# Litianyu141/Gen-FVGN-steady

Hardware: AMD Instinct MI355X
Metric: training iters/sec, 50k-cell cylinder mesh (fwd + loss + bwd + Adam, batch resident in HBM) (higher is better)
Workload: dtype f32

## Files before the change

### gen-fvgn-steady_amd/csrc/cfwd.hip

```cpp
#include <cstdlib>

#include "tchain_kernel.h"

#include "gfv_limits.h"
int* gfv_internal_status_ptr();

namespace {

constexpr float CF_SH = 16.0f;
constexpr float CF_SH_INV = 1.0f / 16.0f;
constexpr float CF_SH_LIMIT = 2048.0f;

__device__ __forceinline__ void cf_barrier() {
  asm volatile("s_waitcnt lgkmcnt(0)\n\ts_barrier" ::: "memory");
}

template <int KT0, int TG, int NW>
struct CfLds {
  static constexpr int KTB = KT0 > 4 ? KT0 : 4;
  static constexpr int B0 = 0;
  static constexpr int B1 = TG * KTB * 2048;
  static constexpr int SINV = B1 + TG * 8192;
  static constexpr int LNP = SINV + TG * 64;
  static constexpr int TOTAL = LNP + TG * 16 * NW * 8;
// ... 109 lines not shown
      for (int q = 0; q < TG; ++q) {
        const gfv_f16x8* f = reinterpret_cast<const gfv_f16x8*>(xbuf + (size_t)(q * KT + T) * 2048) + lane;
        const gfv_f16x8 xh = f[0];
        if (!LOWP) {
          const gfv_f16x8 xl = f[64];
#pragma unroll
          for (int n = 0; n < NT; ++n) {
            acc[q][n] = __builtin_amdgcn_mfma_f32_16x16x32_f16(wl[n][T], xh, acc[q][n], 0, 0, 0);
            acc[q][n] = __builtin_amdgcn_mfma_f32_16x16x32_f16(wh[n][T], xl, acc[q][n], 0, 0, 0);
          }
        }
#pragma unroll
        for (int n = 0; n < NT; ++n) acc[q][n] = gfv_mma_hh<BF>(wh[n][T], xh, acc[q][n]);
      }
    }
  };
  auto load_w = [&](const void* image) {
    const gfv_f16x8* im = reinterpret_cast<const gfv_f16x8*>(image) + (size_t)(NT * w) * 128 + lane;
#pragma unroll
    for (int T = 0; T < 4; ++T)
#pragma unroll
      for (int n = 0; n < NT; ++n) {
        wh[n][T] = im[T * 1024 + n * 128];
        if (!LOWP) wl[n][T] = im[T * 1024 + n * 128 + 64];
      }
  };
  auto hidden = [&](int layer, char* xout, float* save) {
#pragma unroll
    for (int q = 0; q < TG; ++q) {
      const int row = row0 + 16 * q + j;
      const bool live = q < ngt && row < A.M;
      const float si = layer == 0 ? sinv[q * 16 + j] : CF_SH_INV;
      float a[4 * NT];
#pragma unroll
      for (int n = 0; n < NT; ++n) {
        const float4 b = bias[layer][n];
        float v[4] = {(acc[q][n][0] * si) * invw + b.x, (acc[q][n][1] * si) * invw + b.y, (acc[q][n][2] * si) * invw + b.z,
                      (acc[q][n][3] * si) * invw + b.w};
        if (PADD && layer == 0) {
          v[0] += ps[PADD ? q : 0][n].x + pr[PADD ? q : 0][n].x; v[1] += ps[PADD ? q : 0][n].y + pr[PADD ? q : 0][n].y;
          v[2] += ps[PADD ? q : 0][n].z + pr[PADD ? q : 0][n].z; v[3] += ps[PADD ? q : 0][n].w + pr[PADD ? q : 0][n].w;
        }
        if (save && live) st4(save + (size_t)row * 128 + c0 + 16 * n, v);
        const gfv_f2 g01 = gfv_gelu2(gfv_f2{v[0], v[1]}), g23 = gfv_gelu2(gfv_f2{v[2], v[3]});
        a[4 * n + 0] = g01.x; a[4 * n + 1] = g01.y; a[4 * n + 2] = g23.x; a[4 * n + 3] = g23.y;
      }
      float m = 0.f;
#pragma unroll
      for (int e = 0; e < 4 * NT; e += 2) m = max3_abs(m, a[e], a[e + 1]);
      mabs = fmaxf(mabs, live ? m : 0.f);
      if constexpr (NT == 2) {
        float e8[8];
#pragma unroll
        for (int e = 0; e < 8; ++e) e8[e] = a[e] * CF_SH;
        gfv_uint4 hi, lo;
        gfv_split8_t<BF>(e8, hi, lo);
        gfv_uint4* dst = reinterpret_cast<gfv_uint4*>(xout + (size_t)(q * 4 + w) * 2048) + lane;
        dst[0] = hi;
        if (!LOWP) dst[64] = lo;
      } else {
        unsigned h0, h1, l0, l1;
        gfv_split_pair_t<BF>(a[0] * CF_SH, a[1] * CF_SH, h0, l0);
        gfv_split_pair_t<BF>(a[2] * CF_SH, a[3] * CF_SH, h1, l1);
        char* dst = xout + (size_t)(q * 4 + (w >> 1)) * 2048 + lane * 16 + (w & 1) * 8;
        *reinterpret_cast<uint2*>(dst) = make_uint2(h0, h1);
        if (!LOWP) *reinterpret_cast<uint2*>(dst + 1024) = make_uint2(l0, l1);
      }
    }
  };

  mma(b0, std::integral_constant<int, KT0>{});
  load_w(A.layer[1].Wh);
  hidden(0, b1, A.layer[0].save);
  cf_barrier();
  mma(b1, std::integral_constant<int, 4>{});
  load_w(A.layer[2].Wh);
  hidden(1, b0, A.layer[1].save);
  float4 gam[NT], bet[NT];
  if constexpr (FINLN) {
#pragma unroll
    for (int n = 0; n < NT; ++n) { gam[n] = ld4(A.fin_gamma + c0 + 16 * n); bet[n] = ld4(A.fin_beta + c0 + 16 * n); }
  }
  float4 rres[TG][NT];
  if (A.res[0]) {
#pragma unroll
    for (int q = 0; q < TG; ++q) {
      const float* rp = A.res[0] + (size_t)min(row0 + 16 * q + j, A.M - 1) * A.res_ld[0] + c0;
#pragma unroll
      for (int n = 0; n < NT; ++n) rres[q][n] = ld4(rp + 16 * n);
    }
  }
  cf_barrier();
  if constexpr (!FINLN) {
    if (w == 0) {
      mma(b0, std::integral_constant<int, 4>{});
      const int ncol = A.layer[2].N;
      const float* bp = A.layer[2].bias;
#pragma unroll
      for (int q = 0; q < TG; ++q) {
        const int row = row0 + 16 * q + j;
        if (q < ngt && row < A.M) {
#pragma unroll
          for (int r = 0; r < 4; ++r) {
            const int col = 4 * g + r;
            if (col < ncol) A.out[0][(size_t)row * A.out_ld[0] + col] = (acc[q][0][r] * CF_SH_INV) * invw + (bp ? bp[col] : 0.f);
          }
        }
      }
    }
    if (mabs > CF_SH_LIMIT) atomicOr(status, 2);
    return;
  }
  mma(b0, std::integral_constant<int, 4>{});
  const int hcols = (A.hidden > 0 && A.hidden < 128) ? A.hidden : 128;
  float y[TG][4 * NT];
#pragma unroll
  for (int q = 0; q < TG; ++q) {
    const int row = row0 + 16 * q + j;
    const bool live = q < ngt && row < A.M;
    float s = 0.f;
#pragma unroll
    for (int n = 0; n < NT; ++n) {
      const float4 b = bias[2][n];
      float v[4] = {(acc[q][n][0] * CF_SH_INV) * invw + b.x, (acc[q][n][1] * CF_SH_INV) * invw + b.y,
                    (acc[q][n][2] * CF_SH_INV) * invw + b.z, (acc[q][n][3] * CF_SH_INV) * invw + b.w};
      if (A.fin_presave && live) st4(A.fin_presave + (size_t)row * 128 + c0 + 16 * n, v);
#pragma unroll
      for (int r = 0; r < 4; ++r) {
        y[q][4 * n + r] = v[r];
        s += v[r];
      }
    }
    const float mw = row_sum(s) * (1.0f / (16.0f * NT));
    float m2 = 0.f;
#pragma unroll
    for (int e = 0; e < 4 * NT; ++e) {
      const float d = y[q][e] - mw;
      m2 += d * d;
    }
    m2 = row_sum(m2);
    if (g == 0) *reinterpret_cast<float2*>(lnp + ((q * 16 + j) * NW + w) * 2) = make_float2(mw, m2);
  }
  cf_barrier();
  {
    const float inv_h = 1.0f / (float)hcols, npad = (float)(128 - hcols);
#pragma unroll
    for (int q = 0; q < TG; ++q) {
      const int row = row0 + 16 * q + j;
      const bool live = q < ngt && row < A.M;
      const float4* pp = reinterpret_cast<const float4*>(lnp + (q * 16 + j) * 2 * NW);
      float m128, m2a;
      if constexpr (NW == 4) {
        const float4 p0 = pp[0], p1 = pp[1];
        m128 = ((p0.x + p0.z) + (p1.x + p1.z)) * 0.25f;
        const float e0 = p0.x - m128, e1 = p0.z - m128, e2 = p1.x - m128, e3 = p1.z - m128;
        m2a = ((p0.y + p0.w) + (p1.y + p1.w)) + 32.0f * ((e0 * e0 + e1 * e1) + (e2 * e2 + e3 * e3));
      } else {
        const float4 p0 = pp[0], p1 = pp[1], p2 = pp[2], p3 = pp[3];
        m128 = (((p0.x + p0.z) + (p1.x + p1.z)) + ((p2.x + p2.z) + (p3.x + p3.z))) * 0.125f;
        const float e0 = p0.x - m128, e1 = p0.z - m128, e2 = p1.x - m128, e3 = p1.z - m128, e4 = p2.x - m128, e5 = p2.z - m128,
                    e6 = p3.x - m128, e7 = p3.z - m128;
        m2a = (((p0.y + p0.w) + (p1.y + p1.w)) + ((p2.y + p2.w) + (p3.y + p3.w))) +
              16.0f * (((e0 * e0 + e1 * e1) + (e2 * e2 + e3 * e3)) + ((e4 * e4 + e5 * e5) + (e6 * e6 + e7 * e7)));
      }
      const float mean = hcols == 128 ? m128 : (m128 * 128.0f) * inv_h;
      const float dm = m128 - mean;
      const float m2 = hcols == 128 ? m2a : (m2a + 128.0f * dm * dm) - npad * (mean * mean);
      const float rstd = rsqrtf(m2 * inv_h + 1e-5f);
      if (A.fin_stats && live && w == 0 && g == 0) *reinterpret_cast<float2*>(A.fin_stats + 2 * (size_t)row) = make_float2(mean, rstd);
#pragma unroll
      for (int n = 0; n < NT; ++n) {
        const float4 ga = gam[n], be = bet[n];
        float o[4] = {(y[q][4 * n + 0] - mean) * rstd * ga.x + be.x, (y[q][4 * n + 1] - mean) * rstd * ga.y + be.y,
                      (y[q][4 * n + 2] - mean) * rstd * ga.z + be.z, (y[q][4 * n + 3] - mean) * rstd * ga.w + be.w};
        if (live) {
          if (A.out_nores) st4(A.out_nores + (size_t)row * 128 + c0 + 16 * n, o);
          if (A.res[0]) { o[0] += rres[q][n].x; o[1] += rres[q][n].y; o[2] += rres[q][n].z; o[3] += rres[q][n].w; }
          st4(A.out[0] + (size_t)row * A.out_ld[0] + c0 + 16 * n, o);
        }
      }
    }
  }
  if (mabs > CF_SH_LIMIT) atomicOr(status, 2);
}

inline bool cf_al16(const void* p) { return (reinterpret_cast<size_t>(p) & 15) == 0; }

template <int KT0, int N0, bool PADD, bool RAGIN, bool FINLN = true>
void cf_launch(const gfv_rowtile_args_t& a, int lowp, hipStream_t stream) {
  int* st = gfv_internal_status_ptr();
  constexpr int tg = 2;
  const int tiles = (a.M + 16 * tg - 1) / (16 * tg);
  const dim3 grid(PADD ? gfv_xcd_grid(tiles) : tiles), blk(512);
  if (lowp == 2) GFV_LAUNCH((cfwd_kernel<KT0, N0, 2, PADD, 2, RAGIN, 8, FINLN>), grid, blk, 0, stream, a, st);
  else if (lowp) GFV_LAUNCH((cfwd_kernel<KT0, N0, 2, PADD, 1, RAGIN, 8, FINLN>), grid, blk, 0, stream, a, st);
  else GFV_LAUNCH((cfwd_kernel<KT0, N0, 2, PADD, 0, RAGIN, 8, FINLN>), grid, blk, 0, stream, a, st);
}

}

int gfv_internal_cfwd_try(const gfv_rowtile_args_t* a, int lowp, hipStream_t stream, int dry) {
  if (!gfv_internal_status_ptr()) return 0;
  const int on = gfv_internal_limit(GFV_LIM_CFWD_ON);
  const int max_m = gfv_internal_limit(GFV_LIM_CFWD_MAX_M);
  if (!on || a->nlayers != 3 || a->M > max_m || a->M < 1 || (a->flags & (GFV_CHAIN_ROW_OWNER | GFV_CHAIN_COLUMN_OWNER))) return 0;
  const bool dec = a->fin_op == GFV_FIN_PLAIN && a->layer[2].N >= 1 && a->layer[2].N <= 16 && !a->res[0] && !a->out_nores && !a->fin_presave &&
                   !a->fin_stats && !a->padd && a->nseg == 1 && a->layer[0].K == 128;
  if (a->in_op != GFV_IN_NONE || !a->wmax) return 0;
  if (!dec && (a->fin_op != GFV_FIN_LN || !a->fin_gamma || !a->fin_beta)) return 0;
  if (a->in_add || a->gadd || a->in_save || a->in_aux || a->ln_partial || a->gscale || a->dw_partial || a->in_stats || a->fin_aux) return 0;
  for (int l = 0; l < 3; ++l) {
    const gfv_layer_t& L = a->layer[l];
    if (!L.Wh || (L.N != 128 && !(dec && l == 2)) || L.aux || L.bias2 || (L.bias && !cf_al16(L.bias) && !(dec && l == 2))) return 0;
    if (L.op != (l < 2 ? GFV_OP_BIAS_GELU : GFV_OP_NONE)) return 0;
    if (l > 0 && L.K != 128) return 0;
    if (L.save && !cf_al16(L.save)) return 0;
  }
  if (a->layer[2].save) return 0;
  if (!a->out[0] || a->out[1] || a->out[2] || (!dec && ((a->out_ld[0] & 3) || !cf_al16(a->out[0]))) || a->res[1] || a->res[2]) return 0;
  if (a->res[0] && ((a->res_ld[0] & 3) || !cf_al16(a->res[0]))) return 0;
  if ((a->out_nores && !cf_al16(a->out_nores)) || (a->fin_presave && !cf_al16(a->fin_presave)) ||
      (!dec && (!cf_al16(a->fin_gamma) || !cf_al16(a->fin_beta))))
    return 0;
  if (a->fin_stats && (reinterpret_cast<size_t>(a->fin_stats) & 7)) return 0;
  for (int i = 0; i < a->nseg; ++i)
    if (a->seg[i].idx || a->seg[i].csr_rowptr || a->seg[i].csr_scale || a->seg[i].save) return 0;
  const int K0 = a->layer[0].K;
  int shape = -1;
  auto plain = [&](int i, int width) {
    const gfv_seg_t& s = a->seg[i];
    return s.width == width && (s.ld & 3) == 0 && cf_al16(s.ptr);
  };
  if (a->padd) {
    if (a->nseg == 1 && K0 == 128 && plain(0, 128) && a->padd_s && a->padd_r && a->padd_ld >= 256 && (a->padd_ld & 3) == 0 && cf_al16(a->padd))
      shape = 1;
  } else if (a->nseg == 2 && K0 == 192 && plain(0, 64) && plain(1, 128)) {
    shape = 0;
  } else if (dec) {
    if (plain(0, 128)) shape = 4;
  } else if (a->nseg == 1 && K0 == 128 && plain(0, 128)) {
    shape = 2;
  } else if (a->nseg == 1 && K0 <= 32 && a->seg[0].width == K0) {
    shape = 3;
  }
  if (shape < 0) return 0;
  if (dry) return 1;
  if (shape == 0) cf_launch<6, 4, false, false>(*a, lowp, stream);
  else if (shape == 1) cf_launch<4, 8, true, false>(*a, lowp, stream);
  else if (shape == 2) cf_launch<4, 8, false, false>(*a, lowp, stream);
  else if (shape == 4) cf_launch<4, 8, false, false, false>(*a, lowp, stream);
  else cf_launch<1, 2, false, true>(*a, lowp, stream);
  return 1;
}
```

### gen-fvgn-steady_amd/csrc/colchain.hip

```cpp
#include "colchain_kernel.h"

int* gfv_internal_status_ptr();

static int cc_env(const char* name, int dflt) {
  const char* e = getenv(name);
  return e ? atoi(e) : dflt;
}
static bool al16(const void* p) { return (reinterpret_cast<size_t>(p) & 15) == 0; }

static int cc_cus() {
  static int n = 0;
  if (!n) {
    int dev = 0;
    hipDeviceProp_t pr;
    if (hipGetDevice(&dev) == hipSuccess && hipGetDeviceProperties(&pr, dev) == hipSuccess) n = pr.multiProcessorCount;
    if (n <= 0) n = 256;
    const int want = cc_env("GFV_COLCHAIN_WGS", 0);
    if (want > 0 && want <= n) n = want;
  }
  return n;
}

static bool cc_bwd_ok(const gfv_rowtile_args_t* a) {
  static const int on = cc_env("GFV_COLCHAIN_BWD", 1);
  static const int min_m = cc_env("GFV_COLCHAIN_BWD_MIN_M", 2048);
  if (a->flags & GFV_CHAIN_ROW_OWNER) return false;
  if (!(a->flags & GFV_CHAIN_COLUMN_OWNER) && (!on || a->M < min_m)) return false;
  if (!a->dw_partial || a->dw_partial_stride < GFV_DW_FUSED_FLOATS || !a->in_stats || !a->wmax) return false;
  if (a->dw_in) return false;
  const bool noout = a->nlayers == 2;
  const bool rc = a->rc_Wh[0] != nullptr;
  if (rc && (!a->rc_Wh[1] || a->dw_in || !al16(a->rc_Wh[0]) || !al16(a->rc_Wh[1]) || (a->rc_bias[0] && !al16(a->rc_bias[0])) ||
             (a->rc_bias[1] && !al16(a->rc_bias[1]))))
    return false;
  if (!rc && a->rc_Wh[1]) return false;
  if ((a->nlayers != 3 && !noout) || a->in_op != GFV_IN_LNBWD || a->fin_op != GFV_FIN_PLAIN || a->nseg != 1) return false;
  if (noout && (a->layer[1].op != GFV_OP_MUL_DGELU || a->layer[1].save || a->res[0] || a->gadd || a->dw_in || !a->out[0])) return false;
  if (a->seg[0].width != 128 || a->seg[0].idx || a->seg[0].csr_rowptr || a->seg[0].save || a->seg[0].ld != 128 || !al16(a->seg[0].ptr)) return false;
  if (a->M > (1 << 22) || a->out_ld[0] != 128 || (a->res[0] && a->res_ld[0] != 128) || (a->dw_in && a->dw_in_ld != 128)) return false;
  if (a->layer[0].op != GFV_OP_MUL_DGELU || a->layer[1].op != GFV_OP_MUL_DGELU || (!noout && a->layer[2].op != GFV_OP_NONE)) return false;
  for (int l = 0; l < a->nlayers; ++l) {
    const gfv_layer_t& L = a->layer[l];
    if (!L.Wh || (L.N != 128 && !(l == 2 && L.N == 192)) || L.K != 128 || L.bias || L.bias2) return false;
    if (l < 2 && !(rc && l == 0) && (!L.aux || !al16(L.aux))) return false;
    if (L.save && !al16(L.save)) return false;
  }
  if ((!rc && (!a->in_aux || !al16(a->in_aux))) || !a->in_gamma || !al16(a->in_gamma) || a->ln_partial || a->padd) return false;
  const bool out2 = !noout && a->layer[2].N == 192;
  if (!a->out[0] || (out2 ? (!a->out[1] || a->out_ld[1] != 64 || !al16(a->out[1]) || a->dw_in) : a->out[1] != nullptr) || a->out[2] ||
      a->res[1] || a->res[2] || a->out_nores)
    return false;
  if ((a->out_ld[0] & 3) || !al16(a->out[0]) || (a->res[0] && ((a->res_ld[0] & 3) || !al16(a->res[0])))) return false;
  if (a->in_add && !al16(a->in_add)) return false;
  if (a->gadd && (!al16(a->gadd) || !a->gadd_s || !a->gadd_r)) return false;
  if (a->in_save && !al16(a->in_save)) return false;
  if ((reinterpret_cast<size_t>(a->in_stats) & 7) || !al16(a->dw_partial) || (a->dw_partial_stride & 3)) return false;
  return true;
}
extern "C" int gfv_hidden_size(void);
extern "C" int gfv_f16split_enabled(void);
extern "C" int gfv_rowtile_dw_partials(void) { return cc_cus(); }
extern "C" int gfv_rowtile_dw_partials_m(int32_t M) {
  const int tiles = (M + 63) / 64;
  return tiles < cc_cus() ? (tiles > 0 ? tiles : 1) : cc_cus();
}
extern "C" int gfv_rowtile_fuses_dw(const gfv_rowtile_args_t* a) {
  if (!a || gfv_hidden_size() != 128 || gfv_f16split_enabled() == 0) return 0;
  gfv_rowtile_args_t t = *a;
  t.hidden = 128;
  return cc_bwd_ok(&t) ? 1 : 0;
}

int gfv_internal_colchain_try(const gfv_rowtile_args_t* a, hipStream_t stream) {
  if (a->hidden == 128 && cc_bwd_ok(a)) {
    int* st = gfv_internal_status_ptr();
    if (!st) return 0;
    const dim3 grid(gfv_rowtile_dw_partials_m(a->M)), blk(64 * CC_W);
#define CB_K(...) GFV_LAUNCH((colchain_bwd_kernel<__VA_ARGS__>), grid, blk, 0, stream, *a, st)
#define CB_LAUNCH(LOWP, RC)                                                                                                      \
  do {                                                                                                                           \
    if (a->nlayers == 2) CB_K(LOWP, false, false, true, RC);                                                                     \
    else if (a->layer[2].N == 192 && a->gadd) CB_K(LOWP, true, true, false, RC);                                                 \
    else if (a->layer[2].N == 192) CB_K(LOWP, false, true, false, RC);                                                           \
    else if (a->gadd) CB_K(LOWP, true, false, false, RC);                                                                        \
    else CB_K(LOWP, false, false, false, RC);                                                                                    \
  } while (0)
    const bool rc = a->rc_Wh[0] != nullptr;
    if (a->product_form == 2) { if (rc) CB_LAUNCH(2, true); else CB_LAUNCH(2, false); }
    else if (a->product_form != 0) { if (rc) CB_LAUNCH(1, true); else CB_LAUNCH(1, false); }
    else { if (rc) CB_LAUNCH(0, true); else CB_LAUNCH(0, false); }
#undef CB_K
#undef CB_LAUNCH
    return 2;
  }
  return 0;
}
```

### gen-fvgn-steady_amd/csrc/colchain_kernel.h

```cpp
#pragma once
#include "tchain_kernel.h"

namespace {

constexpr int CC_W = 8;
constexpr float CC_SH = 16.0f;
constexpr float CC_SH_INV = 1.0f / 16.0f;
constexpr float CC_SH_LIMIT = 2048.0f;
#ifdef GFV_CC_TIMING
#define CT_DECL long long ct_[16] = {0, 0, 0, 0, 0, 0, 0, 0, 0, 0, 0, 0, 0, 0, 0, 0}; long long ct_prev_ = clock64();
#define CT(k) do { __builtin_amdgcn_s_waitcnt(0xc07f); const long long now_ = clock64(); ct_[k] += now_ - ct_prev_; ct_prev_ = now_; } while (0)
#else
#define CT_DECL
#define CT(k)
#endif
__device__ __forceinline__ void cc_barrier() {
  asm volatile("s_waitcnt lgkmcnt(0)\n\ts_barrier" ::: "memory");
}

struct CcCtx {
  int w, lane, j, g, col0;
  int M;
  int row0;
  int ngt;
// ... 16 lines not shown
      a0 = __builtin_amdgcn_mfma_f32_16x16x32_f16(wl[T], xh0, a0, 0, 0, 0);
      a1 = __builtin_amdgcn_mfma_f32_16x16x32_f16(wl[T], xh1, a1, 0, 0, 0);
      a0 = __builtin_amdgcn_mfma_f32_16x16x32_f16(wh[T], xl0, a0, 0, 0, 0);
      a1 = __builtin_amdgcn_mfma_f32_16x16x32_f16(wh[T], xl1, a1, 0, 0, 0);
    }
    a0 = gfv_mma_hh<LOWP == 2>(wh[T], xh0, a0);
    a1 = gfv_mma_hh<LOWP == 2>(wh[T], xh1, a1);
    if (FENCE) __builtin_amdgcn_sched_barrier(0);
  }
}

template <bool BF>
__device__ __forceinline__ void cc_put_frag(char* xbuf, int q, const CcCtx& c, const float (&a)[4], float scale) {
  unsigned h0, h1, l0, l1;
  const gfv_f2 s01 = gfv_f2{a[0], a[1]} * gfv_splat2(scale), s23 = gfv_f2{a[2], a[3]} * gfv_splat2(scale);
  gfv_split_pair_t<BF>(s01.x, s01.y, h0, l0);
  gfv_split_pair_t<BF>(s23.x, s23.y, h1, l1);
  char* dst = xbuf + (size_t)((q * 4 + (c.w >> 1)) * 2) * 1024 + c.lane * 16 + (c.w & 1) * 8;
  *reinterpret_cast<uint2*>(dst) = make_uint2(h0, h1);
  *reinterpret_cast<uint2*>(dst + 1024) = make_uint2(l0, l1);
}

constexpr int CB_TG = 4;
struct CbLds {
  static constexpr int BUF = CB_TG * 8192;
  static constexpr int B0 = 0, B1 = BUF, B2 = 2 * BUF;
  static constexpr int PART = 3 * BUF;
  static constexpr int SMAX = PART + CB_TG * 16 * 8 * 8;
  static constexpr int TOTAL = SMAX + 64;
};

__device__ __forceinline__ void cb_tr_operand(const char* xbuf, int q0, int ct, int lane, gfv_f16x8& hi, gfv_f16x8& lo) {
  typedef short s4 __attribute__((ext_vector_type(4)));
  typedef __attribute__((address_space(3))) s4* lds_s4;
  const int s = lane & 15, gp = lane >> 4;
  const int off = ((q0 * 4 + (ct >> 1)) * 2) * 1024 + (16 * (s & 3) + 4 * gp + (s >> 2)) * 16 + (ct & 1) * 8;
  const char* p = xbuf + off;
  const s4 h0 = __builtin_amdgcn_ds_read_tr16_b64_v4i16((lds_s4)(p));
  const s4 l0 = __builtin_amdgcn_ds_read_tr16_b64_v4i16((lds_s4)(p + 1024));
  const s4 h1 = __builtin_amdgcn_ds_read_tr16_b64_v4i16((lds_s4)(p + 8192));
  const s4 l1 = __builtin_amdgcn_ds_read_tr16_b64_v4i16((lds_s4)(p + 8192 + 1024));
  typedef short s8 __attribute__((ext_vector_type(8)));
  const s8 h = {h0[0], h0[1], h0[2], h0[3], h1[0], h1[1], h1[2], h1[3]};
  const s8 l = {l0[0], l0[1], l0[2], l0[3], l1[0], l1[1], l1[2], l1[3]};
  hi = __builtin_bit_cast(gfv_f16x8, h);
  lo = __builtin_bit_cast(gfv_f16x8, l);
}

__device__ __forceinline__ int cb_dw_ntile(int w, int i) { return 2 * (w >> 1) + (i >> 2); }
__device__ __forceinline__ int cb_dw_ktile(int w, int i) { return 4 * (w & 1) + (i & 3); }
__device__ __forceinline__ int cb_dw_btile(int w) { return 2 * (w >> 1) + (w & 1); }
template <int LOWP>
__device__ __forceinline__ void cb_dw_tile(const char* gbuf, const char* abuf, int npairs, int w, int lane, floatx4 (&acc)[8],
                                           floatx4& accb) {
  const gfv_f16x8 ones = gfv_frag_ones<LOWP == 2>();
  const int nt0 = 2 * (w >> 1), kt0 = 4 * (w & 1);
  for (int pr = 0; pr < npairs; ++pr) {
    gfv_f16x8 gh[2], gl[2];
    cb_tr_operand(gbuf, 2 * pr, nt0, lane, gh[0], gl[0]);
    cb_tr_operand(gbuf, 2 * pr, nt0 + 1, lane, gh[1], gl[1]);
    {
      const bool odd = (w & 1) != 0;
      const gfv_f16x8 bh = odd ? gh[1] : gh[0], bl = odd ? gl[1] : gl[0];
      if (!LOWP) accb = __builtin_amdgcn_mfma_f32_16x16x32_f16(bl, ones, accb, 0, 0, 0);
      accb = gfv_mma_hh<LOWP == 2>(bh, ones, accb);
    }
#pragma unroll
    for (int kk = 0; kk < 4; ++kk) {
      gfv_f16x8 ah, al;
      cb_tr_operand(abuf, 2 * pr, kt0 + kk, lane, ah, al);
#pragma unroll
      for (int nn = 0; nn < 2; ++nn) {
        if (!LOWP) {
          acc[4 * nn + kk] = __builtin_amdgcn_mfma_f32_16x16x32_f16(gl[nn], ah, acc[4 * nn + kk], 0, 0, 0);
          acc[4 * nn + kk] = __builtin_amdgcn_mfma_f32_16x16x32_f16(gh[nn], al, acc[4 * nn + kk], 0, 0, 0);
        }
        acc[4 * nn + kk] = gfv_mma_hh<LOWP == 2>(gh[nn], ah, acc[4 * nn + kk]);
      }
    }
    __builtin_amdgcn_sched_barrier(0);
  }
}

template <bool BF>
__device__ __forceinline__ void cb_hidden_bwd(CcCtx& c, int q, const floatx4& acc, float inv_in, const float4& z, float sg,
                                              char* gout, char* aout, float (&v)[4]) {
  const gfv_f2 z01 = {z.x, z.y}, z23 = {z.z, z.w};
  gfv_f2 a01, a23, d01, d23;
  gfv_gelu_dgelu2(z01, a01, d01);
  gfv_gelu_dgelu2(z23, a23, d23);
  const gfv_f2 ki = gfv_splat2(inv_in), kw = gfv_splat2(c.invw);
  const gfv_f2 v01 = ((gfv_f2{acc[0], acc[1]} * ki) * kw) * d01, v23 = ((gfv_f2{acc[2], acc[3]} * ki) * kw) * d23;
  v[0] = v01.x; v[1] = v01.y; v[2] = v23.x; v[3] = v23.y;
  const float a[4] = {a01.x, a01.y, a23.x, a23.y};
  const float mq = max3_abs(max3_abs(0.f, v[0], v[1]), v[2], v[3]) * sg;
  const float ma = max3_abs(max3_abs(0.f, a[0], a[1]), a[2], a[3]) * (60000.0f / CC_SH_LIMIT);
  c.mabs = fmaxf(c.mabs, q < c.ngt ? fmaxf(mq, ma) : 0.f);
  cc_put_frag<BF>(gout, q, c, v, sg);
  cc_put_frag<BF>(aout, q, c, a, CC_SH);
}

__device__ __forceinline__ char* cb_own_slot(char* xbuf, int q, const CcCtx& c) {
  return xbuf + (size_t)((q * 4 + (c.w >> 1)) * 2) * 1024 + c.lane * 16 + (c.w & 1) * 8;
}
__device__ __forceinline__ void cb_park4(char* xbuf, int q, const CcCtx& c, const float (&v)[4]) {
  char* d = cb_own_slot(xbuf, q, c);
  *reinterpret_cast<float2*>(d) = make_float2(v[0], v[1]);
  *reinterpret_cast<float2*>(d + 1024) = make_float2(v[2], v[3]);
}
__device__ __forceinline__ void cb_unpark4(char* xbuf, int q, const CcCtx& c, float (&v)[4]) {
  const char* d = cb_own_slot(xbuf, q, c);
  const float2 a = *reinterpret_cast<const float2*>(d), b = *reinterpret_cast<const float2*>(d + 1024);
  v[0] = a.x; v[1] = a.y; v[2] = b.x; v[3] = b.y;
}

template <bool BF>
__device__ __forceinline__ void cb_hidden_bwd_dg(CcCtx& c, int q, const floatx4& acc, float inv_in, const float (&dg)[4], float sg,
                                                 char* gout, float (&v)[4]) {
#pragma unroll
  for (int r = 0; r < 4; ++r) v[r] = ((acc[r] * inv_in) * c.invw) * dg[r];
  const float mq = max3_abs(max3_abs(0.f, v[0], v[1]), v[2], v[3]) * sg;
  c.mabs = fmaxf(c.mabs, q < c.ngt ? mq : 0.f);
  cc_put_frag<BF>(gout, q, c, v, sg);
}

typedef int cb_i32x4 __attribute__((ext_vector_type(4)));
typedef int cb_i32x2 __attribute__((ext_vector_type(2)));
typedef __amdgpu_buffer_rsrc_t cb_rsrc;
constexpr int CB_OFF_DEAD = 0x7ffffff0;
__device__ __forceinline__ cb_rsrc cb_buf(const void* p, size_t bytes) {
  const size_t n = p ? (bytes < 0x7fffffe0ull ? bytes : 0x7fffffe0ull) : 0;
  return __builtin_amdgcn_make_buffer_rsrc(const_cast<void*>(p), 0, (int)n, 0x00020000);
}
typedef float cb_f32x2 __attribute__((ext_vector_type(2)));
__device__ __forceinline__ float4 cb_ld4(cb_rsrc r, int off) {
  const floatx4 f = __builtin_bit_cast(floatx4, __builtin_amdgcn_raw_buffer_load_b128(r, off, 0, 0));
  return make_float4(f[0], f[1], f[2], f[3]);
}
__device__ __forceinline__ float2 cb_ld2(cb_rsrc r, int off) {
  const cb_f32x2 f = __builtin_bit_cast(cb_f32x2, __builtin_amdgcn_raw_buffer_load_b64(r, off, 0, 0));
  return make_float2(f[0], f[1]);
}
__device__ __forceinline__ void cb_st4v(cb_rsrc r, int off, const floatx4& f) {
  __builtin_amdgcn_raw_buffer_store_b128(__builtin_bit_cast(cb_i32x4, f), r, off, 0, 0);
}
__device__ __forceinline__ void cb_st4(cb_rsrc r, int off, const float (&v)[4]) {
  const floatx4 f = {v[0], v[1], v[2], v[3]};
  __builtin_amdgcn_raw_buffer_store_b128(__builtin_bit_cast(cb_i32x4, f), r, off, 0, 0);
}

struct CbIn {
  float4 dy[CB_TG], yv[CB_TG], ga[CB_TG];
  float2 st[CB_TG];
};
struct CbBufs {
  cb_rsrc dy, y3, stats, z2, z1, gadd, gidx, save1, res, out;
};
__device__ __forceinline__ int cb_off(const CcCtx& c, int row0, int q) { return min(row0 + 16 * q + c.j, c.M - 1) * 512 + c.col0 * 4; }

template <bool GADD>
__device__ __forceinline__ void cb_load_gidx(const CbBufs& B, const CcCtx& c, int row0, int (&gidx)[CB_TG]) {
  if (GADD) {
#pragma unroll
    for (int q = 0; q < CB_TG; ++q) gidx[q] = __builtin_amdgcn_raw_buffer_load_b32(B.gidx, min(row0 + 16 * q + c.j, c.M - 1) * 4, 0, 0);
  }
}
__device__ __forceinline__ void cb_load_inputs(const CbBufs& B, const CcCtx& c, int row0, CbIn& in) {
#pragma unroll
  for (int q = 0; q < CB_TG; ++q) {
    const int off = cb_off(c, row0, q);
    in.dy[q] = cb_ld4(B.dy, off);
    in.yv[q] = cb_ld4(B.y3, off);
    in.st[q] = cb_ld2(B.stats, min(row0 + 16 * q + c.j, c.M - 1) * 8);
  }
}
__device__ __forceinline__ void cb_load_dy_stats(const CbBufs& B, const CcCtx& c, int row0, CbIn& in) {
#pragma unroll
  for (int q = 0; q < CB_TG; ++q) {
    in.dy[q] = cb_ld4(B.dy, cb_off(c, row0, q));
    in.st[q] = cb_ld2(B.stats, min(row0 + 16 * q + c.j, c.M - 1) * 8);
  }
}
__device__ __forceinline__ void cb_load_rows(cb_rsrc r, const CcCtx& c, int row0, float4 (&v)[CB_TG]) {
#pragma unroll
  for (int q = 0; q < CB_TG; ++q) v[q] = cb_ld4(r, cb_off(c, row0, q));
}
template <bool GADD>
__device__ __forceinline__ void cb_load_gathers(const CbBufs& B, const CcCtx& c, const int (&gidx)[CB_TG], CbIn& in) {
  if (GADD) {
#pragma unroll
    for (int q = 0; q < CB_TG; ++q) in.ga[q] = cb_ld4(B.gadd, gidx[q] * 256 + (c.col0 & 63) * 4);
  }
}

template <int LOWP, bool GADD, bool OUT2 = false, bool NOOUT = false, bool RC = false>
__global__ __launch_bounds__(64 * CC_W, 2) void colchain_bwd_kernel(const gfv_rowtile_args_t A, int* status) {
  constexpr int TG = CB_TG;
  __shared__ __attribute__((aligned(16))) char lds[CbLds::TOTAL + (RC ? CbLds::BUF : 0)];
  char* b0 = lds + CbLds::B0;
  char* b1 = lds + CbLds::B1;
  char* b2 = lds + CbLds::B2;
  char* b3 = lds + CbLds::TOTAL;
  float* part = reinterpret_cast<float*>(lds + CbLds::PART);
  float* smax = reinterpret_cast<float*>(lds + CbLds::SMAX);

  CcCtx c;
  c.w = __builtin_amdgcn_readfirstlane(threadIdx.x >> 6);
  c.lane = threadIdx.x & 63;
  c.j = c.lane & 15;
  c.g = c.lane >> 4;
  c.col0 = 16 * c.w + 4 * c.g;
  c.M = A.M;
  c.mabs = 0.f;
  c.invw = 1.0f / gfv_pow2_scale(*A.wmax);

  const int nwg = gridDim.x;
  const int wg = (nwg & 7) == 0 ? (int)(blockIdx.x & 7) * (nwg >> 3) + (int)(blockIdx.x >> 3) : (int)blockIdx.x;
  const int NG = (A.M + 15) >> 4;
  const int g_beg = (int)((long)NG * wg / nwg), g_end = (int)((long)NG * (wg + 1) / nwg);

  const size_t rows128 = (size_t)A.M * 512;
  CbBufs B;
  B.dy = cb_buf(A.seg[0].ptr, rows128);
  B.y3 = cb_buf(RC ? nullptr : A.in_aux, rows128);
  B.stats = cb_buf(A.in_stats, (size_t)A.M * 8);
  B.z2 = cb_buf(RC ? nullptr : A.layer[0].aux, rows128);
  B.z1 = cb_buf(A.layer[1].aux, rows128);
  B.gadd = cb_buf(A.gadd, 0x7fffffe0ull);
  B.gidx = cb_buf(c.w < 4 ? A.gadd_s : A.gadd_r, (size_t)A.M * 4);
  B.save1 = cb_buf(NOOUT ? A.out[0] : A.layer[1].save, rows128);
  B.res = cb_buf(NOOUT ? nullptr : A.res[0], rows128);
  B.out = cb_buf(NOOUT ? nullptr : A.out[0], rows128);
  const cb_rsrc out2 = cb_buf(OUT2 ? A.out[1] : nullptr, (size_t)A.M * 256);

  const cb_rsrc w0 = cb_buf(A.layer[0].Wh, 65536), w1 = cb_buf(A.layer[1].Wh, 65536),
                w2 = cb_buf(NOOUT ? nullptr : A.layer[2].Wh, OUT2 ? 131072 : 65536);
  const cb_rsrc rw2 = cb_buf(RC ? A.rc_Wh[0] : nullptr, 65536), rw3 = cb_buf(RC ? A.rc_Wh[1] : nullptr, 65536);
  const int woff = (c.w * 128 + c.lane) * 16;
  floatx4 dw3[8], dw2[8], db3 = floatx4{0.f, 0.f, 0.f, 0.f}, db2 = db3;
#pragma unroll
  for (int kt = 0; kt < 8; ++kt) dw3[kt] = dw2[kt] = floatx4{0.f, 0.f, 0.f, 0.f};
  float dgam[4] = {0.f, 0.f, 0.f, 0.f}, dbet[4] = {0.f, 0.f, 0.f, 0.f};
  float sacc = 0.f;
  float scap = 3.0e38f;

  float step1, step2;
  {
    float l1[2];
#pragma unroll
    for (int l = 0; l < 2; ++l) {
      const cb_rsrc wb = l == 0 ? w0 : w1;
      float acc = 0.f;
#pragma unroll
      for (int T = 0; T < 4; ++T) {
        const gfv_f16x8 h = __builtin_bit_cast(gfv_f16x8, __builtin_amdgcn_raw_buffer_load_b128(wb, woff + T * 16384, 0, 0));
        const gfv_f16x8 lo = __builtin_bit_cast(gfv_f16x8, __builtin_amdgcn_raw_buffer_load_b128(wb, woff + T * 16384 + 1024, 0, 0));
        if (LOWP == 2) {
          const gfv_bf16x8 hb = __builtin_bit_cast(gfv_bf16x8, h);
#pragma unroll
          for (int e = 0; e < 8; ++e) acc += fabsf((float)hb[e]);
        } else {
#pragma unroll
          for (int e = 0; e < 8; ++e) acc += fabsf((float)h[e] + (float)lo[e]);
        }
      }
      l1[l] = gfv_wave_max(row_sum(acc));
    }
    if (c.lane == 0) { smax[c.w] = l1[0]; part[c.w] = l1[1]; }
    cc_barrier();
    float m0 = 0.f, m1 = 0.f;
#pragma unroll
    for (int k = 0; k < 8; ++k) { m0 = fmaxf(m0, smax[k]); m1 = fmaxf(m1, part[k]); }
    cc_barrier();
    const float g0 = 1.13f * m0 * c.invw, g1 = 1.13f * m1 * c.invw;
    step1 = 1.0f / gfv_pow2_ceil(g0);
    step2 = 1.0f / gfv_pow2_ceil(g1);
  }

  constexpr bool PRE = true;
  int gidx[TG] = {0, 0, 0, 0};
  CbIn in;
  float4 zn[RC ? TG : 1];
  if (g_beg < g_end) {
    cb_load_gidx<GADD>(B, c, 16 * g_beg, gidx);
    if constexpr (RC) {
      cb_load_rows(B.z1, c, 16 * g_beg, zn);
      cb_load_dy_stats(B, c, 16 * g_beg, in);
      cb_load_gathers<GADD>(B, c, gidx, in);
    } else if (PRE) {
      cb_load_inputs(B, c, 16 * g_beg, in);
      cb_load_gathers<GADD>(B, c, gidx, in);
    }
  }
  const bool CB_LATE = c.w >= 4;
  CT_DECL
  for (int t0 = g_beg; t0 < g_end; t0 += TG) {
    c.row0 = 16 * t0;
    c.ngt = min(TG, g_end - t0);
    const int np = (c.ngt + 1) >> 1;
    const int next_row0 = t0 + TG < g_end ? 16 * (t0 + TG) : c.M;
    int offL[TG], offS[TG];
#pragma unroll
    for (int q = 0; q < TG; ++q) {
      const int row = c.row0 + 16 * q + c.j;
      offL[q] = cb_off(c, c.row0, q);
      offS[q] = (q < c.ngt && row < c.M) ? row * 512 + c.col0 * 4 : CB_OFF_DEAD;
    }
    if constexpr (RC) {
      gfv_f16x8 rh[4], rl[4];
#pragma unroll
      for (int T = 0; T < 4; ++T) {
        rh[T] = __builtin_bit_cast(gfv_f16x8, __builtin_amdgcn_raw_buffer_load_b128(rw2, woff + T * 16384, 0, 0));
        rl[T] = __builtin_bit_cast(gfv_f16x8, __builtin_amdgcn_raw_buffer_load_b128(rw2, woff + T * 16384 + 1024, 0, 0));
      }
      const float4 zero4 = make_float4(0.f, 0.f, 0.f, 0.f);
#pragma unroll
      for (int q = 0; q < TG; ++q) {
        const float z4[4] = {zn[q].x, zn[q].y, zn[q].z, zn[q].w};
        float a[4];
#pragma unroll
        for (int r = 0; r < 4; ++r) a[r] = gfv_gelu(z4[r]);
        const float ma = max3_abs(max3_abs(0.f, a[0], a[1]), a[2], a[3]) * (60000.0f / CC_SH_LIMIT);
        c.mabs = fmaxf(c.mabs, q < c.ngt ? ma : 0.f);
        cc_put_frag<LOWP == 2>(b3, q, c, a, CC_SH);
      }
// ... 135 lines not shown
      s3 = fminf(gfv_pow2_scale(mx * 13.5f) * 2.0f, scap);
      scap = fminf(scap, s3 * 1048576.0f);
#pragma unroll
      for (int q = 0; q < TG; ++q) {
        const float4* pp = reinterpret_cast<const float4*>(part + (q * 16 + c.j) * 16);
        const float4 p0 = pp[0], p1 = pp[1], p2 = pp[2], p3 = pp[3];
        const float m1 = (((p0.x + p0.z) + (p1.x + p1.z)) + ((p2.x + p2.z) + (p3.x + p3.z))) * 0.0078125f;
        const float m2 = (((p0.y + p0.w) + (p1.y + p1.w)) + ((p2.y + p2.w) + (p3.y + p3.w))) * 0.0078125f;
        float g3[4];
#pragma unroll
        for (int h = 0; h < 2; ++h) {
          const int r = 2 * h;
          const gfv_f2 t = gfv_splat2(rs[q]) * ((gfv_f2{gg[q][r], gg[q][r + 1]} - gfv_splat2(m1)) - gfv_f2{xh[q][r], xh[q][r + 1]} * gfv_splat2(m2));
          g3[r] = t.x; g3[r + 1] = t.y;
        }
        if (A.in_save) cb_st4(cb_buf(A.in_save, rows128), offS[q], g3);
        cc_put_frag<LOWP == 2>(b0, q, c, g3, s3);
      }
    }
    if (sacc != 0.f && sacc != s3) {
      const float ratio = s3 / sacc;
#pragma unroll
      for (int kt = 0; kt < 8; ++kt) { dw3[kt] *= ratio; dw2[kt] *= ratio; }
      db3 *= ratio;
      db2 *= ratio;
    }
    sacc = s3;
    const float s2s = s3 * step1, s1s = s2s * step2;
    if (A.gscale && c.w == 0 && c.lane < c.ngt) {
      const size_t grp = (size_t)(c.row0 >> 4) + c.lane;
      A.gscale[grp] = s3 * 0.25f;
      A.gscale[(size_t)A.gscale_ld + grp] = s2s * 0.25f;
      A.gscale[2 * (size_t)A.gscale_ld + grp] = s1s * 0.25f;
    }
    CT(2);
    cc_barrier();
    CT(3);
    cb_load_gidx<GADD>(B, c, next_row0, gidx);
    {
      const float inv_in = 1.0f / s3;
      floatx4 a0, a1;
      cc_mma_pair<4, LOWP, true>(b0, 0, wh, wl, c.lane, a0, a1);
#pragma unroll
      for (int p = 0; p < TG / 2; ++p) {
        if (p >= np) break;
        floatx4 n0 = a0, n1 = a1;
        float v0[4], v1[4];
        if (!CB_LATE && p + 1 < TG / 2) cc_mma_pair<4, LOWP, true>(b0, p + 1, wh, wl, c.lane, n0, n1);
        if constexpr (RC) {
          float d0[4], d1[4];
          cb_unpark4(b1, 2 * p, c, d0);
          cb_unpark4(b1, 2 * p + 1, c, d1);
          cb_hidden_bwd_dg<LOWP == 2>(c, 2 * p, a0, inv_in, d0, s2s, b1, v0);
          cb_hidden_bwd_dg<LOWP == 2>(c, 2 * p + 1, a1, inv_in, d1, s2s, b1, v1);
        } else {
          cb_hidden_bwd<LOWP == 2>(c, 2 * p, a0, inv_in, zq[2 * p], s2s, b1, b2, v0);
          cb_hidden_bwd<LOWP == 2>(c, 2 * p + 1, a1, inv_in, zq[2 * p + 1], s2s, b1, b2, v1);
        }
        if (A.layer[0].save) {
          const cb_rsrc s0 = cb_buf(A.layer[0].save, rows128);
          cb_st4(s0, offS[2 * p], v0);
          cb_st4(s0, offS[2 * p + 1], v1);
        }
        if (CB_LATE && p + 1 < TG / 2) cc_mma_pair<4, LOWP, true>(b0, p + 1, wh, wl, c.lane, n0, n1);
        a0 = n0; a1 = n1;
      }
    }
#pragma unroll
    for (int T = 0; T < 4; ++T) {
      wh[T] = __builtin_bit_cast(gfv_f16x8, __builtin_amdgcn_raw_buffer_load_b128(w1, woff + T * 16384, 0, 0));
      wl[T] = __builtin_bit_cast(gfv_f16x8, __builtin_amdgcn_raw_buffer_load_b128(w1, woff + T * 16384 + 1024, 0, 0));
    }
#pragma unroll
    for (int q = 0; q < TG; ++q) zq[q] = cb_ld4(B.z1, offL[q]);
    CT(4);
    cc_barrier();
    CT(5);
    if constexpr (RC) cb_load_rows(B.z1, c, next_row0, zn);
    cb_dw_tile<LOWP>(b0, b2, np, c.w, c.lane, dw3, db3);
    if constexpr (RC) cb_dw_tile<LOWP>(b1, b3, np, c.w, c.lane, dw2, db2);
    CT(6);
    cc_barrier();
    CT(7);
    {
      const float inv_in = 1.0f / s2s;
      floatx4 a0, a1;
      cc_mma_pair<4, LOWP, true>(b1, 0, wh, wl, c.lane, a0, a1);
#pragma unroll
      for (int p = 0; p < TG / 2; ++p) {
        if (p >= np) break;
        floatx4 n0 = a0, n1 = a1;
        float v0[4], v1[4];
        if (!CB_LATE && p + 1 < TG / 2) cc_mma_pair<4, LOWP, true>(b1, p + 1, wh, wl, c.lane, n0, n1);
        if constexpr (RC) {
          const float d0[4] = {gfv_dgelu(zq[2 * p].x), gfv_dgelu(zq[2 * p].y), gfv_dgelu(zq[2 * p].z), gfv_dgelu(zq[2 * p].w)};
          const float d1[4] = {gfv_dgelu(zq[2 * p + 1].x), gfv_dgelu(zq[2 * p + 1].y), gfv_dgelu(zq[2 * p + 1].z),
                               gfv_dgelu(zq[2 * p + 1].w)};
          cb_hidden_bwd_dg<LOWP == 2>(c, 2 * p, a0, inv_in, d0, s1s, b0, v0);
          cb_hidden_bwd_dg<LOWP == 2>(c, 2 * p + 1, a1, inv_in, d1, s1s, b0, v1);
        } else {
          cb_hidden_bwd<LOWP == 2>(c, 2 * p, a0, inv_in, zq[2 * p], s1s, b0, b2, v0);
          cb_hidden_bwd<LOWP == 2>(c, 2 * p + 1, a1, inv_in, zq[2 * p + 1], s1s, b0, b2, v1);
        }
        cb_st4(B.save1, offS[2 * p], v0);
        cb_st4(B.save1, offS[2 * p + 1], v1);
        if (CB_LATE && p + 1 < TG / 2) cc_mma_pair<4, LOWP, true>(b1, p + 1, wh, wl, c.lane, n0, n1);
        a0 = n0; a1 = n1;
      }
    }
    if constexpr (!NOOUT) {
#pragma unroll
      for (int T = 0; T < 4; ++T) {
        wh[T] = __builtin_bit_cast(gfv_f16x8, __builtin_amdgcn_raw_buffer_load_b128(w2, woff + T * 16384, 0, 0));
        wl[T] = __builtin_bit_cast(gfv_f16x8, __builtin_amdgcn_raw_buffer_load_b128(w2, woff + T * 16384 + 1024, 0, 0));
      }
    }
    float4 rr[NOOUT ? 1 : TG];
    if constexpr (!NOOUT) {
#pragma unroll
      for (int q = 0; q < TG; ++q) rr[q] = cb_ld4(B.res, offL[q]);
    }
    CT(8);
    cc_barrier();
    CT(9);
    if constexpr (!NOOUT) {
      const float inv_in = 1.0f / s1s;
      floatx4 a0, a1;
      cc_mma_pair<4, LOWP, true>(b0, 0, wh, wl, c.lane, a0, a1);
#pragma unroll
      for (int p = 0; p < TG / 2; ++p) {
        if (p >= np) break;
        floatx4 n0 = a0, n1 = a1;
        if (!CB_LATE && p + 1 < TG / 2) cc_mma_pair<4, LOWP, true>(b0, p + 1, wh, wl, c.lane, n0, n1);
        const floatx4 o0 = (a0 * inv_in) * c.invw + floatx4{rr[2 * p].x, rr[2 * p].y, rr[2 * p].z, rr[2 * p].w};
        const floatx4 o1 = (a1 * inv_in) * c.invw + floatx4{rr[2 * p + 1].x, rr[2 * p + 1].y, rr[2 * p + 1].z, rr[2 * p + 1].w};
        cb_st4v(B.out, offS[2 * p], o0);
        cb_st4v(B.out, offS[2 * p + 1], o1);
        if (CB_LATE && p + 1 < TG / 2) cc_mma_pair<4, LOWP, true>(b0, p + 1, wh, wl, c.lane, n0, n1);
        a0 = n0; a1 = n1;
      }
      if constexpr (OUT2) {
        if (c.w < 4) {
          gfv_f16x8 xh2[4], xl2[4];
#pragma unroll
          for (int T = 0; T < 4; ++T) {
            xh2[T] = __builtin_bit_cast(gfv_f16x8, __builtin_amdgcn_raw_buffer_load_b128(w2, 65536 + woff + T * 16384, 0, 0));
            xl2[T] = __builtin_bit_cast(gfv_f16x8, __builtin_amdgcn_raw_buffer_load_b128(w2, 65536 + woff + T * 16384 + 1024, 0, 0));
          }
#pragma unroll
          for (int p = 0; p < TG / 2; ++p) {
            if (p >= np) break;
            floatx4 e0, e1;
            cc_mma_pair<4, LOWP, true>(b0, p, xh2, xl2, c.lane, e0, e1);
            const floatx4 o0 = (e0 * inv_in) * c.invw, o1 = (e1 * inv_in) * c.invw;
            const int ra = c.row0 + 32 * p + c.j, rb = ra + 16;
            cb_st4v(out2, (2 * p < c.ngt && ra < c.M) ? ra * 256 + c.col0 * 4 : CB_OFF_DEAD, o0);
            cb_st4v(out2, (2 * p + 1 < c.ngt && rb < c.M) ? rb * 256 + c.col0 * 4 : CB_OFF_DEAD, o1);
          }
        }
      }
    }
    CT(10);
    if constexpr (RC) {
      cb_load_dy_stats(B, c, next_row0, in);
      cb_load_gathers<GADD>(B, c, gidx, in);
    } else {
      if (PRE) {
        cb_load_inputs(B, c, next_row0, in);
        cb_load_gathers<GADD>(B, c, gidx, in);
      }
      cb_dw_tile<LOWP>(b1, b2, np, c.w, c.lane, dw2, db2);
    }
    CT(11);
  }

#ifdef GFV_CC_TIMING
  if (c.lane == 0 && A.fin_aux) {
    long long* dbg = reinterpret_cast<long long*>(const_cast<float*>(A.fin_aux)) + ((size_t)blockIdx.x * CC_W + c.w) * 16;
    for (int kk = 0; kk < 16; ++kk) dbg[kk] = ct_[kk];
  }
#endif
  if (A.dw_partial) {
    float* blk = A.dw_partial + (size_t)blockIdx.x * A.dw_partial_stride;
    const float is = sacc != 0.f ? 1.0f / sacc : 0.f;
    const float r2 = 1.0f / step1, r1 = r2 / step2;
    const float u3 = is * CC_SH_INV, u2 = (is * r2) * CC_SH_INV;
#pragma unroll
    for (int kt = 0; kt < 8; ++kt)
#pragma unroll
      for (int r = 0; r < 4; ++r) {
        const int n = 16 * cb_dw_ntile(c.w, kt) + 4 * c.g + r, k = 16 * cb_dw_ktile(c.w, kt) + c.j;
        blk[n * 128 + k] = dw3[kt][r] * u3;
        blk[16384 + 128 + n * 128 + k] = dw2[kt][r] * u2;
      }
    if (c.j == 0) {
#pragma unroll
      for (int r = 0; r < 4; ++r) {
        const int nb = 16 * cb_dw_btile(c.w) + 4 * c.g + r;
        blk[16384 + nb] = db3[r] * is;
        blk[2 * 16384 + 128 + nb] = db2[r] * (is * r2);
      }
    }
#pragma unroll
    for (int r = 0; r < 4; ++r) {
      const float dg = gfv_row16_sum(dgam[r]), db = gfv_row16_sum(dbet[r]);
      if (c.j == 0) {
        blk[2 * 16384 + 256 + c.col0 + r] = dg;
        blk[2 * 16384 + 384 + c.col0 + r] = db;
      }
    }
  }
  if (c.mabs > 60000.0f) atomicOr(status, 2);
}


}
```

### gen-fvgn-steady_amd/csrc/rowtile.hip

```cpp
#include <atomic>
#include <stdio.h>
#include <stdlib.h>
#include <mutex>
#include "gfv_common.h"
#include "gfv_limits.h"
#include "gfv_prof.h"
#include "../../include/gfv.h"

namespace {
constexpr int BM = 64;
}

int gfv_internal_tchain_launch(const gfv_rowtile_args_t* args, int ragged, int f16, hipStream_t stream);

static std::atomic<int> g_f16_default{-1};
static thread_local int g_f16split = -1;
static int f16_default() {
  int d = g_f16_default.load(std::memory_order_relaxed);
  if (d < 0) {
    const char* e = getenv("GFV_F16SPLIT");
    d = e ? ((atoi(e) == 2 || atoi(e) == 3) ? atoi(e) : (atoi(e) != 0)) : 1;
    int expect = -1;
    if (!g_f16_default.compare_exchange_strong(expect, d)) d = expect;
  }
// ... 22 lines not shown

static thread_local int g_last_path = -1;
extern "C" int gfv_rowtile_last_path(void) { return g_last_path; }
namespace {
struct LimitDef { const char* env; int dflt; };
const LimitDef k_limits[GFV_LIM_COUNT] = {
    {"GFV_CBWD", 1},        {"GFV_CBWD_MAX_M", 25000},      {"GFV_CFWD", 1},          {"GFV_CFWD_MAX_M", 250000},
    {"GFV_CTRANS", 1},         {"GFV_CTRANS_MAX_M", 16384},
    {"GFV_LIN1S", 1},       {"GFV_LIN1S_MAX_M", 16384}};
int g_limit[GFV_LIM_COUNT];
bool g_limit_set[GFV_LIM_COUNT];
std::once_flag g_limit_once;
void limits_init() {
  for (int i = 0; i < GFV_LIM_COUNT; ++i) {
    const char* e = getenv(k_limits[i].env);
    g_limit[i] = e ? atoi(e) : k_limits[i].dflt;
    g_limit_set[i] = false;
  }
}
}
int gfv_internal_limit(int which) {
  std::call_once(g_limit_once, limits_init);
  return (which >= 0 && which < GFV_LIM_COUNT) ? g_limit[which] : 0;
}
extern "C" int gfv_get_limit(int32_t which) { return (which >= 0 && which < GFV_LIM_COUNT) ? gfv_internal_limit(which) : -1; }
extern "C" int gfv_set_limit(int32_t which, int32_t value) {
  if (which < 0 || which >= GFV_LIM_COUNT) return GFV_ERR_ARG;
  std::call_once(g_limit_once, limits_init);
  if (value < 0) {
    const char* e = getenv(k_limits[which].env);
    g_limit[which] = e ? atoi(e) : k_limits[which].dflt;
  } else {
    g_limit[which] = value;
  }
  return GFV_OK;
}
extern "C" const char* gfv_limit_name(int32_t which) { return (which >= 0 && which < GFV_LIM_COUNT) ? k_limits[which].env : nullptr; }

static thread_local int g_last_ln_rows = 0;
extern "C" int gfv_rowtile_last_ln_rows(void) { return g_last_ln_rows; }

extern "C" int gfv_rowtile_tiles(int32_t M) { return (M + BM - 1) / BM; }

static int rowtile_chain_impl(const gfv_rowtile_args_t* args, void* stream);
extern "C" int gfv_rowtile_chain(const gfv_rowtile_args_t* args, void* stream) {
  if (!args) return GFV_ERR_ARG;
  if (args->product_form < 0 || args->product_form > 4 || (args->hidden != 0 && (args->hidden < 16 || args->hidden > 128 || (args->hidden & 15))))
    return GFV_ERR_ARG;
  if (args->product_form == 0 && args->hidden == 0) return rowtile_chain_impl(args, stream);
  const int f0 = g_f16split, h0 = g_hidden;
  if (args->product_form) g_f16split = args->product_form - 1;
  if (args->hidden) g_hidden = args->hidden;
  const int rc = rowtile_chain_impl(args, stream);
  g_f16split = f0;
  g_hidden = h0;
  return rc;
}
int gfv_internal_lin1_try(const gfv_rowtile_args_t* a, int lowp, hipStream_t stream, int dry);
int gfv_internal_cfwd_try(const gfv_rowtile_args_t* a, int lowp, hipStream_t stream, int dry);
bool gfv_internal_wimg_form_ok(const float* wmax);
int gfv_internal_cbwd_try(const gfv_rowtile_args_t* a, int lowp, hipStream_t stream, int dry);
static int cfwd_try(const gfv_rowtile_args_t* args, int lowp, hipStream_t stream, int dry) {
  if (args->nlayers != 3 || (args->fin_op != GFV_FIN_LN && args->fin_op != GFV_FIN_PLAIN)) return 0;
  gfv_rowtile_args_t local = *args;
  local.hidden = g_hidden;
  return gfv_internal_cfwd_try(&local, lowp, stream, dry);
}
static int cbwd_try(const gfv_rowtile_args_t* args, int lowp, hipStream_t stream, int dry) {
  if (args->in_op != GFV_IN_LNBWD || args->dw_partial || !args->in_stats) return 0;
  gfv_rowtile_args_t local = *args;
  local.hidden = g_hidden;
  return gfv_internal_cbwd_try(&local, lowp, stream, dry);
}
static int rowtile_chain_impl(const gfv_rowtile_args_t* args, void* stream) {
  if (!args || args->M < 0 || args->nlayers < 1 || args->nlayers > 3 || args->nseg < 1 || args->nseg > 3) return GFV_ERR_ARG;
  if (args->M == 0) {
    g_last_ln_rows = 0;
    return GFV_OK;
  }
  for (int i = 0; i < args->nseg; ++i)
    if (args->seg[i].width < 1 || args->seg[i].width > 128) return GFV_ERR_ARG;
  for (int l = 0; l + 1 < args->nlayers; ++l)
    if (args->layer[l].N != 128 || args->layer[l + 1].K != 128) return GFV_ERR_ARG;
  int k0 = 0;
  for (int i = 0; i < args->nseg; ++i) k0 += args->seg[i].width;
  if (k0 != args->layer[0].K) return GFV_ERR_ARG;
  const gfv_layer_t& last = args->layer[args->nlayers - 1];
  if (last.N > 384 || last.N < 1) return GFV_ERR_ARG;
  if ((args->rc_Wh[0] || args->rc_Wh[1]) && !args->dw_partial) return GFV_ERR_ARG;
  if (args->padd && (args->nlayers < 2 || args->padd_ld < 256 || (args->padd_ld & 3) || !args->padd_s || !args->padd_r)) return GFV_ERR_ARG;
  for (int l = 0; l < args->nlayers; ++l)
    if (args->layer[l].ldw != 0 && args->layer[l].ldw < args->layer[l].K) return GFV_ERR_ARG;
  if (last.N > 128 && (last.N & 15)) return GFV_ERR_ARG;
  if ((args->fin_op != GFV_FIN_PLAIN || args->in_op == GFV_IN_LN || args->in_op == GFV_IN_LNBWD) &&
      (args->fin_op != GFV_FIN_PLAIN ? last.N != 128 : false))
    return GFV_ERR_ARG;
  if ((args->in_op == GFV_IN_LN || args->in_op == GFV_IN_LNBWD) && (args->nseg != 1 || args->seg[0].width != 128))
    return GFV_ERR_ARG;
  bool fast_t = true;
  for (int i = 0; i < args->nseg; ++i) fast_t = fast_t && (args->seg[i].width % 32 == 0) && (args->seg[i].ld % 4 == 0);
  for (int l = 0; l < args->nlayers; ++l) {
    const bool lastl = (l == args->nlayers - 1);
    fast_t = fast_t && (args->layer[l].K % 4 == 0) && (args->layer[l].ldw % 4 == 0) && (args->layer[l].N % (lastl ? 64 : 128) == 0);
  }
  if (args->fin_op != GFV_FIN_PLAIN) fast_t = fast_t && last.N == 128;
  for (int c = 0; c < 3; ++c) {
    if (args->out[c]) fast_t = fast_t && (args->out_ld[c] % 4 == 0);
    if (args->res[c]) fast_t = fast_t && (args->res_ld[c] % 4 == 0);
  }
  bool rag_t = !fast_t && args->in_op != GFV_IN_LNBWD && args->fin_op != GFV_FIN_LNBWD;
  for (int l = 0; l + 1 < args->nlayers; ++l) rag_t = rag_t && args->layer[l].N == 128;
  if (last.N > 128) rag_t = rag_t && (last.N % 64 == 0);
  if (last.N % 16) rag_t = rag_t && last.op != GFV_OP_MUL_DGELU && args->fin_op == GFV_FIN_PLAIN && !args->out_nores;
  if (args->in_op == GFV_IN_LN) rag_t = rag_t && args->seg[0].width == 128 && (args->seg[0].ld % 4 == 0);
  if (args->gadd) rag_t = rag_t && args->seg[0].width == 128 && (args->seg[0].ld % 4 == 0);
  for (int l = 1; l < args->nlayers; ++l) rag_t = rag_t && (args->layer[l].K == 128);
  {
    bool csr = false;
    for (int i = 0; i < args->nseg; ++i) {
      const gfv_seg_t& sg = args->seg[i];
      csr = csr || sg.csr_rowptr != nullptr || sg.save != nullptr;
      if (sg.csr_rowptr && (!sg.idx || (i == 0 && args->in_add))) return GFV_ERR_ARG;
    }
    if (csr && (!fast_t || args->in_op == GFV_IN_LNBWD || args->fin_op == GFV_FIN_LNBWD))
      return GFV_ERR_ARG;
  }
  bool f16 = (fast_t || rag_t) && f16_mode() != 0 && args->wmax != nullptr;
  for (int l = 0; l < args->nlayers; ++l) f16 = f16 && args->layer[l].Wh != nullptr;
  for (int i = 0; i + 1 < args->nseg; ++i) f16 = f16 && (args->seg[i].width % 32 == 0);
  if (f16 && !gfv_internal_wimg_form_ok(args->wmax)) return GFV_ERR_ARG;
  for (int l = 0; l < args->nlayers; ++l)
    if ((!args->layer[l].W || args->layer[l].bias2) && !f16) return GFV_ERR_ARG;
  if (!fast_t && !rag_t) {
    static const bool dbg = getenv("GFV_ROWTILE_DEBUG") != nullptr;
    if (dbg)
      fprintf(stderr, "[gfv] gfv_rowtile_chain: unsupported shape M=%d nseg=%d widths=%d,%d,%d ld0=%d nlayers=%d K0=%d Nlast=%d out_ld=%d in_op=%d fin_op=%d\n",
              args->M, args->nseg, args->seg[0].width, args->nseg > 1 ? args->seg[1].width : 0,
              args->nseg > 2 ? args->seg[2].width : 0, args->seg[0].ld, args->nlayers, args->layer[0].K, last.N,
              args->out_ld[0], args->in_op, args->fin_op);
    return GFV_ERR_ARG;
  }
  void* tok = nullptr;
  if (gfv_prof_enabled()) {
    double fl = 0, by = 0;
    for (int l = 0; l < args->nlayers; ++l) {
      fl += 2.0 * args->M * (double)args->layer[l].K * args->layer[l].N;
      by += 4.0 * ((double)args->layer[l].K * args->layer[l].N + args->layer[l].N);
      if (args->layer[l].save) by += 4.0 * args->M * args->layer[l].N;
      if (args->layer[l].aux) by += 4.0 * args->M * args->layer[l].N;
    }
    by += 4.0 * args->M * (double)args->layer[0].K + 4.0 * args->M * (double)last.N;
    for (int i = 0; i < args->nseg; ++i) if (args->seg[i].idx) by += 4.0 * args->M;
    if (args->in_aux || args->fin_aux) by += 4.0 * args->M * 128.0;
    if (args->in_save) by += 4.0 * args->M * 128.0;
    if (args->fin_presave) by += 4.0 * args->M * 128.0;
    if (args->out_nores) by += 4.0 * args->M * 128.0;
    if (args->padd) by += 4.0 * args->M * 258.0;
    for (int c = 0; c < 3; ++c) if (args->res[c]) by += 4.0 * args->M * 128.0;
    const int lnm = args->in_op == GFV_IN_LNBWD ? 1 : (args->fin_op == GFV_FIN_LNBWD ? 2 : 0);
    int kind = fast_t ? GFV_K_TCHAIN0 + lnm : GFV_K_TCHAIN_RAG;
    for (int i = 0; i < args->nseg; ++i)
      if (args->seg[i].csr_rowptr || args->seg[i].save) kind = GFV_K_TCHAIN_CSR;
    if (fast_t && f16 && args->nlayers == 1 && gfv_internal_lin1_try(args, f16_mode() >= 2 ? f16_mode() - 1 : 0, (hipStream_t)stream, 1))
      kind = GFV_K_LIN1;
    if (f16 && cfwd_try(args, f16_mode() >= 2 ? f16_mode() - 1 : 0, (hipStream_t)stream, 1))
      kind = GFV_K_COLCHAIN_FWD;
    if (args->dw_partial) {
      kind = GFV_K_COLCHAIN_BWD;
      const int nfused = 2 + (args->rc_Wh[0] ? 2 : 0);
      fl += nfused * 2.0 * args->M * 128.0 * 128.0;
      by += 8.0 * args->M + 4.0 * (double)gfv_rowtile_dw_partials_m(args->M) * (double)args->dw_partial_stride;
    }
    tok = gfv_prof_begin(kind, fl, by, (hipStream_t)stream);
  }
  g_last_path = (fast_t ? 1 : 2) + (f16 ? 4 : 0);
  g_last_ln_rows = (args->M + BM - 1) / BM;
  if (args->dw_partial && !(fast_t && f16)) return GFV_ERR_ARG;
  if (fast_t && f16 && args->nlayers == 1 && gfv_internal_lin1_try(args, f16_mode() >= 2 ? f16_mode() - 1 : 0, (hipStream_t)stream, 0)) {
    g_last_path += 32;
  } else if (f16 && !args->dw_partial && cfwd_try(args, f16_mode() >= 2 ? f16_mode() - 1 : 0, (hipStream_t)stream, 0)) {
    g_last_path += 64;
  } else if (fast_t && f16 && cbwd_try(args, f16_mode() >= 2 ? f16_mode() - 1 : 0, (hipStream_t)stream, 0)) {
    g_last_path += 128;
    g_last_ln_rows = (args->M + 31) / 32;
  } else if (fast_t) {
    const int took = gfv_internal_tchain_launch(args, 0, f16 ? 1 : 0, (hipStream_t)stream);
    if (args->dw_partial && took != 2) return GFV_ERR_ARG;
    g_last_path += 8 * took;
  }
  else
    gfv_internal_tchain_launch(args, 1, f16 ? 1 : 0, (hipStream_t)stream);
  gfv_prof_end(tok, (hipStream_t)stream);
  GFV_CHECK_LAUNCH();
  return GFV_OK;
}
```

### gen-fvgn-steady_amd/csrc/tchain_kernel.h

```cpp
#pragma once
#include <stdlib.h>
#include "gfv_common.h"
#include "gfv_prof.h"
#include "gfv_split.h"
#include "../../include/gfv.h"

#ifdef GFV_TIMING
#define TS_DECL long long ts_[10] = {0, 0, 0, 0, 0, 0, 0, 0, 0, 0}; long long t_prev_ = clock64(); const long long t_start_ = t_prev_;
#define TS(k) do { const long long now_ = clock64(); ts_[k] += now_ - t_prev_; t_prev_ = now_; } while (0)
#define TS_WAIT() __builtin_amdgcn_s_waitcnt(0)
#else
#define TS_DECL
#define TS(k)
#define TS_WAIT()
#endif

namespace {

constexpr int WK = 32;
constexpr int WS_FLOATS = 128 * WK;
constexpr int PAR_GAMMA = 640, PAR_BETA = 768, PAR_FLOATS = 896;

struct WBlk {
  const float* w;
// ... 622 lines not shown
            } else {
              {
                const float4 b = ld4(par + 128 * layer + 16 * nt + 4 * g);
                v[0] += b.x; v[1] += b.y; v[2] += b.z; v[3] += b.w;
              }
              if (layer == 0 && A.padd) {
                const float4 pa = ld4(pad_s[tt] + 16 * nt), pb = ld4(pad_r[tt] + 16 * nt);
                v[0] += pa.x + pb.x; v[1] += pa.y + pb.y; v[2] += pa.z + pb.z; v[3] += pa.w + pb.w;
              }
              if (lop == GFV_OP_BIAS_GELU) {
                if (L.save && live) st4_save(L.save + mrow + 16 * nt, v);
#pragma unroll
                for (int r = 0; r < 4; ++r) v[r] = gfv_gelu(v[r]);
              }
            }
#pragma unroll
            for (int r = 0; r < 4; ++r) act[tt][nt][r] = v[r];
          }
        }
        if (H) {
          sx = row_scale(act[0]);
          if (A.gscale && lop == GFV_OP_MUL_DGELU) group_scale_out(A.gscale + (size_t)(layer + 1) * A.gscale_ld + rowgroup, sx, lane);
          to_halves<BF>(act[0], sx, xh, xl);
        }
        TS_WAIT();
        TS(6);
      } else {
        float* out = pass == 0 ? A.out[0] : (pass == 1 ? A.out[1] : A.out[2]);
        const float* res = pass == 0 ? A.res[0] : (pass == 1 ? A.res[1] : A.res[2]);
        const int old = pass == 0 ? A.out_ld[0] : (pass == 1 ? A.out_ld[1] : A.out_ld[2]);
        const int rld = pass == 0 ? A.res_ld[0] : (pass == 1 ? A.res_ld[1] : A.res_ld[2]);
        const int ncols = min(128, L.N - 128 * pass);
        const int ntv = (ncols + 15) >> 4;
        const bool rag_out = RAG && ((ncols & 15) || (old & 3));
        float dgam[8][4], dbet[8][4];
        if (lnb_fin) {
#pragma unroll
          for (int t = 0; t < 8; ++t)
#pragma unroll
            for (int r = 0; r < 4; ++r) dgam[t][r] = dbet[t][r] = 0.f;
        }
#pragma unroll
        for (int tt = 0; tt < T; ++tt) {
          const int m = rowbase + 16 * tt;
          const bool live = m < A.M;
          const size_t mc = (size_t)(live ? m : A.M - 1);
          float v[8][4];
#pragma unroll
          for (int nt = 0; nt < 8; ++nt) {
#pragma unroll
            for (int r = 0; r < 4; ++r) v[nt][r] = H ? (acc[tt][nt][r] * invx) * invw : acc[tt][nt][r];
            if (nt < ntv) {
              const float4 b = ld4(par + 128 * layer + 128 * pass + 16 * nt + 4 * g);
              v[nt][0] += b.x; v[nt][1] += b.y; v[nt][2] += b.z; v[nt][3] += b.w;
            }
            if (L.op == GFV_OP_MUL_DGELU && nt < ntv) {
              const float4 z = ld4(L.aux + mc * (size_t)L.N + 128 * pass + 16 * nt + 4 * g);
              v[nt][0] *= gfv_dgelu(z.x); v[nt][1] *= gfv_dgelu(z.y); v[nt][2] *= gfv_dgelu(z.z); v[nt][3] *= gfv_dgelu(z.w);
            }
          }
          if (A.fin_op == GFV_FIN_LN) {
            if (A.fin_presave && live) {
#pragma unroll
              for (int nt = 0; nt < 8; ++nt) st4_save(A.fin_presave + mc * 128 + 16 * nt + 4 * g, v[nt]);
            }
            ln_apply(v, par + PAR_GAMMA, par + PAR_BETA, g, lnw, (A.fin_stats && live) ? A.fin_stats + 2 * mc : nullptr);
          } else if (lnb_fin) {
            float y[8][4];
#pragma unroll
            for (int nt = 0; nt < 8; ++nt) {
              const float4 yy = ld4(A.fin_aux + mc * 128 + 16 * nt + 4 * g);
              y[nt][0] = yy.x; y[nt][1] = yy.y; y[nt][2] = yy.z; y[nt][3] = yy.w;
              const float livef = live ? 1.0f : 0.0f;
              v[nt][0] *= livef; v[nt][1] *= livef; v[nt][2] *= livef; v[nt][3] *= livef;
            }
            if (tt == 0) ln_bwd<true>(v, y, par + PAR_GAMMA, g, dgam, dbet, lnw);
            else ln_bwd<false>(v, y, par + PAR_GAMMA, g, dgam, dbet, lnw);
          }
          if (H && A.gscale && npass == 1 && A.nlayers <= 2 && L.op == GFV_OP_MUL_DGELU && !res) {
            float rs = row_scale(v);
            if (!live) rs = 8.5070592e37f;
            group_scale_out(A.gscale + (size_t)A.nlayers * A.gscale_ld + rowgroup, rs, lane);
          }
          if (live) {
            if (pass == 0 && A.out_nores) {
#pragma unroll
              for (int nt = 0; nt < 8; ++nt) st4(A.out_nores + mc * 128 + 16 * nt + 4 * g, v[nt]);
            }
#pragma unroll
            for (int nt = 0; nt < 8; ++nt) {
              if (nt < ntv) {
                if (rag_out) {
#pragma unroll
                  for (int r = 0; r < 4; ++r) {
                    const int col = 16 * nt + 4 * g + r;
                    if (col < ncols) out[mc * (size_t)old + col] = v[nt][r] + (res ? res[mc * (size_t)rld + col] : 0.f);
                  }
                } else {
                  if (res) {
                    const float4 rv = ld4(res + mc * (size_t)rld + 16 * nt + 4 * g);
                    v[nt][0] += rv.x; v[nt][1] += rv.y; v[nt][2] += rv.z; v[nt][3] += rv.w;
                  }
                  st4(out + mc * (size_t)old + 16 * nt + 4 * g, v[nt]);
                }
              }
            }
          }
        }
        if (lnb_fin) ln_park(dgam, dbet, red, wave, li, g);
        TS_WAIT();
        TS(7);
      }
    }
  }

#ifdef GFV_TIMING
  if (A.ln_partial && LNM == 0) {
    ts_[8] = clock64() - t_start_;
    ts_[9] = t_start_;
    if (lane == 0)
      for (int k = 0; k < 10; ++k) reinterpret_cast<long long*>(A.ln_partial)[((size_t)blockIdx.x * 4 + wave) * 10 + k] = ts_[k];
    return;
  }
#endif
  if (A.ln_partial) {
    __syncthreads();
    const int q = tid >> 8, t = tid & 255;
    const float* rq = red + q * 1024;
    const float s = rq[t] + rq[256 + t] + rq[512 + t] + rq[768 + t];
    const size_t tile64 = (size_t)tile * (NW / 4) * T + q * T;
    if (tile64 < (size_t)((A.M + 63) / 64)) A.ln_partial[tile64 * 256 + t] = s;
#pragma unroll
    for (int x = 1; x < T; ++x)
      if (tile64 + x < (size_t)((A.M + 63) / 64)) A.ln_partial[(tile64 + x) * 256 + t] = 0.f;
  }
}

}
```

### gen-fvgn-steady_amd/gfv/engine.py

```python
from __future__ import annotations

import contextlib
import os
import struct

import torch

from . import cmdlist
from . import lib as L
from . import ops
from .ops import LayerSpec, Seg

_MODE = {"explicit": 0, "implicit": 1, "imex": 2}


def _empty(dev, *shape):
    return torch.empty(shape, dtype=torch.float32, device=dev)


def pick_concurrent_stream(priority=0, candidates=8):
    if torch.cuda.is_current_stream_capturing():
        return torch.cuda.Stream(priority=priority)
    main = torch.cuda.current_stream()
    cycles = 400_000
# ... 12 lines not shown
        e1.record(main)
        torch.cuda.synchronize()
        return e0.elapsed_time(e1)

    timed(None)
    alone = min(timed(None) for _ in range(2))
    first = None
    for _ in range(candidates):
        cand = torch.cuda.Stream(priority=priority)
        first = first or cand
        timed(cand)
        if min(timed(cand) for _ in range(2)) < 1.5 * alone:
            return cand
    return first


class GradStore:

    def __init__(self, names, shapes, device, flat=None, skip=()):
        self.off, self.shape = {}, {}
        off = 0
        for n, sh in zip(names, shapes):
            k = 1
            for d in sh:
                k *= int(d)
            self.off[n], self.shape[n] = off, tuple(sh)
            off += (k + 3) // 4 * 4
        self.total = off
        self.flat = torch.zeros(off, dtype=torch.float32, device=device) if flat is None else flat
        self.skip = set(skip)

    def numel(self, n):
        k = 1
        for d in self.shape[n]:
            k *= d
        return k

    def view(self, n):
        if n in self.skip:
            return None
        return self.flat[self.off[n]:self.off[n] + self.numel(n)].view(self.shape[n])

    def block(self, first, last):
        end = self.off[last] + (self.numel(last) + 3) // 4 * 4
        return self.off[first], end - self.off[first]


class Engine:
    def __init__(self, message_passing_num=3, integrator="imex", ncn_smooth=True, net="TransFVGN_v2", conserved_form=True,
                 order="2nd", hidden=128):
        self.hidden = int(hidden)
        self._dw_ws, self._dw_ws_main = None, None
        self._pending = []
        self._defer_mode = os.environ.get("GFV_DEFER", "1") == "1"
        self._wt, self._wt_key, self._wt_live = {}, None, False
        self._wt_desc, self._wt_n, self._wt_max = None, 0, (0, 0)
        self._last_gn = False
        self.mp = message_passing_num
        self.mode = _MODE[integrator]
        self.smooth = 1 if ncn_smooth else 0
        self.nc = 0 if conserved_form else 1
        if order not in ("1st", "2nd", "3rd", "4th"):
            raise ValueError("order must be specified in [\"1st\", \"2nd\", \"3rd\", \"4th\"]")
        self.order_terms = {"1st": 2, "2nd": 5, "3rd": 9, "4th": 14}[order]
        self.n_proc = 2 if net in ("TransFVGN_v2", "TransFVGN") else 1
        self.net = net
        self.overlap = os.environ.get("GFV_OVERLAP", "1") != "0"
        self.factor = os.environ.get("GFV_EDGE_FACTOR", "1") != "0"
        self.f16split = os.environ.get("GFV_F16SPLIT", "1") != "0"
        self.csr_fuse = ops.csr_prologue_enabled()
        self._fuse_mask = int(os.environ.get("GFV_CSR_FUSE_MASK", "4"))
        self._csr1_max = int(os.environ.get("GFV_CSR1_MAX_M", "16384"))
        self.fuse_dw = os.environ.get("GFV_FUSE_DW", "1") != "0"
        self.recompute = os.environ.get("GFV_RECOMPUTE", "0") != "0"
        self._slice_fuse = os.environ.get("GFV_SLICE_FUSE", "1") != "0"
        self._trans_fuse = os.environ.get("GFV_TRANS_FUSE", "1") != "0"
        self._trans_fuse_min = int(os.environ.get("GFV_TRANS_FUSE_MIN_M", "16385"))
        self._trans_fuse_fwd_small = bool(L.get_limit("GFV_CTRANS")) if torch.cuda.is_available() else True
        self._trans_reduce_merge = os.environ.get("GFV_TRANS_REDUCE_MERGE", "1") != "0"
        self._tail_env = ("GFV_TAIL_MAIN" in os.environ) or ("GFV_TAIL_SPLIT" in os.environ)
        self._tail_main = int(os.environ.get("GFV_TAIL_MAIN", "2"))
        self._tail_split = int(os.environ.get("GFV_TAIL_SPLIT", "1"))
        self._fuse_noout = os.environ.get("GFV_FUSE_NOOUT", "1") != "0"
        self._fuse_dw_min = int(os.environ.get("GFV_COLCHAIN_BWD_MIN_M", "2048"))
        self._cbwd_max_fixed = None
        self._wi, self._wi_key, self._wmax, self._wi_abs = None, None, None, None
        self._pkey_cache = None
        self._zero_e = None
        self._etmp = None
        self._prep_ws = None
        self._fvm_cnt = None
        self._fvm_fuse = os.environ.get("GFV_FVM_FUSE", "1") != "0"
        self._agg_ln = os.environ.get("GFV_AGG_LN", "1") != "0"
        self._side, self._sides = None, []
        self._keep = []
        self.dist_world, self.dist_group, self.dist_force = 1, None, False
        self._retired = []
        self.bucket_hook = None

    class _Fork:
        def __init__(self, eng, keep):
            self.eng, self.keep = eng, keep

        def __enter__(self):
            e = self.eng
            if not e.overlap:
                return self
            if e._side is None:
                e._side = pick_concurrent_stream()
                e._sides = [e._side]
            L.stream_wait(e._side, torch.cuda.current_stream())
            e._keep.extend(t for t in self.keep if t is not None)
            self._ctx = torch.cuda.stream(e._side)
            self._ctx.__enter__()
            return self

        def __exit__(self, *exc):
            if self.eng.overlap:
                self._ctx.__exit__(*exc)
            return False

    def fork(self, *keep):
        return Engine._Fork(self, keep)

    @contextlib.contextmanager
    def model_width(self):
        lib = L.load()
        if self.hidden == 128 and lib.gfv_hidden_size() == 128:
            yield
            return
        L.check(lib.gfv_set_hidden_size(self.hidden), "gfv_set_hidden_size")
        try:
            yield
        finally:
            L.check(lib.gfv_set_hidden_size(128), "gfv_set_hidden_size")

    @property
    def _cbwd_max(self):
        if self._cbwd_max_fixed is not None:
            return self._cbwd_max_fixed
        return L.get_limit("GFV_CBWD_MAX_M") if L.get_limit("GFV_CBWD") else 0

    def _tail_cfg(self, pl):
        if self._tail_env:
            return self._tail_main, self._tail_split
        if pl.E < 32000:
            return 2, 0
        return (2, 2) if pl.E < 150000 else (2, 1)

    def defer(self, fn, *keep):
        if not self.overlap:
            fn()
        elif self._defer_mode:
            self._pending.append((fn, keep))
        else:
            with self.fork(*keep):
                fn()

    def flush(self, on_main=False, split=0):
        if not self._pending:
            return
        pend, self._pending = self._pending, []
        if split and len(pend) > 1:
            k = 1 if split == 1 else len(pend) - 1
            main_part, side_part = (pend[:k], pend[k:]) if split == 1 else (pend[k:], pend[:k])
            self._pending = side_part
            self.flush()
            self._pending = main_part
            self.flush(on_main=True)
            return
        if on_main:
            ws, self._dw_ws = self._dw_ws, self._dw_ws_main
            try:
                for fn, _ in pend:
                    fn()
            finally:
# ... 52 lines not shown
        if self._wi is None or self._wi_key != self._pkey(P, fresh=True):
            raise RuntimeError("static weight images belong to another parameter set: call build_static_images(P) first")
        wi = self._wi["fwd"]
        if len(wi.valid) != len(wi.images) and cmdlist.active() is None:
            L.check(L.load().gfv_weight_absmax(self._wi_abs[0].data_ptr(), self._wi_abs[1], self._wmax.data_ptr(),
                                               L.stream_ptr()), "gfv_weight_absmax")
            wi.build()
        return ops.set_weight_images(wi)

    def capture_signature(self):
        wi = self._wi or {}
        return (self._wi_key, self._wt_key, L.load().gfv_f16split_enabled(),
                tuple((ph, len(w.images), None if w._desc is None else w._desc.data_ptr()) for ph, w in sorted(wi.items())))

    def _wi_exit(self, phase, prev):
        if not self.f16split:
            return
        self._wi[phase].invalidate()
        ops.set_weight_images(prev)

    def _T(self, W, perm=False):
        hit = self._wt.get((W.data_ptr(), perm)) if self._wt_live else None
        if hit is not None:
            return hit
        if not perm:
            return ops.transpose(W)
        if perm == "c":
            return ops.transpose(W, col0=256, ncols=128)
        if perm == "ab":
            return torch.cat((ops.transpose(W, col0=0, ncols=128), ops.transpose(W, col0=128, ncols=128)), 1).contiguous()
        out = _empty(W.device, 192, 128)
        ops.transpose(W, out=out[0:128], col0=64, ncols=128)
        ops.transpose(W, out=out[128:192], col0=0, ncols=64)
        return out

    def prepare_transposes(self, P):
        lib = L.load()
        key = self._pkey(P)
        if self._wt_key != key:
            rows = []
            self._retired.append((self._wt, self._wt_desc))
            self._wt = {}
            dev = next(iter(P.values())).device
            for n, W in P.items():
                if not n.endswith(".weight") or W.dim() != 2:
                    continue
                if any(t in n for t in (".to_q.", ".to_k.", ".to_v.", ".in_project_slice.")):
                    continue
                if ".encoder." in n and n.endswith(".0.0.weight"):
                    continue
                r, c = W.shape
                if ".nb_module.net.0.0.weight" in n:
                    out = _empty(dev, 192, 128)
                    rows.append((W.data_ptr() + 4 * 64, out.data_ptr(), r, 128, c, 0))
                    rows.append((W.data_ptr(), out.data_ptr() + 4 * 128 * 128, r, 64, c, 0))
                    self._wt[(W.data_ptr(), True)] = out
                elif self.factor and ".eb_module.net.0.0.weight" in n:
                    oc, oab = _empty(dev, 128, 128), _empty(dev, 128, 256)
                    rows.append((W.data_ptr() + 4 * 256, oc.data_ptr(), r, 128, c, 0))
                    rows.append((W.data_ptr(), oab.data_ptr(), r, 128, c, 256))
                    rows.append((W.data_ptr() + 4 * 128, oab.data_ptr() + 4 * 128, r, 128, c, 256))
                    self._wt[(W.data_ptr(), "c")] = oc
                    self._wt[(W.data_ptr(), "ab")] = oab
                else:
                    out = _empty(dev, c, r)
                    rows.append((W.data_ptr(), out.data_ptr(), r, c, c, 0))
                    self._wt[(W.data_ptr(), False)] = out
            blob = b"".join(struct.pack("<QQiiii", a, b, r, c, ld, ldo) for a, b, r, c, ld, ldo in rows)
            self._wt_desc = torch.frombuffer(bytearray(blob), dtype=torch.uint8).to(dev)
            self._wt_n = len(rows)
            self._wt_max = (max(r[2] for r in rows), max(r[3] for r in rows))
            self._wt_key = key
        L.check(lib.gfv_transpose_batch(self._wt_desc.data_ptr(), self._wt_n, self._wt_max[0], self._wt_max[1],
                                        L.stream_ptr()), "gfv_transpose_batch")
        self._wt_live = True

    @staticmethod
    def _mlp_names(prefix, ln):
        lin = prefix + ".0" if ln else prefix
        return [f"{lin}.0.weight", f"{lin}.0.bias", f"{lin}.2.weight", f"{lin}.2.bias", f"{lin}.4.weight",
                f"{lin}.4.bias"] + ([f"{prefix}.1.weight", f"{prefix}.1.bias"] if ln else [])

    def mlp3_fwd(self, P, prefix, M, segs, *, ln=True, res=None, in_add=None, want_nores=False, keep=True, w1=None,
                 padd=None, saved_segs=None, nores_from_saved=False):
        names = self._mlp_names(prefix, ln)
        W1, b1, W2, b2, W3, b3 = (P[n] for n in names[:6])
        if w1 is not None:
            W1 = w1
        dev = W1.device
        nout = W3.shape[0]
        would_fuse = (ln and self.fuse_dw and self.f16split and self.hidden == 128 and nout == 128
                      and M >= self._fuse_dw_min and M > self._cbwd_max
                      and (self._fuse_noout or all(sg.width % 32 == 0 for sg in segs)))
        fused_bwd = keep and would_fuse
        would_stats = would_fuse or (ln and self.f16split and nout == 128 and M <= self._cbwd_max)
        lean = fused_bwd and self.recompute
        if keep:
            stats = _empty(dev, M, 2) if would_stats else None
            z1 = _empty(dev, M, 128)
            z2 = _empty(dev, M, 128) if not lean else None
            y3 = _empty(dev, M, 128) if (ln and not lean) else None
        else:
            from_saved = (want_nores and nores_from_saved and would_stats and ln and nout == 128
                          and not (would_fuse and self.recompute))
            z1 = z2 = None
            y3 = _empty(dev, M, 128) if from_saved else None
            stats = _empty(dev, M, 2) if from_saved else None
        out = _empty(dev, M, nout)
        if want_nores and nores_from_saved and y3 is not None and stats is not None and nout == 128:
            want_nores = False
        nores = _empty(dev, M, 128) if want_nores else None
        ops.rowtile_chain(
            M, segs,
            [LayerSpec(W1, b1, L.OP_BIAS_GELU, save=z1), LayerSpec(W2, b2, L.OP_BIAS_GELU, save=z2), LayerSpec(W3, b3)],
            [out], in_add=in_add, fin_op=L.FIN_LN if ln else L.FIN_PLAIN,
            fin_gamma=P[names[6]] if ln else None, fin_beta=P[names[7]] if ln else None, fin_presave=y3,
            res=[res] if res is not None else None, out_nores=nores, fin_stats=stats,
            **(dict(padd=padd[0], padd_s=padd[1], padd_r=padd[2]) if padd is not None else {}))
        if not keep:
            return out, nores, dict(y3=y3, stats=stats)
        saved = dict(z1=z1, z2=z2, y3=y3, segs=segs if saved_segs is None else saved_segs, in_add=in_add, M=M, ln=ln,
                     prefix=prefix, stats=stats, lean=lean, fused=fused_bwd)
        return out, nores, saved

    def _rematerialize(self, P, sv):
        if not sv.get("lean") or sv["z2"] is not None:
            return
        names = self._mlp_names(sv["prefix"], sv["ln"])
        M, dev = sv["M"], sv["z1"].device
        sv["z2"], sv["y3"] = _empty(dev, M, 128), _empty(dev, M, 128)
        ops.rowtile_chain(M, [Seg(sv["z1"])], [LayerSpec(P[names[2]], P[names[3]], L.OP_BIAS_GELU, save=sv["z2"]),
                                              LayerSpec(P[names[4]], P[names[5]])], [sv["y3"]], in_op=L.IN_GELU)

    def mlp3_bwd(self, P, sv, G, grads, *, outs=None, res=None, gadd=None, W1t=None, g_ld=None, g_add=None):
        prefix, M, ln = sv["prefix"], sv["M"], sv["ln"]
        names = self._mlp_names(prefix, ln)
        W1, W2, W3 = P[names[0]], P[names[2]], P[names[4]]
        dev = W1.device
        nout = W3.shape[0]
        W3t, W2t = self._T(W3), self._T(W2)
        if (self.fuse_dw and ln and sv.get("fused", sv.get("stats") is not None) and G.stride(0) == 128 and g_ld is None and gadd is None
                and (outs is not None or (res is None and self._fuse_noout))
                and self._mlp3_bwd_fused(P, sv, G, grads, names, W3t, W2t,
                                         None if outs is None else (W1t if W1t is not None else self._T(W1)), outs, res, g_add)):
            return
        self._rematerialize(P, sv)
        gz2, gz1 = _empty(dev, M, 128), _empty(dev, M, 128)
        part = _empty(dev, ops.ln_rows(M), 2, 128) if ln else None
        g3 = _empty(dev, M, 128) if ln else G
        gseg = Seg(G, width=nout, ld=G.stride(0) if g_ld is None else g_ld)
        kw = dict(in_op=L.IN_LNBWD, in_gamma=P[names[6]], in_aux=sv["y3"], in_save=g3, ln_partial=part,
                  in_stats=sv.get("stats")) if ln else {}
        if gadd is not None:
            kw.update(gadd=gadd[0], gadd_s=gadd[1], gadd_r=gadd[2])
        if g_add is not None:
            assert ln, "the addend is folded into the LayerNorm-backward prologue"
            kw.update(in_add=g_add)
        gs = _empty(dev, 3, ops.gscale_ld(M))
        if outs is not None:
            if W1t is None:
                W1t = self._T(W1)
            have = ops.rowtile_chain(M, [gseg],
                                     [LayerSpec(W3t, None, L.OP_MUL_DGELU, save=gz2, aux=sv["z2"]),
                                      LayerSpec(W2t, None, L.OP_MUL_DGELU, save=gz1, aux=sv["z1"]), LayerSpec(W1t)],
                                     outs, res=res, gscale=gs, **kw)
        else:
            have = ops.rowtile_chain(M, [gseg],
                                     [LayerSpec(W3t, None, L.OP_MUL_DGELU, save=gz2, aux=sv["z2"]),
                                      LayerSpec(W2t, None, L.OP_MUL_DGELU, aux=sv["z1"])], [gz1], gscale=gs, **kw)
        tiles_n = ops.last_ln_rows()
        s0, s1, s2 = (gs[0], gs[1], gs[2]) if have else (None, None, None)
        if not ln and (gadd is not None or g_add is not None):
            s0 = None
        tiles = self._first_layer_tiles(sv, gz1, s2)
        tiles.append(self._tile(gz2, 128, Seg(sv["z1"]), a_op=1, gscale=s1))
        tiles.append(self._tile(g3, nout, Seg(sv["z2"]), a_op=1, ldg=(G.stride(0) if g_ld is None else g_ld) if not ln else None,
                                gscale=s0))
        def side():
            lay = [(names[0], names[1], len(sv["segs"])), (names[2], names[3], 1), (names[4], names[5], 1)]
            pieces = [self._slab_piece(grads, lay, self._dw_block(grads, lay, tiles, M, reduce=False))]
            if ln:
                pieces.append(self._ln_piece(part, tiles_n, grads, names[6], names[7]))
            ops.reduce_multi(pieces)
        self.defer(side, gz1, gz2, g3, G, part, gs, sv["z1"], sv["z2"], sv["in_add"], *[sg.t for sg in sv["segs"]],
                   *[sg.idx for sg in sv["segs"]])

    def _mlp3_bwd_fused(self, P, sv, G, grads, names, W3t, W2t, W1t, outs, res, g_add):
        M = sv["M"]
        dev = G.device
        lib = L.load()
        nwg = lib.gfv_rowtile_dw_partials_m(M)
        dwp = _empty(dev, nwg, L.DW_FUSED_FLOATS)
        gz1 = _empty(dev, M, 128)
        gs = _empty(dev, 3, ops.gscale_ld(M))
        if outs is None:
            layers = [LayerSpec(W3t, None, L.OP_MUL_DGELU, aux=sv["z2"]), LayerSpec(W2t, None, L.OP_MUL_DGELU, aux=sv["z1"])]
            outs = [gz1]
        else:
            layers = [LayerSpec(W3t, None, L.OP_MUL_DGELU, aux=sv["z2"]),
                      LayerSpec(W2t, None, L.OP_MUL_DGELU, save=gz1, aux=sv["z1"]), LayerSpec(W1t)]
        kw = dict(res=res, in_op=L.IN_LNBWD, in_gamma=P[names[6]], in_aux=sv["y3"], in_stats=sv["stats"], dw_partial=dwp, gscale=gs,
                  in_add=g_add, rc=(P[names[2]], P[names[3]], P[names[4]], P[names[5]]) if sv["z2"] is None else None)
        if not ops.rowtile_chain(M, [Seg(G)], layers, outs, query_fused=True, **kw):
            return False
        ops.rowtile_chain(M, [Seg(G)], layers, outs, **kw)
        segs = sv["segs"]
        fused_pieces = self._fused_pieces(dwp, nwg, grads, names)

        def side():
            lay = [(names[0], names[1], len(segs))]
            first = self._dw_block(grads, lay, self._first_layer_tiles(sv, gz1, gs[2]), M, reduce=False)
            ops.reduce_multi([self._slab_piece(grads, lay, first)] + fused_pieces)
        self.defer(side, dwp, gz1, gs, sv["in_add"], *[sg.t for sg in segs], *[sg.idx for sg in segs])
        return True

    @staticmethod
    def _gview2(grads, n0, n1):
        off, length = grads.block(n0, n1)
        return grads.flat[off:off + length]

    @staticmethod
    def _piece(partial, out, n_chunks, chunk_stride, cols, rows=1, ld_out=None):
        p = dict(partial=partial, out=out, n_chunks=n_chunks, chunk_stride=chunk_stride, rows=rows, cols=cols)
        if ld_out is not None:
            p["ld_out"] = ld_out
        return p

    def _ln_piece(self, part, n_rows, grads, gamma, beta):
        return self._piece(part, self._gview2(grads, gamma, beta), n_rows, 256, 256)

    def _fused_pieces(self, dwp, nwg, grads, names):
        base, FL, WB = dwp.data_ptr(), L.DW_FUSED_FLOATS, L.DW_FUSED_WB
        return [self._piece(base + 4 * L.DW_FUSED_OFF_W2, self._gview2(grads, names[2], names[3]), nwg, FL, WB),
                self._piece(base + 4 * L.DW_FUSED_OFF_W3, self._gview2(grads, names[4], names[5]), nwg, FL, WB),
                self._piece(base + 4 * L.DW_FUSED_OFF_LN, self._gview2(grads, names[6], names[7]), nwg, FL, 256)]

    @staticmethod
    def _layers_block(grads, layers):
        last = layers[-1]
        return grads.block(layers[0][0], last[1] if last[1] is not None else last[0])

    def _slab_piece(self, grads, layers, slabs):
        wptr, n, blen, _ = slabs
        return self._piece(wptr, grads.flat.data_ptr() + 4 * self._layers_block(grads, layers)[0], n, blen, blen)

    def _first_layer_tiles(self, sv, gz1, scale):
        return [self._tile(gz1, 128, sg, in_add=sv["in_add"] if i == 0 else None, gscale=scale,
                           a_op=L.DW_COLSCALE if sg.width <= 16 else 0) for i, sg in enumerate(sv["segs"])]

    @staticmethod
    def _tile(G, n_out, seg, *, a_op=0, a_gamma=None, a_beta=None, in_add=None, ldg=None, g_offset=0, gscale=None):
        return dict(G=G, n_out=n_out, seg=seg, a_op=a_op, a_gamma=a_gamma, a_beta=a_beta, in_add=in_add,
                    ldg=G.stride(0) if ldg is None else ldg, g_offset=g_offset, gscale=gscale)

    def _workspace(self, n_floats, dev):
        if self._dw_ws is None or self._dw_ws.numel() < n_floats or self._dw_ws.device != dev:
            self._dw_ws = torch.zeros(int(n_floats * 1.25) + 1024, dtype=torch.float32, device=dev)
        return self._dw_ws

    def _dw_block(self, grads, layers, tiles, M, row0s=None, reduce=True, ws_offset=0):
        lib = L.load()
        off0, blen = self._layers_block(grads, layers)
        ct = (L.DwTile * 6)()
        ti = 0
        for li, (wname, bname, nt) in enumerate(layers):
            K = grads.shape[wname][1]
            koff = 0
            for j in range(nt):
                t, c = tiles[ti], ct[ti]
                sg = t["seg"]
                row0 = 0 if row0s is None else row0s[ti]
                c.G = t["G"].data_ptr() + 4 * t["g_offset"]
                c.A = sg.t.data_ptr() + 4 * sg.offset
                c.idx = None if sg.idx is None else sg.idx.data_ptr()
                c.in_add = None if t["in_add"] is None else t["in_add"].data_ptr()
                c.a_gamma = None if t["a_gamma"] is None else t["a_gamma"].data_ptr()
                c.a_beta = None if t["a_beta"] is None else t["a_beta"].data_ptr()
                c.gscale = None if t.get("gscale") is None else t["gscale"].data_ptr()
                c.ldg, c.n_out, c.width, c.ld = t["ldg"], t["n_out"], sg.width, sg.ld
                c.a_op, c.ld_out = t["a_op"], K
                if row0s is None:
                    c.out_off = grads.off[wname] - off0 + koff
                    c.db_off = (grads.off[bname] - off0) if (bname is not None and j == 0) else -1
                    koff += sg.width
                else:
                    c.out_off = grads.off[wname] - off0 + row0 * K
                    c.db_off = (grads.off[bname] - off0 + row0) if bname is not None else -1
                ti += 1
        need = lib.gfv_dw_multi_workspace_floats(M, ti, blen)
        dev = grads.flat.device
        ws = self._workspace(ws_offset + need, dev)
        wptr = ws.data_ptr() + 4 * ws_offset
        L.check(lib.gfv_dw_multi(ct, ti, M, blen, wptr, (grads.flat.data_ptr() + 4 * off0) if reduce else None, 0,
                                 L.stream_ptr()), "gfv_dw_multi")
        if not reduce:
            return wptr, lib.gfv_dw_slabs(M, ti, None), blen, (need + 3) // 4 * 4

    def _dw_jobs(self, grads, jobs, pieces=()):
        lib = L.load()
        dev = grads.flat.device
        needs = [(lib.gfv_dw_multi_workspace_floats(j["M"], len(j["tiles"]), self._layers_block(grads, j["layers"])[1]) + 3) // 4 * 4
                 for j in jobs]
        self._workspace(sum(needs) + 8, dev)
        out, off = [], 0
        for j, need in zip(jobs, needs):
            slabs = self._dw_block(grads, j["layers"], j["tiles"], j["M"], row0s=j.get("row0s"), reduce=False, ws_offset=off)
            assert slabs[3] <= need
            out.append(self._slab_piece(grads, j["layers"], slabs))
            off += need
        out += list(pieces)
        for k in range(0, len(out), 12):
            ops.reduce_multi(out[k:k + 12])

    @staticmethod
    def _put(grads, name, value):
        cmdlist.call(grads.view(name).copy_, value.reshape(grads.shape[name]))

    def gn_fwd(self, P, prefix, x, e, pl, keep=True):
        N, E = pl.N, pl.E
        fuse = self.csr_fuse
        if self.factor:
            W1 = P[f"{prefix}.eb_module.net.0.0.weight"]
            pab = _empty(x.device, N, 256)
            if fuse and ((self._fuse_mask & 1) or N <= self._csr1_max) and ops.stack_ready(W1[:, 0:128], W1[:, 128:256], rows=True):
                nb = _empty(x.device, N, 128) if keep else None
                ops.rowtile_chain(N, [Seg(x, csr=(pl.n_rowptr, pl.n_col_node), save=nb)],
                                  [LayerSpec(W1[:, 0:128], stack=W1[:, 128:256])], [(pab, 256), (pab.data_ptr() + 512, 256)])
            else:
                nb = ops.seg_gather_sum(x, pl.n_rowptr, pl.n_col_node, N)
                ops.rowtile_chain(N, [Seg(nb)], [LayerSpec(W1[:, 0:128], stack=W1[:, 128:256])],
                                  [(pab, 256), (pab.data_ptr() + 512, 256)])
            e_out, e_new, sv_e = self.mlp3_fwd(P, f"{prefix}.eb_module.net", E, [Seg(e)], res=e, want_nores=True,
                                               w1=W1[:, 256:384], padd=(pab, pl.es, pl.er), nores_from_saved=self._agg_ln, keep=keep)
            sv_e["nb"] = nb
        else:
            nb = ops.seg_gather_sum(x, pl.n_rowptr, pl.n_col_node, N)
            e_out, e_new, sv_e = self.mlp3_fwd(P, f"{prefix}.eb_module.net", E, [Seg(nb, pl.es), Seg(nb, pl.er), Seg(e)],
                                               res=e, want_nores=True, nores_from_saved=self._agg_ln, keep=keep)
        if e_new is None:
            ln_names = self._mlp_names(f"{prefix}.eb_module.net", True)
            agg = ops.seg_gather_sum_ln(sv_e["y3"], sv_e["stats"], P[ln_names[6]], P[ln_names[7]], pl.n_rowptr, pl.n_col_edge2, N)
        else:
            agg = ops.seg_gather_sum(e_new.view(2 * E, 64), pl.n_rowptr, pl.n_col_edge2, N)
        if fuse and (self._fuse_mask & 2):
            nbm = _empty(x.device, N, 128) if keep else None
            x_out, _, sv_n = self.mlp3_fwd(P, f"{prefix}.nb_module.net", N,
                                           [Seg(agg, csr=(pl.n_rowptr, pl.n_col_node), scale=pl.inv_deg, save=nbm), Seg(x)],
                                           res=x, saved_segs=[Seg(nbm, width=64, ld=128), Seg(x)] if keep else None, keep=keep)
        else:
            nbm = ops.seg_gather_sum(agg, pl.n_rowptr, pl.n_col_node, N, scale=pl.inv_deg)
            x_out, _, sv_n = self.mlp3_fwd(P, f"{prefix}.nb_module.net", N, [Seg(nbm), Seg(x)], res=x, keep=keep)
        if not keep:
            return x_out, e_out, None
        return x_out, e_out, dict(sv_e=sv_e, sv_n=sv_n, prefix=prefix)

    def _edge_tmp(self, dev):
        if self._etmp is None or self._etmp[0].flat.device != dev:
            e = GradStore(["W1c", "b1", "W2", "b2", "W3", "b3"], [(128, 128), (128,), (128, 128), (128,), (128, 128), (128,)], dev)
            n = GradStore(["W1ab"], [(128, 256)], dev)
            self._etmp = (e, n)
        return self._etmp

    def _edge_gather_adjoint(self, gz1, pl, Wabt):
        N, dev = pl.N, gz1.device
        g_nb = _empty(dev, N, 128)
        if self.csr_fuse and (self._fuse_mask & 4):
            G_s, G_r = _empty(dev, N, 128), _empty(dev, N, 128)
            ops.rowtile_chain(N, [Seg(gz1, csr=(pl.s_rowptr, pl.s_col), save=G_s), Seg(gz1, csr=(pl.r_rowptr, pl.r_col), save=G_r)],
                              [LayerSpec(Wabt)], [g_nb])
        else:
            G_s = ops.seg_gather_sum(gz1, pl.s_rowptr, pl.s_col, N)
            G_r = ops.seg_gather_sum(gz1, pl.r_rowptr, pl.r_col, N)
            ops.rowtile_chain(N, [Seg(G_s), Seg(G_r)], [LayerSpec(Wabt)], [g_nb])
        return g_nb, G_s, G_r

    def _edge_dw(self, grads, names, M, N, tilesE, G_s, G_r, nb, before=(), after=()):
        lib = L.load()
        dev = grads.flat.device
        tmpE, tmpN = self._edge_tmp(dev)
        layE, layN = [("W1c", "b1", 1), ("W2", "b2", 1), ("W3", "b3", 1)][:len(tilesE)], [("W1ab", None, 2)]
        self._workspace(lib.gfv_dw_multi_workspace_floats(M, len(tilesE), self._layers_block(tmpE, layE)[1])
                        + lib.gfv_dw_multi_workspace_floats(N, 2, self._layers_block(tmpN, layN)[1]) + 8, dev)
        w1, slabs1, blen1, used = self._dw_block(tmpE, layE, tilesE, M, reduce=False)
        w2, slabs2, blen2, _ = self._dw_block(tmpN, layN, [self._tile(G_s, 128, Seg(nb)), self._tile(G_r, 128, Seg(nb))], N,
                                              reduce=False, ws_offset=used)
        assert w2 == w1 + 4 * used
        gW1 = grads.view(names[0])
        ob, lb = tmpE.block("b1", layE[-1][1])
        assert lb == grads.block(names[1], names[2 * len(tilesE) - 1])[1]
        ops.reduce_multi([*before,
                          self._piece(w1, gW1.data_ptr() + 4 * 256, slabs1, blen1, 128, rows=128, ld_out=384),
                          self._piece(w1 + 4 * ob, grads.flat.data_ptr() + 4 * grads.off[names[1]], slabs1, blen1, lb),
                          self._piece(w2, gW1.data_ptr(), slabs2, blen2, 256, rows=128, ld_out=384), *after])

    def edge_bwd_factored(self, P, sv, G, grads, pl, gadd):
        prefix, M, N = sv["prefix"], sv["M"], pl.N
        names = self._mlp_names(prefix, True)
        W1, W2, W3 = P[names[0]], P[names[2]], P[names[4]]
        dev = W1.device
        W3t, W2t, W1ct, Wabt = self._T(W3), self._T(W2), self._T(W1, perm="c"), self._T(W1, perm="ab")
        e = sv["segs"][0].t
        if self.fuse_dw and sv.get("fused", sv.get("stats") is not None) and e.stride(0) == 128 and G.stride(0) == 128:
            fused = self._edge_bwd_fused(P, sv, G, grads, pl, gadd, names, (W3t, W2t, W1ct, Wabt))
            if fused is not None:
                return fused
        self._rematerialize(P, sv)
        gz2, gz1, g3, g_e_in = (_empty(dev, M, 128) for _ in range(4))
        part = _empty(dev, ops.ln_rows(M), 2, 128)
        gs = _empty(dev, 3, ops.gscale_ld(M))
        have = ops.rowtile_chain(M, [Seg(G)],
                                 [LayerSpec(W3t, None, L.OP_MUL_DGELU, save=gz2, aux=sv["z2"]),
                                  LayerSpec(W2t, None, L.OP_MUL_DGELU, save=gz1, aux=sv["z1"]), LayerSpec(W1ct)],
                                 [g_e_in], res=[G], in_op=L.IN_LNBWD, in_gamma=P[names[6]], in_aux=sv["y3"], in_save=g3,
                                 ln_partial=part, gadd=gadd[0], gadd_s=gadd[1], gadd_r=gadd[2], gscale=gs, in_stats=sv.get("stats"))
        tiles_n = ops.last_ln_rows()
        s0, s1, s2 = (gs[0], gs[1], gs[2]) if have else (None, None, None)
        g_nb, G_s, G_r = self._edge_gather_adjoint(gz1, pl, Wabt)
        nb = sv["nb"]
        def side():
            self._edge_dw(grads, names, M, N, [self._tile(gz1, 128, Seg(e), gscale=s2),
                                               self._tile(gz2, 128, Seg(sv["z1"]), a_op=1, gscale=s1),
                                               self._tile(g3, 128, Seg(sv["z2"]), a_op=1, gscale=s0)], G_s, G_r, nb,
                          after=[self._ln_piece(part, tiles_n, grads, names[6], names[7])])
        self.defer(side, gz1, gz2, g3, G_s, G_r, nb, e, part, gs, sv["z1"], sv["z2"])
        return g_nb, g_e_in

    def _edge_bwd_fused(self, P, sv, G, grads, pl, gadd, names, Wt):
        M, N = sv["M"], pl.N
        W3t, W2t, W1ct, Wabt = Wt
        dev = G.device
        e = sv["segs"][0].t
        lib = L.load()
        nwg = lib.gfv_rowtile_dw_partials_m(M)
        lean = sv["z2"] is None
        dwp = _empty(dev, nwg, L.DW_FUSED_FLOATS)
        gz1, g_e_in = _empty(dev, M, 128), _empty(dev, M, 128)
        layers = [LayerSpec(W3t, None, L.OP_MUL_DGELU, aux=sv["z2"]), LayerSpec(W2t, None, L.OP_MUL_DGELU, save=gz1, aux=sv["z1"]),
                  LayerSpec(W1ct)]
        gs = _empty(dev, 3, ops.gscale_ld(M))
        kw = dict(res=[G], in_op=L.IN_LNBWD, in_gamma=P[names[6]], in_aux=sv["y3"], in_stats=sv["stats"], gadd=gadd[0], gadd_s=gadd[1],
                  gadd_r=gadd[2], dw_partial=dwp, gscale=gs,
                  rc=(P[names[2]], P[names[3]], P[names[4]], P[names[5]]) if lean else None)
        if not ops.rowtile_chain(M, [Seg(G)], layers, [g_e_in], query_fused=True, **kw):
            return None
        ops.rowtile_chain(M, [Seg(G)], layers, [g_e_in], **kw)
        g_nb, G_s, G_r = self._edge_gather_adjoint(gz1, pl, Wabt)
        nb = sv["nb"]

        def side():
            self._edge_dw(grads, names, M, N, [self._tile(gz1, 128, Seg(e), gscale=gs[2])], G_s, G_r, nb,
                          before=self._fused_pieces(dwp, nwg, grads, names))
        self.defer(side, dwp, gz1, e, G_s, G_r, nb, gs)
        return g_nb, g_e_in

    def gn_bwd(self, P, sv, g_x_out, g_e_out, grads, pl):
        N, E = pl.N, pl.E
        dev = g_x_out.device
        prefix = sv["prefix"]
        W1n = P[f"{prefix}.nb_module.net.0.0.weight"]
        W1t = self._T(W1n, perm=True)
        g_x_in, g_nbm = _empty(dev, N, 128), _empty(dev, N, 64)
        self.mlp3_bwd(P, sv["sv_n"], g_x_out, grads, outs=[g_x_in, (g_nbm, 64)], res=[g_x_out, None], W1t=W1t)
        g_agg = ops.seg_gather_sum(g_nbm, pl.n_rowptr, pl.n_col_node, N, src_scale=pl.inv_deg)
        if "nb" in sv["sv_e"]:
            g_nb, g_e_in = self.edge_bwd_factored(P, sv["sv_e"], g_e_out, grads, pl, (g_agg, pl.es, pl.er))
        else:
            gnb2, g_e_in = _empty(dev, E, 256), _empty(dev, E, 128)
            self.mlp3_bwd(P, sv["sv_e"], g_e_out, grads, outs=[(gnb2, 256), (gnb2.data_ptr() + 512, 256), g_e_in],
                          res=[None, None, g_e_out], gadd=(g_agg, pl.es, pl.er))
            g_nb = ops.seg_gather_sum(gnb2.view(2 * E, 128), pl.n_rowptr, pl.n_col_edge2, N)
        ops.seg_gather_sum(g_nb, pl.n_rowptr, pl.n_col_node, N, out=g_x_in, accumulate=True)
        last = self._defer_mode and self._last_gn
        tail_main, tail_split = self._tail_cfg(pl)
        self.flush(on_main=last and tail_main >= 3, split=tail_split if last else 0)
        return g_x_in, g_e_in

    def trans_fwd(self, P, prefix, xg, emb, pl, keep=True):
        lib = L.load()
        st = L.stream_ptr()
        N, B = pl.N, pl.B
        dev = xg.device
        a = f"{prefix}.Attn"
        fx_in, fx_mid, x_mid = _empty(dev, N, 128), _empty(dev, N, 128), _empty(dev, N, 128)
        ops.rowtile_chain(N, [Seg(xg)],
                          [LayerSpec(P[f"{a}.in_project_fx.weight"], P[f"{a}.in_project_fx.bias"],
                                     stack=P[f"{a}.in_project_x.weight"], bias2=P[f"{a}.in_project_x.bias"])],
                          [fx_mid, x_mid], in_add=emb, in_save=fx_in)
        w = _empty(dev, N, 256)
        temp = P[f"{a}.graph_temperature"]
        partial = _empty(dev, pl.n_chunks, 256, 17)
        if self._slice_fuse:
            L.check(lib.gfv_slice_softmax_token(x_mid.data_ptr(), P[f"{a}.in_project_slice.weight"].data_ptr(),
                                                P[f"{a}.in_project_slice.bias"].data_ptr(), temp.data_ptr(), fx_mid.data_ptr(),
                                                pl.chunk_beg.data_ptr(), pl.chunk_end.data_ptr(), pl.n_chunks, w.data_ptr(),
                                                partial.data_ptr(), st), "slice_softmax_token")
        else:
            L.check(lib.gfv_slice_softmax_fwd(x_mid.data_ptr(), P[f"{a}.in_project_slice.weight"].data_ptr(),
                                              P[f"{a}.in_project_slice.bias"].data_ptr(), temp.data_ptr(), w.data_ptr(), N,
                                              st), "slice_softmax_fwd")
            L.check(lib.gfv_slice_token_partial(w.data_ptr(), fx_mid.data_ptr(), pl.chunk_beg.data_ptr(),
                                                pl.chunk_end.data_ptr(), pl.n_chunks, partial.data_ptr(), st), "token_partial")
        partial, gptr = self._graph_partials(partial, pl)
        token, norm = (_empty(dev, B, 8, 32, 16), _empty(dev, B, 8, 32)) if keep else (None, None)
        attn, out_token = _empty(dev, B, 8, 32, 32) if keep else None, _empty(dev, B, 8, 32, 16)
        L.check(lib.gfv_slice_attention_fwd(partial.data_ptr(), gptr.data_ptr(), B, P[f"{a}.to_q.weight"].data_ptr(),
                                            P[f"{a}.to_k.weight"].data_ptr(), P[f"{a}.to_v.weight"].data_ptr(),
                                            L.ptr(token), L.ptr(norm), L.ptr(attn), out_token.data_ptr(), st),
                "slice_attention_fwd")
        if not keep:
            del partial, fx_mid, x_mid
        out_x = _empty(dev, N, 128)
        L.check(lib.gfv_deslice(w.data_ptr(), out_token.data_ptr(), pl.batch.data_ptr(), out_x.data_ptr(), N,
                                4 if B == 1 else 0, st), "deslice")
        if not keep:
            del w
        fx1, z = (_empty(dev, N, 128), _empty(dev, N, 256)) if keep else (None, None)
        out = _empty(dev, N, 128)
        if not (self._trans_fuse and (N >= self._trans_fuse_min or self._trans_fuse_fwd_small) and ops.trans_mlp_fwd(
                out_x, fx_in, P[f"{a}.to_out.0.weight"], P[f"{a}.to_out.0.bias"], P[f"{prefix}.ln_2.weight"], P[f"{prefix}.ln_2.bias"],
                P[f"{prefix}.mlp.linear_pre.0.weight"], P[f"{prefix}.mlp.linear_pre.0.bias"], P[f"{prefix}.mlp.linear_post.weight"],
                P[f"{prefix}.mlp.linear_post.bias"], fx1, z, out)):
            if not keep:
                fx1, z = _empty(dev, N, 128), _empty(dev, N, 256)
            ops.rowtile_chain(N, [Seg(out_x)], [LayerSpec(P[f"{a}.to_out.0.weight"], P[f"{a}.to_out.0.bias"])], [fx1],
                              res=[fx_in])
            ops.rowtile_chain(N, [Seg(fx1)],
                              [LayerSpec(P[f"{prefix}.mlp.linear_pre.0.weight"], P[f"{prefix}.mlp.linear_pre.0.bias"])],
                              [(z, 256), (z.data_ptr() + 512, 256)], in_op=L.IN_LN, in_gamma=P[f"{prefix}.ln_2.weight"],
                              in_beta=P[f"{prefix}.ln_2.bias"])
            ops.rowtile_chain(N, [Seg(z, width=128, ld=256), Seg(z, width=128, ld=256, offset=128)],
                              [LayerSpec(P[f"{prefix}.mlp.linear_post.weight"], P[f"{prefix}.mlp.linear_post.bias"])], [out],
                              in_op=L.IN_GELU, res=[fx1])
        if not keep:
            return out, None
        sv = dict(prefix=prefix, fx_in=fx_in, fx_mid=fx_mid, x_mid=x_mid, w=w, token=token, norm=norm, attn=attn,
                  out_token=out_token, out_x=out_x, fx1=fx1, z=z)
        return out, sv

    def _graph_partials(self, partial, pl):
        out = _empty(partial.device, pl.B, 256, 17)
        L.check(L.load().gfv_reduce_partials_seg(partial.data_ptr(), pl.gchunk_ptr.data_ptr(), pl.B, 256 * 17,
                                                 out.data_ptr(), L.stream_ptr()), "reduce_partials_seg")
        return out, pl.gunit_ptr

    def _trans_group_alone(self, grads, job, pieces):
        if job is None:
# ... 244 lines not shown
        if sync:
            from . import parallel
            before = parallel.snapshot_normalizer(buffers)

        def update(acc):
            L.check(lib.gfv_normalizer_update(src.data_ptr(), 12, N, 1 if acc else 0, buffers["acc_count"].data_ptr(),
                                              buffers["num_accumulations"].data_ptr(), buffers["acc_sum"].data_ptr(),
                                              buffers["acc_sum_squared"].data_ptr(), pws.data_ptr(),
                                              mean_std.data_ptr(), L.stream_ptr()), "normalizer_update")
        update(accumulate)
        if sync:
            parallel.allreduce_normalizer(buffers, before, self.dist_world, self.dist_group, force=self.dist_force)
            update(False)

    def prep_fwd(self, x, buffers, pl, norm_global, accumulate, want_edge_attr15=True, x_raw=None):
        lib = L.load()
        st = L.stream_ptr()
        N, E, B = pl.N, pl.E, pl.B
        dev = x.device
        assert x.is_contiguous() and x.shape[1] == 12
        if os.environ.get("GFV_PREP_FUSE", "1") == "0" or B > 1024:
            return self._prep_fwd_unfused(x, buffers, pl, norm_global, accumulate, want_edge_attr15, x_raw)
        stats = _empty(dev, B, 6)
        ws = self._prep_ws
        need = lib.gfv_prep_workspace_bytes(B) // 4
        if ws is None or ws.numel() < need or ws.device != dev:
            ws = self._prep_ws = torch.zeros(need, dtype=torch.float32, device=dev)
        mean_std = _empty(dev, 18)
        fused_norm = False
        if norm_global:
            if accumulate:
                self._normalizer_update(x if x_raw is None else x_raw, buffers, N, True, mean_std)
            else:
                fused_norm = True
        own_raw = x_raw is None
        if own_raw:
            x_raw = _empty(dev, N, 12)
        L.check(lib.gfv_prep_stats((x if own_raw else x_raw).data_ptr(), 12, pl.gnode_ptr.data_ptr(), B, stats.data_ptr(), ws.data_ptr(),
                                   x_raw.data_ptr() if own_raw else None,
                                   buffers["acc_count"].data_ptr() if fused_norm else None,
                                   buffers["acc_sum"].data_ptr() if fused_norm else None,
                                   buffers["acc_sum_squared"].data_ptr() if fused_norm else None,
                                   mean_std.data_ptr() if fused_norm else None, st), "prep_stats")
        uv_old = _empty(dev, N, 2)
        ea16 = _empty(dev, E, 16)
        ea15 = _empty(dev, E, 15) if want_edge_attr15 else None
        L.check(lib.gfv_prep_apply(x_raw.data_ptr(), x.data_ptr(), pl.batch.data_ptr(), stats.data_ptr(), pl.uvp_dim.data_ptr(),
                                   mean_std.data_ptr(), 1 if norm_global else 0, uv_old.data_ptr(), N, pl.pos.data_ptr(),
                                   pl.es.data_ptr(), pl.er.data_ptr(), ea16.data_ptr(),
                                   None if ea15 is None else ea15.data_ptr(), E, st), "prep_apply")
        return uv_old, ea16, ea15

    def _prep_fwd_unfused(self, x, buffers, pl, norm_global, accumulate, want_edge_attr15=True, x_raw=None):
        lib = L.load()
        st = L.stream_ptr()
        N, E, B = pl.N, pl.E, pl.B
        dev = x.device
        if x_raw is not None:
            cmdlist.call(x.copy_, x_raw)
        stats = _empty(dev, B, 6)
        nws = _empty(dev, B, 64 * 12)
        L.check(lib.gfv_graph_norm_stats_ws(x.data_ptr(), 12, pl.gnode_ptr.data_ptr(), B, stats.data_ptr(), nws.data_ptr(), st),
                "norm_stats")
        mean_std = _empty(dev, 18)
        if norm_global:
            self._normalizer_update(x, buffers, N, accumulate, mean_std)
        uv_old = _empty(dev, N, 2)
        L.check(lib.gfv_node_prep(x.data_ptr(), 12, pl.batch.data_ptr(), stats.data_ptr(), pl.uvp_dim.data_ptr(),
                                  mean_std.data_ptr(), 1 if norm_global else 0, uv_old.data_ptr(), N, st), "node_prep")
        ea16 = _empty(dev, E, 16)
        ea15 = _empty(dev, E, 15) if want_edge_attr15 else None
        L.check(lib.gfv_edge_attr(x.data_ptr(), 12, pl.pos.data_ptr(), pl.es.data_ptr(), pl.er.data_ptr(), ea16.data_ptr(),
                                  None if ea15 is None else ea15.data_ptr(), E, st), "edge_attr")
        return uv_old, ea16, ea15

    def simulator_fwd(self, P, x, ea16, pl, prefix="simulator", keep=True):
        N, E = pl.N, pl.E
        xn, _, sv_nenc = self.mlp3_fwd(P, f"{prefix}.encoder.nb_encoder", N, [Seg(x, width=12, ld=12)], keep=keep)
        en, _, sv_eenc = self.mlp3_fwd(P, f"{prefix}.encoder.eb_encoder", E, [Seg(ea16, width=15, ld=16)], keep=keep)
        procs = []
        if self.net == "EPD":
            blocks = []
            for ig in range(self.mp):
                xn, en, sv = self.gn_fwd(P, f"{prefix}.GN_block_list.{ig}", xn, en, pl, keep=keep)
                blocks.append(sv)
            procs.append(dict(blocks=blocks, trans=None))
        else:
            pps = [prefix] if self.net == "TransFVGN_v1" else [f"{prefix}.processpr_list.{ip}" for ip in range(self.n_proc)]
            for pp in pps:
                emb = xn
                blocks = []
                for ig in range(self.mp):
                    xn, en, sv = self.gn_fwd(P, f"{pp}.GN_block_list.{ig}", xn, en, pl, keep=keep)
                    blocks.append(sv)
                xn, svt = self.trans_fwd(P, f"{pp}.TransBlock", xn, emb, pl, keep=keep)
                procs.append(dict(blocks=blocks, trans=svt))
        dec, _, sv_dec = self.mlp3_fwd(P, f"{prefix}.decoder.node_decode_module", N, [Seg(xn)], ln=False, keep=keep)
        if not keep:
            return dec, None
        return dec, dict(sv_nenc=sv_nenc, sv_eenc=sv_eenc, procs=procs, sv_dec=sv_dec)

    def simulator_bwd(self, P, sv, g_dec, grads, pl):
        N, E = pl.N, pl.E
        dev = g_dec.device
        g_x = _empty(dev, N, 128)
        self.mlp3_bwd(P, sv["sv_dec"], g_dec, grads, outs=[g_x])
        self.flush()
        g_e = None
        pending = None
        for proc in reversed(sv["procs"]):
            g_emb = None
            if proc["trans"] is not None:
                g_x = self.trans_bwd(P, proc["trans"], g_x, grads, pl, g_add=pending)
                pending = None
                g_emb = g_x
            elif pending is not None:
                g_x, pending = g_x + pending, None
            for blk in reversed(proc["blocks"]):
                if g_e is None:
                    if self._zero_e is None or self._zero_e.shape[0] != E or self._zero_e.device != dev:
                        self._zero_e = torch.zeros((E, 128), dtype=torch.float32, device=dev)
                    g_e = self._zero_e
                self._last_gn = proc is sv["procs"][0] and blk is proc["blocks"][0]
                g_x, g_e = self.gn_bwd(P, blk, g_x, g_e, grads, pl)
            if g_emb is not None:
                pending = g_emb
            if self.bucket_hook is not None and proc is sv["procs"][-1] and len(sv["procs"]) > 1:
                self.flush()
                self.bucket_hook()
        tail = self._tail_cfg(pl)[0] if self._defer_mode else 0
        self.mlp3_bwd(P, sv["sv_eenc"], g_e, grads)
        self.flush(on_main=tail >= 2)
        self.mlp3_bwd(P, sv["sv_nenc"], g_x, grads, g_add=pending)
        self.flush(on_main=tail >= 1)

    def forward(self, P, buffers, x, pl, *, norm_global=True, accumulate=True, want_outputs=True, want_edge_attr15=True,
                before_prep=None, x_raw=None, train_loss=None, keep=True, static_weights=False):
        if static_weights:
            prev = self._wi_static_enter(P)
        else:
            with self.fork():
                prev = self._wi_enter("fwd", P)
        try:
            if before_prep is not None:
                before_prep()
            uv_old, ea16, ea15 = self.prep_fwd(x, buffers, pl, norm_global, accumulate, want_edge_attr15, x_raw=x_raw)
            if not static_weights:
                self.join()
            dec, sv_sim = self.simulator_fwd(P, x, ea16, pl, keep=keep)
        finally:
            if not static_weights:
                self._wi_exit("fwd", prev)
            elif self.f16split:
                ops.set_weight_images(prev)
        if not keep:
            del ea16
        losses, uvp_node, uvp_cell, sv_fvm = self.fvm_fwd(dec, uv_old, pl, want_outputs, train_loss=train_loss, keep=keep)
        return losses, uvp_node, uvp_cell, ea15, (dict(sim=sv_sim, fvm=sv_fvm) if keep else None)

    def backward(self, P, ctx, gloss, grads, pl):
        with self.fork():
            self.prepare_transposes(P)
            prev = self._wi_enter("bwd", P)
        try:
            g_dec = self.fvm_bwd(ctx["fvm"], gloss, pl)
            self.join()
            self.simulator_bwd(P, ctx["sim"], g_dec, grads, pl)
            self.join()
        finally:
            self._wt_live = False
            self._wi_exit("bwd", prev)
        return grads
```

### gen-fvgn-steady_amd/gfv/lib.py

```python
from __future__ import annotations

import ctypes as C
import os

import torch

HERE = os.path.dirname(os.path.abspath(__file__))
LIB_PATH = os.environ.get("GFV_LIB", os.path.join(HERE, "libgfv.so"))

c_float_p = C.c_void_p
c_int_p = C.c_void_p

OP_NONE, OP_BIAS_GELU, OP_MUL_DGELU = 0, 1, 2
IN_NONE, IN_GELU, IN_LN, IN_LNBWD = 0, 1, 2, 3
FIN_PLAIN, FIN_LN, FIN_LNBWD = 0, 1, 2
CHAIN_ROW_OWNER, CHAIN_COLUMN_OWNER = 1, 2
DW_COLSCALE = 8


class Seg(C.Structure):
    _fields_ = [("ptr", C.c_void_p), ("idx", C.c_void_p), ("width", C.c_int32), ("ld", C.c_int32),
                ("csr_rowptr", C.c_void_p), ("csr_scale", C.c_void_p), ("save", C.c_void_p)]


class Layer(C.Structure):
    _fields_ = [("W", C.c_void_p), ("bias", C.c_void_p), ("K", C.c_int32), ("N", C.c_int32), ("op", C.c_int32),
                ("ldw", C.c_int32), ("save", C.c_void_p), ("aux", C.c_void_p), ("Wh", C.c_void_p),
                ("bias2", C.c_void_p)]


class RowtileArgs(C.Structure):
    _fields_ = [
        ("M", C.c_int32), ("nseg", C.c_int32), ("seg", Seg * 3), ("in_add", C.c_void_p), ("in_op", C.c_int32),
        ("nlayers", C.c_int32), ("in_gamma", C.c_void_p), ("in_beta", C.c_void_p), ("in_aux", C.c_void_p),
        ("gadd", C.c_void_p), ("gadd_s", C.c_void_p), ("gadd_r", C.c_void_p), ("in_save", C.c_void_p),
        ("ln_partial", C.c_void_p), ("layer", Layer * 3), ("fin_op", C.c_int32), ("hidden", C.c_int32),
        ("fin_gamma", C.c_void_p), ("fin_beta", C.c_void_p), ("fin_aux", C.c_void_p), ("fin_presave", C.c_void_p),
        ("res", C.c_void_p * 3), ("res_ld", C.c_int32 * 3), ("out_ld", C.c_int32 * 3), ("out", C.c_void_p * 3),
        ("out_nores", C.c_void_p), ("padd", C.c_void_p), ("padd_s", C.c_void_p), ("padd_r", C.c_void_p),
        ("padd_ld", C.c_int32), ("flags", C.c_int32), ("wmax", C.c_void_p),
        ("gscale", C.c_void_p), ("gscale_ld", C.c_int32), ("product_form", C.c_int32),
        ("fin_stats", C.c_void_p), ("in_stats", C.c_void_p), ("dw_partial", C.c_void_p), ("dw_partial_stride", C.c_int64),
        ("dw_in", C.c_void_p), ("dw_in_ld", C.c_int32), ("reserved2_", C.c_int32),
        ("rc_Wh", C.c_void_p * 2), ("rc_bias", C.c_void_p * 2),
    ]


ABI_VERSION = 3

DW_FUSED_FLOATS = 2 * 128 * 128 + 4 * 128
DW_FUSED_WB = 128 * 128 + 128
DW_FUSED_OFF_W3 = 0
DW_FUSED_OFF_W2 = DW_FUSED_WB
DW_FUSED_OFF_LN = 2 * DW_FUSED_WB
assert DW_FUSED_OFF_LN + 256 == DW_FUSED_FLOATS


class WimgDesc(C.Structure):
    _fields_ = [("W", C.c_void_p), ("img", C.c_void_p), ("ldw", C.c_int32), ("N", C.c_int32), ("K", C.c_int32),
                ("reserved", C.c_int32)]


class DwTile(C.Structure):
    _fields_ = [("G", C.c_void_p), ("A", C.c_void_p), ("idx", C.c_void_p), ("in_add", C.c_void_p),
                ("a_gamma", C.c_void_p), ("a_beta", C.c_void_p), ("ldg", C.c_int32), ("n_out", C.c_int32),
                ("width", C.c_int32), ("ld", C.c_int32), ("a_op", C.c_int32), ("ld_out", C.c_int32),
                ("out_off", C.c_int64), ("db_off", C.c_int64), ("gscale", C.c_void_p)]


class ReducePiece(C.Structure):
    _fields_ = [("partial", C.c_void_p), ("out", C.c_void_p), ("chunk_stride", C.c_int64), ("n_chunks", C.c_int32),
                ("rows", C.c_int32), ("cols", C.c_int32), ("ld_in", C.c_int32), ("ld_out", C.c_int32), ("reserved", C.c_int32)]


class TransMlp(C.Structure):
    _fields_ = [("x", C.c_void_p), ("res", C.c_void_p), ("img_out", C.c_void_p), ("img_pre", C.c_void_p), ("img_post", C.c_void_p),
                ("b_out", C.c_void_p), ("b_pre", C.c_void_p), ("b_post", C.c_void_p), ("gamma", C.c_void_p), ("beta", C.c_void_p),
                ("wmax", C.c_void_p), ("fx1", C.c_void_p), ("z", C.c_void_p), ("out", C.c_void_p), ("M", C.c_int32),
                ("reserved", C.c_int32)]


class TransMlpBwd(C.Structure):
    _fields_ = [("g", C.c_void_p), ("g_add", C.c_void_p), ("g_sum", C.c_void_p), ("z", C.c_void_p), ("fx1", C.c_void_p),
                ("img_post_t", C.c_void_p), ("img_pre_t", C.c_void_p), ("img_out_t", C.c_void_p), ("gamma", C.c_void_p),
                ("wmax", C.c_void_p), ("g_z", C.c_void_p), ("g_fx1", C.c_void_p), ("g_out_x", C.c_void_p),
                ("ln_partial", C.c_void_p), ("gscale", C.c_void_p), ("M", C.c_int32), ("reserved", C.c_int32)]


class FvmMesh(C.Structure):
    _fields_ = ([("N", C.c_int32), ("E", C.c_int32), ("C", C.c_int32), ("B", C.c_int32), ("terms", C.c_int32), ("mode", C.c_int32),
                 ("smooth", C.c_int32), ("reserved", C.c_int32)]
                + [(n, C.c_void_p) for n in (
                    "node_type", "batch", "ftype", "cbatch", "gcell_ptr", "pos", "fpos", "y", "centroid", "area", "theta", "sigma",
                    "uvp_dim", "dt", "crow", "kcell", "kS", "frow", "fk", "nfrow", "nfcol2", "nrow", "ncell", "An", "rn",
                    "xo_rowptr", "xo_in", "xo_B", "sumB")])


POOL_MAX_GRAPHS, POOL_MAX_ATTRS, POOL_ROW_HEAD = 64, 56, 8
POOL_COPY, POOL_ADD, POOL_ROWPTR, POOL_FILL = 0, 1, 2, 3


class PoolArgs(C.Structure):
    _fields_ = [("table_host", C.c_void_p), ("table_dev", C.c_void_p), ("n_entries", C.c_int32), ("n_attrs", C.c_int32),
                ("max_graphs", C.c_int32), ("slice_chunk", C.c_int32), ("max_chunks", C.c_int64),
                ("attr_info", C.c_int32 * POOL_MAX_ATTRS), ("dst", C.c_void_p * POOL_MAX_ATTRS),
                ("dst_cap_words", C.c_int64 * POOL_MAX_ATTRS), ("small", C.c_void_p * 6), ("B", C.c_int32),
                ("reserved", C.c_int32), ("idx", C.c_int32 * POOL_MAX_GRAPHS)]


_lib = None

_SIGNATURES = {
    "gfv_pool_args_bytes": (C.c_size_t, []),
    "gfv_pool_table_bytes": (C.c_size_t, [C.c_int32, C.c_int32]),
    "gfv_pool_table_check": (C.c_int, [C.c_void_p, C.c_int32, C.c_int32, C.c_void_p]),
    "gfv_pool_assemble": (C.c_int, [C.POINTER(PoolArgs), C.c_void_p]),
    "gfv_pool_payback": (C.c_int, [C.c_void_p, C.c_void_p, C.c_int32, C.c_int32, C.c_int32, C.c_void_p, C.c_int32, C.c_void_p,
                                   C.c_int64, C.c_void_p, C.c_void_p]),
    "gfv_abi_version": (C.c_int, []),
    "gfv_struct_size": (C.c_int, [C.c_int32]),
    "gfv_seg_gather_sum": (C.c_int, [C.c_void_p, C.c_void_p, C.c_void_p, C.c_void_p, C.c_void_p, C.c_void_p, C.c_int32,
                                     C.c_int32, C.c_int32, C.c_void_p]),
    "gfv_seg_gather_sum_nnz": (C.c_int, [C.c_void_p, C.c_void_p, C.c_void_p, C.c_void_p, C.c_void_p, C.c_void_p, C.c_int32,
                                         C.c_int32, C.c_int32, C.c_int64, C.c_void_p]),
    "gfv_seg_gather_sum_ex": (C.c_int, [C.c_void_p, C.c_void_p, C.c_void_p, C.c_void_p, C.c_void_p, C.c_void_p, C.c_int32,
                                        C.c_int32, C.c_int32, C.c_int64, C.c_int64, C.c_void_p]),
    "gfv_seg_gather_sum_ln": (C.c_int, [C.c_void_p, C.c_void_p, C.c_void_p, C.c_void_p, C.c_void_p, C.c_void_p, C.c_void_p, C.c_int32,
                                        C.c_int64, C.c_int64, C.c_void_p]),
    "gfv_transpose_batch": (C.c_int, [C.c_void_p, C.c_int32, C.c_int32, C.c_int32, C.c_void_p]),
    "gfv_status_flags": (C.c_int, [C.POINTER(C.c_int32)]),
    "gfv_status_mirror": (C.c_int, [C.POINTER(C.POINTER(C.c_int32))]),
    "gfv_status_publish": (C.c_int, [C.c_void_p]),
    "gfv_profile_enable": (C.c_int, [C.c_int]),
    "gfv_profile_collect": (C.c_int, [C.c_int, C.POINTER(C.c_double)]),
    "gfv_profile_reset": (C.c_int, []),
    "gfv_profile_set_sizes": (C.c_int, [C.c_double, C.c_double]),
    "gfv_gather_pair": (C.c_int, [C.c_void_p, C.c_void_p, C.c_void_p, C.c_void_p, C.c_void_p, C.c_int32, C.c_int32,
                                  C.c_void_p]),
# ... 275 lines not shown
```

### gen-fvgn-steady_amd/gfv/ops.py

```python
from __future__ import annotations

import ctypes as C

import torch

from . import lib as L


def _p(t):
    return None if t is None else t.data_ptr()


def seg_gather_sum(src, rowptr, col, n_rows, scale=None, src_scale=None, out=None, accumulate=False):
    lib = L.load()
    F = src.shape[-1]
    L.f32c(src)
    if out is None:
        assert not accumulate
        out = torch.empty((n_rows, F), dtype=torch.float32, device=src.device)
    rc = lib.gfv_seg_gather_sum_ex(_p(src), _p(L.i32c(rowptr)), _p(L.i32c(col)), _p(scale), _p(src_scale), _p(out),
                                   n_rows, F, 1 if accumulate else 0, col.shape[0], src.shape[0], L.stream_ptr())
    L.check(rc, "gfv_seg_gather_sum")
    return out

# ... 11 lines not shown

def gather_pair(a, s, r, base=None, out=None):
    lib = L.load()
    F = a.shape[-1]
    E = s.shape[0]
    if out is None:
        out = torch.empty((E, 2 * F), dtype=torch.float32, device=a.device)
    rc = lib.gfv_gather_pair(_p(L.f32c(a)), _p(L.i32c(s)), _p(L.i32c(r)), _p(base), _p(out), E, F, L.stream_ptr())
    L.check(rc, "gfv_gather_pair")
    return out


def transpose(w, out=None, col0=0, ncols=None):
    lib = L.load()
    rows, cols = w.shape
    ncols = cols - col0 if ncols is None else ncols
    if out is None:
        out = torch.empty((ncols, rows), dtype=torch.float32, device=w.device)
    rc = lib.gfv_transpose(L.f32c(w).data_ptr() + 4 * col0, cols, _p(out), rows, ncols, L.stream_ptr())
    L.check(rc, "gfv_transpose")
    return out


def reduce_partials(partial, n_chunks, n, out=None, accumulate=False):
    lib = L.load()
    if out is None:
        out = torch.empty((n,), dtype=torch.float32, device=partial.device)
    rc = lib.gfv_reduce_partials(_p(partial), n_chunks, n, _p(out), 1 if accumulate else 0, L.stream_ptr())
    L.check(rc, "gfv_reduce_partials")
    return out


def reduce_multi(pieces):
    lib = L.load()
    arr = (L.ReducePiece * len(pieces))()
    for a, p in zip(arr, pieces):
        a.partial = p["partial"].data_ptr() if torch.is_tensor(p["partial"]) else p["partial"]
        a.out = p["out"].data_ptr() if torch.is_tensor(p["out"]) else p["out"]
        a.n_chunks, a.chunk_stride, a.rows, a.cols = p["n_chunks"], p["chunk_stride"], p["rows"], p["cols"]
        a.ld_in = p.get("ld_in", p["cols"])
        a.ld_out = p.get("ld_out", p["cols"])
    L.check(lib.gfv_reduce_multi(arr, len(pieces), L.stream_ptr()), "gfv_reduce_multi")


def csr_prologue_enabled():
    import os
    return os.environ.get("GFV_CSR_FUSE", "1") != "0"


def rowtile_tiles(M):
    return (M + 63) // 64


def ln_rows(M):
    return (M + 31) // 32


def last_ln_rows():
    return L.load().gfv_rowtile_last_ln_rows()


def gscale_ld(M):
    return (M + 127) // 128 * 8


class Seg:

    def __init__(self, t, idx=None, width=None, ld=None, offset=0, csr=None, scale=None, save=None):
        self.t, self.idx = t, idx
        self.width = t.shape[-1] if width is None else width
        self.ld = t.stride(0) if ld is None else ld
        self.offset = offset
        self.csr, self.scale, self.save = csr, scale, save
        assert csr is None or idx is None

    def fill(self, cs):
        cs.ptr = self.t.data_ptr() + 4 * self.offset
        cs.idx = _p(self.idx) if self.csr is None else self.csr[1].data_ptr()
        cs.width = self.width
        cs.ld = self.ld
        cs.csr_rowptr = None if self.csr is None else self.csr[0].data_ptr()
        cs.csr_scale = _p(self.scale)
        cs.save = _p(self.save)


class LayerSpec:
    def __init__(self, W, bias=None, op=L.OP_NONE, save=None, aux=None, stack=None, bias2=None, stack_cols=None):
        self.W, self.bias, self.op, self.save, self.aux = W, bias, op, save, aux
        self.stack, self.bias2, self.stack_cols = stack, bias2, stack_cols


class WeightImages:

    def __init__(self, device, wmax):
        self.device, self.wmax = device, wmax
        self.images = {}
        self.valid = set()
        self.static = []
        self._desc, self._desc_keys, self._max_frags = None, (), 0
        self._retired = []
        self._bf = None

    def add_static(self, tensors):
        for t in tensors:
            st = t.untyped_storage()
            self.static.append((st.data_ptr(), st.data_ptr() + st.nbytes()))
        self.static.sort()

    def _is_static(self, ptr):
        import bisect
        i = bisect.bisect_right(self.static, (ptr, 1 << 62)) - 1
        return i >= 0 and self.static[i][0] <= ptr < self.static[i][1]

    @staticmethod
    def _parts(key, img):
        if key[0] != "stack":
            return [(key, img.data_ptr())]
        per = img.numel() // (len(key) - 1)
        return [(k, img.data_ptr() + i * per) for i, k in enumerate(key[1:])]

    @staticmethod
    def _upload(items, device):
        parts = [pt for key, img in items for pt in WeightImages._parts(key, img)]
        descs = (L.WimgDesc * len(parts))()
        for d, (key, dst) in zip(descs, parts):
            d.W, d.img, d.ldw, d.N, d.K = key[0], dst, key[1], key[2], key[3]
        return torch.frombuffer(bytearray(bytes(descs)), dtype=torch.uint8).to(device), len(parts)

    def lookup(self, W, stack=None):
        key = (W.data_ptr(), W.stride(0), W.shape[0], W.shape[1])
        if stack is not None:
            assert W.shape == stack.shape and W.shape[0] == 128
            key = ("stack", key, (stack.data_ptr(), stack.stride(0), stack.shape[0], stack.shape[1]))
        bf = L.load().gfv_f16split_enabled() == 3
        if bf != self._bf:
            self._bf = bf
            self.invalidate()
            if self.images and not torch.cuda.is_current_stream_capturing():
                self.build()
        img = self.images.get(key)
        if img is not None:
            return img.data_ptr() if key in self.valid else 0
        blocks = key[1:] if key[0] == "stack" else (key,)
        if not all(self._is_static(k[0]) for k in blocks) or torch.cuda.is_current_stream_capturing():
            return 0
        lib = L.load()
        nbytes = sum(lib.gfv_weight_image_bytes(k[2], k[3]) for k in blocks)
        img = torch.empty((nbytes,), dtype=torch.uint8, device=self.device)
        desc, nd = self._upload([(key, img)], self.device)
        L.check(lib.gfv_weight_images(desc.data_ptr(), nd, img.numel() // 32, self.wmax.data_ptr(), L.stream_ptr()),
                "gfv_weight_images")
        self.images[key] = img
        self.valid.add(key)
        return img.data_ptr()

    def build(self):
        if not self.images:
            return
        if len(self._desc_keys) != len(self.images) and not torch.cuda.is_current_stream_capturing():
            self._desc_keys = tuple(self.images)
            self._retired.append(self._desc)
            self._desc, self._ndesc = self._upload(list(self.images.items()), self.device)
            self._max_frags = max(img.numel() for img in self.images.values()) // 32
        if self._desc is None:
            return
        L.check(L.load().gfv_weight_images(self._desc.data_ptr(), self._ndesc, self._max_frags,
                                           self.wmax.data_ptr(), L.stream_ptr()), "gfv_weight_images")
        self._bf = L.load().gfv_f16split_enabled() == 3
        self.valid = set(self._desc_keys)

    def invalidate(self):
        self.valid = set()


_WI = None


def stack_ready(Wa, Wb, rows=False):
    return (_WI is not None and L.load().gfv_f16split_enabled() and Wa.shape == Wb.shape and Wa.shape[0] == 128
            and _WI.lookup(Wa, Wb) != 0)


def set_weight_images(wi):
    global _WI
    prev, _WI = _WI, wi
    return prev


def rowtile_chain(M, segs, layers, outs, *, in_add=None, in_op=L.IN_NONE, in_gamma=None, in_beta=None, in_aux=None,
                  gadd=None, gadd_s=None, gadd_r=None, in_save=None, ln_partial=None, fin_op=L.FIN_PLAIN,
                  fin_gamma=None, fin_beta=None, fin_aux=None, fin_presave=None, res=None, out_nores=None,
                  padd=None, padd_s=None, padd_r=None, wimg=None, gscale=None, family=0, fin_stats=None, in_stats=None,
                  dw_partial=None, query_fused=False, rc=None):
    lib = L.load()
    wi = wimg if wimg is not None else _WI
    if layers[-1].stack is not None:
        ly = layers[-1]
        h = wi.lookup(ly.W, ly.stack) if (wi is not None and len(layers) == 1 and lib.gfv_f16split_enabled()) else 0
        if not h:
            assert len(layers) == 1 and len(outs) == 2 and res is None and out_nores is None
            kw = dict(in_add=in_add, in_op=in_op, in_gamma=in_gamma, in_beta=in_beta, wimg=wimg)
            rowtile_chain(M, segs, [LayerSpec(ly.W, ly.bias, ly.op)], [outs[0]], in_save=in_save, **kw)
            rowtile_chain(M, segs, [LayerSpec(ly.stack, ly.bias2, ly.op)], [outs[1]], **kw)
            return
    a = L.RowtileArgs()
    a.M = M
    a.nseg = len(segs)
    for i, s in enumerate(segs):
        s.fill(a.seg[i])
    a.in_add = _p(in_add)
    a.in_op = in_op
    a.nlayers = len(layers)
    a.in_gamma, a.in_beta, a.in_aux = _p(in_gamma), _p(in_beta), _p(in_aux)
    a.gadd, a.gadd_s, a.gadd_r = _p(gadd), _p(gadd_s), _p(gadd_r)
    a.in_save, a.ln_partial = _p(in_save), _p(ln_partial)
    for i, ly in enumerate(layers):
        cl = a.layer[i]
        stacked = ly.stack is not None or ly.stack_cols is not None
        cl.W, cl.bias, cl.bias2 = (None if stacked else _p(ly.W)), _p(ly.bias), _p(ly.bias2)
        cl.N = ly.W.shape[0] * (2 if ly.stack is not None else 1)
        cl.K = ly.W.shape[1] * (2 if ly.stack_cols is not None else 1)
        assert ly.W.stride(1) == 1
        cl.ldw = 0 if (ly.stack is not None or ly.stack_cols is not None) else ly.W.stride(0)
        cl.op = ly.op
        cl.save, cl.aux = _p(ly.save), _p(ly.aux)
    if wi is not None:
        hs = [wi.lookup(ly.W, ly.stack if ly.stack is not None else ly.stack_cols) for ly in layers]
        if all(hs):
            for i, h in enumerate(hs):
                a.layer[i].Wh = h
            a.wmax = wi.wmax.data_ptr()
    a.fin_op = fin_op
    a.fin_gamma, a.fin_beta, a.fin_aux, a.fin_presave = _p(fin_gamma), _p(fin_beta), _p(fin_aux), _p(fin_presave)
    for i, o in enumerate(outs):
        t, ld = o if isinstance(o, tuple) else (o, o.stride(0))
        a.out[i] = t.data_ptr() if torch.is_tensor(t) else t
        a.out_ld[i] = ld
    if res is not None:
        for i, o in enumerate(res):
            if o is None:
                continue
            t, ld = o if isinstance(o, tuple) else (o, o.stride(0))
            a.res[i] = t.data_ptr() if torch.is_tensor(t) else t
            a.res_ld[i] = ld
    a.out_nores = _p(out_nores)
    a.flags = family
    a.fin_stats, a.in_stats = _p(fin_stats), _p(in_stats)
    if dw_partial is not None:
        a.dw_partial, a.dw_partial_stride = dw_partial.data_ptr(), dw_partial.stride(0)
    if rc is not None:
        W2, b2, W3, b3 = rc
        h2, h3 = (wi.lookup(W2), wi.lookup(W3)) if wi is not None else (0, 0)
        if not (h2 and h3):
            if query_fused:
                return False
            raise RuntimeError("recompute form: no split-fp16 image of the forward's second / third Linear")
        a.rc_Wh[0], a.rc_Wh[1] = h2, h3
        a.rc_bias[0], a.rc_bias[1] = _p(b2), _p(b3)
    if padd is not None:
        a.padd, a.padd_s, a.padd_r, a.padd_ld = _p(padd), _p(padd_s), _p(padd_r), padd.stride(0)
    if gscale is not None:
        assert gscale.dim() == 2 and gscale.shape[0] >= 3 and gscale.shape[1] >= gscale_ld(M)
        a.gscale, a.gscale_ld = gscale.data_ptr(), gscale.stride(0)
    if query_fused:
        return bool(lib.gfv_rowtile_fuses_dw(C.byref(a)))
    rc = lib.gfv_rowtile_chain(C.byref(a), L.stream_ptr())
    L.check(rc, "gfv_rowtile_chain")
    return gscale is not None and lib.gfv_rowtile_last_path() >= 5


def trans_mlp_fwd(x, res, Wout, bout, gamma, beta, Wpre, bpre, Wpost, bpost, fx1, z, out):
    lib = L.load()
    if _WI is None or not lib.gfv_f16split_enabled():
        return False
    hs = (_WI.lookup(Wout), _WI.lookup(Wpre), _WI.lookup(Wpost))
    if not all(hs):
        return False
    a = L.TransMlp()
    a.x, a.res, a.img_out, a.img_pre, a.img_post = x.data_ptr(), res.data_ptr(), hs[0], hs[1], hs[2]
    a.b_out, a.b_pre, a.b_post = _p(bout), _p(bpre), _p(bpost)
    a.gamma, a.beta, a.wmax = gamma.data_ptr(), beta.data_ptr(), _WI.wmax.data_ptr()
    a.fx1, a.z, a.out, a.M = _p(fx1), _p(z), out.data_ptr(), x.shape[0]
    L.check(lib.gfv_trans_mlp_fwd(C.byref(a), L.stream_ptr()), "gfv_trans_mlp_fwd")
    return True


def trans_mlp_bwd(g, g_add, g_sum, z, fx1, Wpost_t, Wpre_t, Wout_t, gamma, g_z, g_fx1, g_out_x, ln_partial, gscale):
    lib = L.load()
    if _WI is None or not lib.gfv_f16split_enabled():
        return False
    hs = (_WI.lookup(Wpost_t), _WI.lookup(Wpre_t), _WI.lookup(Wout_t))
    if not all(hs):
        return False
    a = L.TransMlpBwd()
    a.g, a.g_add, a.g_sum, a.z, a.fx1 = g.data_ptr(), _p(g_add), _p(g_sum), z.data_ptr(), fx1.data_ptr()
    a.img_post_t, a.img_pre_t, a.img_out_t = hs
    a.gamma, a.wmax = gamma.data_ptr(), _WI.wmax.data_ptr()
    a.g_z, a.g_fx1, a.g_out_x = g_z.data_ptr(), g_fx1.data_ptr(), g_out_x.data_ptr()
    a.ln_partial, a.gscale, a.M = _p(ln_partial), _p(gscale), g.shape[0]
    L.check(lib.gfv_trans_mlp_bwd(C.byref(a), L.stream_ptr()), "gfv_trans_mlp_bwd")
    return True


def linear_dw(G, n_out, segs, M, *, ldg=None, in_add=None, a_op=0, a_gamma=None, a_beta=None, dW=None, db=None,
              want_db=True, accumulate=False, workspace=None, g_offset=0, gscale=None, col_scale=False):
    if col_scale:
        assert a_op == 0
        a_op = L.DW_COLSCALE
    lib = L.load()
    K = sum(s.width for s in segs)
    dev = G.device
    if dW is None:
        dW = torch.empty((n_out, K), dtype=torch.float32, device=dev)
    if db is None and want_db:
        db = torch.empty((n_out,), dtype=torch.float32, device=dev)
    need = lib.gfv_linear_dw_workspace_floats(M, n_out, K)
    if workspace is None or workspace.numel() < need:
        workspace = torch.empty((max(need, 1),), dtype=torch.float32, device=dev)
    cs = (L.Seg * 3)()
    for i, s in enumerate(segs):
        s.fill(cs[i])
    ldg = G.stride(0) if ldg is None else ldg
    rc = lib.gfv_linear_dw_gs(G.data_ptr() + 4 * g_offset, ldg, n_out, cs, len(segs), _p(in_add), a_op, _p(a_gamma),
                              _p(a_beta), M, _p(dW), _p(gscale), _p(db), _p(workspace), 1 if accumulate else 0,
                              L.stream_ptr())
    L.check(rc, "gfv_linear_dw_gs")
    return dW, db
```

### include/gfv.h

```cpp
#ifndef GFV_H_
#define GFV_H_
#include <stddef.h>
#include <stdint.h>

#ifdef __cplusplus
extern "C" {
#endif

#define GFV_ABI_VERSION 3
int gfv_abi_version(void);
int gfv_struct_size(int32_t which);

int gfv_seg_gather_sum(const float* src, const int32_t* rowptr, const int32_t* col, const float* scale,
                       const float* src_scale, float* out, int32_t n_rows, int32_t F, int32_t accumulate, void* stream);

int gfv_seg_gather_sum_nnz(const float* src, const int32_t* rowptr, const int32_t* col, const float* scale,
                           const float* src_scale, float* out, int32_t n_rows, int32_t F, int32_t accumulate,
                           int64_t nnz_hint, void* stream);

int gfv_seg_gather_sum_ex(const float* src, const int32_t* rowptr, const int32_t* col, const float* scale,
                          const float* src_scale, float* out, int32_t n_rows, int32_t F, int32_t accumulate,
                          int64_t nnz_hint, int64_t n_src_hint, void* stream);

int gfv_seg_gather_sum_ln(const float* y, const float* stats, const float* gamma, const float* beta, const int32_t* rowptr,
                          const int32_t* col, float* out, int32_t n_rows, int64_t nnz_hint, int64_t n_src_hint, void* stream);

int gfv_gather_pair(const float* a, const int32_t* s, const int32_t* r, const float* base, float* out,
                    int32_t n_edges, int32_t F, void* stream);

typedef struct {
  const float* ptr;
  const int32_t* idx;
  int32_t width;
  int32_t ld;
  const int32_t* csr_rowptr;
  const float* csr_scale;
  float* save;
} gfv_seg_t;

enum {
  GFV_OP_NONE = 0,
  GFV_OP_BIAS_GELU = 1,
  GFV_OP_MUL_DGELU = 2
};
enum { GFV_IN_NONE = 0, GFV_IN_GELU = 1, GFV_IN_LN = 2, GFV_IN_LNBWD = 3 };
enum { GFV_CHAIN_ROW_OWNER = 1,
       GFV_CHAIN_COLUMN_OWNER = 2    };
enum { GFV_FIN_PLAIN = 0, GFV_FIN_LN = 1, GFV_FIN_LNBWD = 2 };

typedef struct {
  const float* W;
  const float* bias;
  int32_t K, N;
  int32_t op;
  int32_t ldw;
  float* save;
  const float* aux;
  const void* Wh;
  const float* bias2;
} gfv_layer_t;

typedef struct {
  int32_t M;
  int32_t nseg;
  gfv_seg_t seg[3];
  const float* in_add;
  int32_t in_op;
  int32_t nlayers;
  const float* in_gamma;
  const float* in_beta;
  const float* in_aux;
  const float* gadd;
  const int32_t* gadd_s;
  const int32_t* gadd_r;
  float* in_save;
  float* ln_partial;
  gfv_layer_t layer[3];
  int32_t fin_op;
  int32_t hidden;
  const float* fin_gamma;
  const float* fin_beta;
  const float* fin_aux;
  float* fin_presave;
  const float* res[3];
  int32_t res_ld[3];
  int32_t out_ld[3];
  float* out[3];
  float* out_nores;
  const float* padd;
  const int32_t* padd_s;
  const int32_t* padd_r;
  int32_t padd_ld;
  int32_t flags;
  const float* wmax;
  float* gscale;
  int32_t gscale_ld;
  int32_t product_form;
  float* fin_stats;
  const float* in_stats;
  float* dw_partial;
  int64_t dw_partial_stride;
  const float* dw_in;
  int32_t dw_in_ld;
  int32_t reserved2_;
  const void* rc_Wh[2];
  const float* rc_bias[2];
} gfv_rowtile_args_t;
enum { GFV_DW_FUSED_FLOATS = 2 * 128 * 128 + 4 * 128 };
int gfv_rowtile_dw_partials(void);
int gfv_rowtile_dw_partials_m(int32_t M);
int gfv_rowtile_fuses_dw(const gfv_rowtile_args_t* args);

int gfv_rowtile_tiles(int32_t M);
int gfv_rowtile_ln_rows(int32_t M);
int gfv_rowtile_last_ln_rows(void);
int gfv_get_limit(int32_t which);
int gfv_set_limit(int32_t which, int32_t value);
const char* gfv_limit_name(int32_t which);
int gfv_rowtile_chain(const gfv_rowtile_args_t* args, void* stream);
int gfv_rowtile_last_path(void);

typedef struct {
  const float* W;
  void* img;
  int32_t ldw, N, K, reserved;
} gfv_wimg_desc_t;
size_t gfv_weight_image_bytes(int32_t N, int32_t K);
int gfv_f16split_enabled(void);
int gfv_set_f16split(int32_t on);
int gfv_set_f16split_thread(int32_t on);
int gfv_hidden_size(void);
int gfv_set_hidden_size(int32_t h);
int gfv_weight_absmax(const gfv_wimg_desc_t* descs_dev, int32_t n_desc, float* wmax, void* stream);
int gfv_weight_images(const gfv_wimg_desc_t* descs_dev, int32_t n_desc, int64_t max_frags, const float* wmax,
                      void* stream);
int gfv_weight_images_form(const float* wmax);

int gfv_dw_chunks(int32_t M);
int gfv_linear_dw(const float* G, int32_t ldg, int32_t n_out, const gfv_seg_t* segs, int32_t nseg,
                  const float* in_add, int32_t a_gelu, int32_t M, float* dW, float* db, float* workspace,
                  int32_t accumulate, void* stream);
int gfv_linear_dw_gs(const float* G, int32_t ldg, int32_t n_out, const gfv_seg_t* segs, int32_t nseg,
                     const float* in_add, int32_t a_op, const float* a_gamma, const float* a_beta, int32_t M,
                     float* dW, const float* gscale, float* db, float* workspace, int32_t accumulate, void* stream);
size_t gfv_linear_dw_workspace_floats(int32_t M, int32_t n_out, int32_t K);
int gfv_linear_dw_ex(const float* G, int32_t ldg, int32_t n_out, const gfv_seg_t* segs, int32_t nseg,
                     const float* in_add, int32_t a_op, const float* a_gamma, const float* a_beta, int32_t M,
                     float* dW, int32_t reserved, float* db, float* workspace, int32_t accumulate, void* stream);

typedef struct {
  const float* G;
  const float* A;
  const int32_t* idx;
  const float* in_add;
  const float* a_gamma;
  const float* a_beta;
  int32_t ldg, n_out, width, ld;
  int32_t a_op;
  int32_t ld_out;
  int64_t out_off;
  int64_t db_off;
  const float* gscale;
} gfv_dw_tile_t;
enum { GFV_DW_COLSCALE = 8 };
enum { GFV_FLAG_DW_RANGE = 1,
       GFV_FLAG_CHAIN_RANGE = 2 };
int gfv_status_flags(int32_t* flags_out);
int gfv_status_mirror(int32_t** host_word);
int gfv_status_publish(void* stream);
int gfv_dw_slabs(int32_t M, int32_t ntiles, int32_t* rows_per_slab);
size_t gfv_dw_multi_workspace_floats(int32_t M, int32_t ntiles, int64_t block_floats);
int gfv_dw_multi(const gfv_dw_tile_t* tiles, int32_t ntiles, int32_t M, int64_t block_floats, float* workspace,
                 float* grad_block, int32_t accumulate, void* stream);

int gfv_reduce_partials(const float* partial, int32_t n_chunks, int32_t n, float* out, int32_t accumulate,
                        void* stream);

int gfv_reduce_partials_2d(const float* partial, int32_t n_chunks, int64_t chunk_stride, int32_t rows, int32_t cols,
                           int32_t ld_out, float* out, void* stream);

typedef struct {
  const float* partial;
  float* out;
  int64_t chunk_stride;
  int32_t n_chunks, rows, cols, ld_in, ld_out, reserved;
} gfv_reduce_piece_t;
int gfv_reduce_multi(const gfv_reduce_piece_t* pieces, int32_t n_pieces, void* stream);

int gfv_reduce_partials_seg(const float* partial, const int32_t* seg_ptr, int32_t n_seg, int32_t n, float* out,
                            void* stream);

// ... 269 lines not shown
```

Baseline: 284.8.

## Fuse narrow-input first-layer weight gradient into backward chain and drop unused outputs

Adds a DW1N path to the column-chain backward kernel: when the first Linear has a narrow input (width up to 15), its weight and bias gradients are computed in-kernel with MFMA from an LDS tile of the input, so the input-gradient output and a separate dW GEMM are no longer needed. The forward chain can now skip writing its final output when only presave/stats are consumed (no_out). The last processor block's edge backward can run with a null edge-gradient segment instead of a materialised zero tensor. Together these cut HBM traffic and kernel launches, at the cost of more LDS use, more template variants and more validation logic.

```diff
diff --git a/gen-fvgn-steady_amd/csrc/cfwd.hip b/gen-fvgn-steady_amd/csrc/cfwd.hip
--- a/gen-fvgn-steady_amd/csrc/cfwd.hip
+++ b/gen-fvgn-steady_amd/csrc/cfwd.hip
@@ -215,7 +215,7 @@
     for (int n = 0; n < NT; ++n) { gam[n] = ld4(A.fin_gamma + c0 + 16 * n); bet[n] = ld4(A.fin_beta + c0 + 16 * n); }
   }
   float4 rres[TG][NT];
-  if (A.res[0]) {
+  if (A.res[0] && A.out[0]) {
 #pragma unroll
     for (int q = 0; q < TG; ++q) {
       const float* rp = A.res[0] + (size_t)min(row0 + 16 * q + j, A.M - 1) * A.res_ld[0] + c0;
@@ -306,7 +306,7 @@
         const float4 ga = gam[n], be = bet[n];
         float o[4] = {(y[q][4 * n + 0] - mean) * rstd * ga.x + be.x, (y[q][4 * n + 1] - mean) * rstd * ga.y + be.y,
                       (y[q][4 * n + 2] - mean) * rstd * ga.z + be.z, (y[q][4 * n + 3] - mean) * rstd * ga.w + be.w};
-        if (live) {
+        if (live && A.out[0]) {
           if (A.out_nores) st4(A.out_nores + (size_t)row * 128 + c0 + 16 * n, o);
           if (A.res[0]) { o[0] += rres[q][n].x; o[1] += rres[q][n].y; o[2] += rres[q][n].z; o[3] += rres[q][n].w; }
           st4(A.out[0] + (size_t)row * A.out_ld[0] + c0 + 16 * n, o);
@@ -350,7 +350,7 @@
     if (L.save && !cf_al16(L.save)) return 0;
   }
   if (a->layer[2].save) return 0;
-  if (!a->out[0] || a->out[1] || a->out[2] || (!dec && ((a->out_ld[0] & 3) || !cf_al16(a->out[0]))) || a->res[1] || a->res[2]) return 0;
+  if ((!a->out[0] && (dec || a->out_nores || !a->fin_presave || !a->fin_stats)) || a->out[1] || a->out[2] || (!dec && ((a->out_ld[0] & 3) || !cf_al16(a->out[0]))) || a->res[1] || a->res[2]) return 0;
   if (a->res[0] && ((a->res_ld[0] & 3) || !cf_al16(a->res[0]))) return 0;
   if ((a->out_nores && !cf_al16(a->out_nores)) || (a->fin_presave && !cf_al16(a->fin_presave)) ||
       (!dec && (!cf_al16(a->fin_gamma) || !cf_al16(a->fin_beta))))
diff --git a/gen-fvgn-steady_amd/csrc/colchain.hip b/gen-fvgn-steady_amd/csrc/colchain.hip
--- a/gen-fvgn-steady_amd/csrc/colchain.hip
+++ b/gen-fvgn-steady_amd/csrc/colchain.hip
@@ -27,7 +27,6 @@
   if (a->flags & GFV_CHAIN_ROW_OWNER) return false;
   if (!(a->flags & GFV_CHAIN_COLUMN_OWNER) && (!on || a->M < min_m)) return false;
   if (!a->dw_partial || a->dw_partial_stride < GFV_DW_FUSED_FLOATS || !a->in_stats || !a->wmax) return false;
-  if (a->dw_in) return false;
   const bool noout = a->nlayers == 2;
   const bool rc = a->rc_Wh[0] != nullptr;
   if (rc && (!a->rc_Wh[1] || a->dw_in || !al16(a->rc_Wh[0]) || !al16(a->rc_Wh[1]) || (a->rc_bias[0] && !al16(a->rc_bias[0])) ||
@@ -35,9 +34,15 @@
     return false;
   if (!rc && a->rc_Wh[1]) return false;
   if ((a->nlayers != 3 && !noout) || a->in_op != GFV_IN_LNBWD || a->fin_op != GFV_FIN_PLAIN || a->nseg != 1) return false;
-  if (noout && (a->layer[1].op != GFV_OP_MUL_DGELU || a->layer[1].save || a->res[0] || a->gadd || a->dw_in || !a->out[0])) return false;
+  if (a->dw_in) {
+    if (!noout || rc || a->dw_in_width < 1 || a->dw_in_width > 15 || a->dw_in_ld < a->dw_in_width || (reinterpret_cast<size_t>(a->dw_in) & 3) ||
+        (size_t)a->M * (size_t)a->dw_in_ld >= ((size_t)1 << 29) || a->dw_partial_stride < GFV_DW_FUSED_FLOATS_IN || a->out[0] || a->gscale)
+      return false;
+  }
+  if (noout && (a->layer[1].op != GFV_OP_MUL_DGELU || a->layer[1].save || a->res[0] || a->gadd || (!a->out[0] && !a->dw_in))) return false;
+  if (!a->seg[0].ptr && (!a->gadd || a->res[0] || noout)) return false;
   if (a->seg[0].width != 128 || a->seg[0].idx || a->seg[0].csr_rowptr || a->seg[0].save || a->seg[0].ld != 128 || !al16(a->seg[0].ptr)) return false;
-  if (a->M > (1 << 22) || a->out_ld[0] != 128 || (a->res[0] && a->res_ld[0] != 128) || (a->dw_in && a->dw_in_ld != 128)) return false;
+  if (a->M > (1 << 22) || a->out_ld[0] != 128 || (a->res[0] && a->res_ld[0] != 128)) return false;
   if (a->layer[0].op != GFV_OP_MUL_DGELU || a->layer[1].op != GFV_OP_MUL_DGELU || (!noout && a->layer[2].op != GFV_OP_NONE)) return false;
   for (int l = 0; l < a->nlayers; ++l) {
     const gfv_layer_t& L = a->layer[l];
@@ -47,7 +52,7 @@
   }
   if ((!rc && (!a->in_aux || !al16(a->in_aux))) || !a->in_gamma || !al16(a->in_gamma) || a->ln_partial || a->padd) return false;
   const bool out2 = !noout && a->layer[2].N == 192;
-  if (!a->out[0] || (out2 ? (!a->out[1] || a->out_ld[1] != 64 || !al16(a->out[1]) || a->dw_in) : a->out[1] != nullptr) || a->out[2] ||
+  if ((!a->out[0] && !a->dw_in) || (out2 ? (!a->out[1] || a->out_ld[1] != 64 || !al16(a->out[1]) || a->dw_in) : a->out[1] != nullptr) || a->out[2] ||
       a->res[1] || a->res[2] || a->out_nores)
     return false;
   if ((a->out_ld[0] & 3) || !al16(a->out[0]) || (a->res[0] && ((a->res_ld[0] & 3) || !al16(a->res[0])))) return false;
diff --git a/gen-fvgn-steady_amd/csrc/colchain_kernel.h b/gen-fvgn-steady_amd/csrc/colchain_kernel.h
--- a/gen-fvgn-steady_amd/csrc/colchain_kernel.h
+++ b/gen-fvgn-steady_amd/csrc/colchain_kernel.h
@@ -122,7 +122,7 @@
   }
 }
 
-template <bool BF>
+template <bool BF, bool GFRAG = true>
 __device__ __forceinline__ void cb_hidden_bwd(CcCtx& c, int q, const floatx4& acc, float inv_in, const float4& z, float sg,
                                               char* gout, char* aout, float (&v)[4]) {
   const gfv_f2 z01 = {z.x, z.y}, z23 = {z.z, z.w};
@@ -136,8 +136,13 @@
   const float mq = max3_abs(max3_abs(0.f, v[0], v[1]), v[2], v[3]) * sg;
   const float ma = max3_abs(max3_abs(0.f, a[0], a[1]), a[2], a[3]) * (60000.0f / CC_SH_LIMIT);
   c.mabs = fmaxf(c.mabs, q < c.ngt ? fmaxf(mq, ma) : 0.f);
-  cc_put_frag<BF>(gout, q, c, v, sg);
+  if (GFRAG) cc_put_frag<BF>(gout, q, c, v, sg);
   cc_put_frag<BF>(aout, q, c, a, CC_SH);
+}
+
+__device__ __forceinline__ float* cb_dw1n_block(char* xbuf, int w, int q) { return reinterpret_cast<float*>(xbuf + w * 4096 + q * 1024); }
+__device__ __forceinline__ void cb_dw1n_put(char* xbuf, const CcCtx& c, int q, const float (&v)[4]) {
+  *reinterpret_cast<float4*>(cb_dw1n_block(xbuf, c.w, q) + c.j * 16 + 4 * c.g) = make_float4(v[0], v[1], v[2], v[3]);
 }
 
 __device__ __forceinline__ char* cb_own_slot(char* xbuf, int q, const CcCtx& c) {
@@ -236,11 +241,13 @@
 template <int LOWP, bool GADD, bool OUT2 = false, bool NOOUT = false, bool RC = false>
 __global__ __launch_bounds__(64 * CC_W, 2) void colchain_bwd_kernel(const gfv_rowtile_args_t A, int* status) {
   constexpr int TG = CB_TG;
-  __shared__ __attribute__((aligned(16))) char lds[CbLds::TOTAL + (RC ? CbLds::BUF : 0)];
+  constexpr bool DW1N = NOOUT && !RC;
+  __shared__ __attribute__((aligned(16))) char lds[CbLds::TOTAL + (RC ? CbLds::BUF : 0) + (DW1N ? 4096 : 0)];
   char* b0 = lds + CbLds::B0;
   char* b1 = lds + CbLds::B1;
   char* b2 = lds + CbLds::B2;
   char* b3 = lds + CbLds::TOTAL;
+  float* xtile = reinterpret_cast<float*>(lds + CbLds::TOTAL);
   float* part = reinterpret_cast<float*>(lds + CbLds::PART);
   float* smax = reinterpret_cast<float*>(lds + CbLds::SMAX);
 
@@ -281,6 +288,8 @@
 #pragma unroll
   for (int kt = 0; kt < 8; ++kt) dw3[kt] = dw2[kt] = floatx4{0.f, 0.f, 0.f, 0.f};
   float dgam[4] = {0.f, 0.f, 0.f, 0.f}, dbet[4] = {0.f, 0.f, 0.f, 0.f};
+  const bool dw1n = DW1N && A.dw_in != nullptr;
+  floatx4 dw1 = floatx4{0.f, 0.f, 0.f, 0.f};
   float sacc = 0.f;
   float scap = 3.0e38f;
 
@@ -582,6 +591,20 @@
     CT(6);
     cc_barrier();
     CT(7);
+    float xr[2] = {0.f, 0.f};
+    if constexpr (DW1N) {
+      if (dw1n) {
+        const cb_rsrc xin = cb_buf(A.dw_in, ((size_t)(A.M - 1) * A.dw_in_ld + A.dw_in_width) * 4);
+        const int xw = A.dw_in_width;
+#pragma unroll
+        for (int u = 0; u < 2; ++u) {
+          const int rt = 8 * c.w + 4 * u + c.g, row = c.row0 + rt;
+          const bool livex = (rt >> 4) < c.ngt && row < c.M && c.j < xw;
+          const float t = __builtin_bit_cast(float, __builtin_amdgcn_raw_buffer_load_b32(xin, livex ? (row * A.dw_in_ld + c.j) * 4 : CB_OFF_DEAD, 0, 0));
+          xr[u] = c.j == xw ? 1.0f : t;
+        }
+      }
+    }
     {
       const float inv_in = 1.0f / s2s;
       floatx4 a0, a1;
@@ -599,8 +622,14 @@
           cb_hidden_bwd_dg<LOWP == 2>(c, 2 * p, a0, inv_in, d0, s1s, b0, v0);
           cb_hidden_bwd_dg<LOWP == 2>(c, 2 * p + 1, a1, inv_in, d1, s1s, b0, v1);
         } else {
-          cb_hidden_bwd<LOWP == 2>(c, 2 * p, a0, inv_in, zq[2 * p], s1s, b0, b2, v0);
-          cb_hidden_bwd<LOWP == 2>(c, 2 * p + 1, a1, inv_in, zq[2 * p + 1], s1s, b0, b2, v1);
+          cb_hidden_bwd<LOWP == 2, !NOOUT>(c, 2 * p, a0, inv_in, zq[2 * p], s1s, b0, b2, v0);
+          cb_hidden_bwd<LOWP == 2, !NOOUT>(c, 2 * p + 1, a1, inv_in, zq[2 * p + 1], s1s, b0, b2, v1);
+        }
+        if constexpr (DW1N) {
+          if (dw1n) {
+            cb_dw1n_put(b0, c, 2 * p, v0);
+            cb_dw1n_put(b0, c, 2 * p + 1, v1);
+          }
         }
         cb_st4(B.save1, offS[2 * p], v0);
         cb_st4(B.save1, offS[2 * p + 1], v1);
@@ -613,6 +642,12 @@
       for (int T = 0; T < 4; ++T) {
         wh[T] = __builtin_bit_cast(gfv_f16x8, __builtin_amdgcn_raw_buffer_load_b128(w2, woff + T * 16384, 0, 0));
         wl[T] = __builtin_bit_cast(gfv_f16x8, __builtin_amdgcn_raw_buffer_load_b128(w2, woff + T * 16384 + 1024, 0, 0));
+      }
+    }
+    if constexpr (DW1N) {
+      if (dw1n) {
+        xtile[128 * c.w + c.lane] = xr[0];
+        xtile[128 * c.w + 64 + c.lane] = xr[1];
       }
     }
     float4 rr[NOOUT ? 1 : TG];
@@ -660,6 +695,23 @@
         }
       }
     }
+    if constexpr (DW1N) {
+      if (dw1n) {
+        int tvar = 0;
+        asm volatile("" : "+v"(tvar));
+        const int l4 = (c.lane + tvar) * 4;
+        const char* ga = b0 + c.w * 4096 + l4;
+        const char* xa = lds + CbLds::TOTAL + l4;
+#pragma unroll
+        for (int q = 0; q < TG; ++q) {
+          if (q >= c.ngt) break;
+#pragma unroll
+          for (int st = 0; st < 4; ++st)
+            dw1 = __builtin_amdgcn_mfma_f32_16x16x4f32(*reinterpret_cast<const float*>(ga + 1024 * q + 256 * st),
+                                                       *reinterpret_cast<const float*>(xa + 1024 * q + 256 * st), dw1, 0, 0, 0);
+        }
+      }
+    }
     CT(10);
     if constexpr (RC) {
       cb_load_dy_stats(B, c, next_row0, in);
@@ -701,6 +753,17 @@
         blk[2 * 16384 + 128 + nb] = db2[r] * (is * r2);
       }
     }
+    if constexpr (DW1N) {
+      if (dw1n) {
+        const int xw = A.dw_in_width;
+#pragma unroll
+        for (int r = 0; r < 4; ++r) {
+          const int n = 16 * c.w + 4 * c.g + r;
+          if (c.j < xw) blk[GFV_DW_FUSED_OFF_IN + n * xw + c.j] = dw1[r];
+          else if (c.j == xw) blk[GFV_DW_FUSED_OFF_IN + 128 * xw + n] = dw1[r];
+        }
+      }
+    }
 #pragma unroll
     for (int r = 0; r < 4; ++r) {
       const float dg = gfv_row16_sum(dgam[r]), db = gfv_row16_sum(dbet[r]);
diff --git a/gen-fvgn-steady_amd/csrc/rowtile.hip b/gen-fvgn-steady_amd/csrc/rowtile.hip
--- a/gen-fvgn-steady_amd/csrc/rowtile.hip
+++ b/gen-fvgn-steady_amd/csrc/rowtile.hip
@@ -128,6 +128,16 @@
     if (args->seg[i].width < 1 || args->seg[i].width > 128) return GFV_ERR_ARG;
   for (int l = 0; l + 1 < args->nlayers; ++l)
     if (args->layer[l].N != 128 || args->layer[l + 1].K != 128) return GFV_ERR_ARG;
+  for (int i = 0; i < args->nseg; ++i) {
+    if (args->seg[i].ptr) continue;
+    if (i != 0 || args->nseg != 1 || !args->gadd || args->res[0] || !args->dw_partial || args->in_op != GFV_IN_LNBWD || args->nlayers != 3)
+      return GFV_ERR_ARG;
+  }
+  if (!args->out[0] && !(args->dw_in && args->dw_partial && args->nlayers == 2 && args->in_op == GFV_IN_LNBWD)) {
+    if (args->nlayers != 3 || args->fin_op != GFV_FIN_LN || !args->fin_presave || !args->fin_stats || !args->layer[0].save ||
+        !args->layer[1].save || args->out_nores || args->out[1] || args->out[2] || args->dw_partial)
+      return GFV_ERR_ARG;
+  }
   int k0 = 0;
   for (int i = 0; i < args->nseg; ++i) k0 += args->seg[i].width;
   if (k0 != args->layer[0].K) return GFV_ERR_ARG;
@@ -195,14 +205,15 @@
       if (args->layer[l].save) by += 4.0 * args->M * args->layer[l].N;
       if (args->layer[l].aux) by += 4.0 * args->M * args->layer[l].N;
     }
-    by += 4.0 * args->M * (double)args->layer[0].K + 4.0 * args->M * (double)last.N;
+    if (args->seg[0].ptr) by += 4.0 * args->M * (double)args->layer[0].K;
+    if (args->out[0]) by += 4.0 * args->M * (double)last.N;
     for (int i = 0; i < args->nseg; ++i) if (args->seg[i].idx) by += 4.0 * args->M;
     if (args->in_aux || args->fin_aux) by += 4.0 * args->M * 128.0;
     if (args->in_save) by += 4.0 * args->M * 128.0;
     if (args->fin_presave) by += 4.0 * args->M * 128.0;
     if (args->out_nores) by += 4.0 * args->M * 128.0;
     if (args->padd) by += 4.0 * args->M * 258.0;
-    for (int c = 0; c < 3; ++c) if (args->res[c]) by += 4.0 * args->M * 128.0;
+    for (int c = 0; c < 3; ++c) if (args->res[c] && args->out[c]) by += 4.0 * args->M * 128.0;
     const int lnm = args->in_op == GFV_IN_LNBWD ? 1 : (args->fin_op == GFV_FIN_LNBWD ? 2 : 0);
     int kind = fast_t ? GFV_K_TCHAIN0 + lnm : GFV_K_TCHAIN_RAG;
     for (int i = 0; i < args->nseg; ++i)
diff --git a/gen-fvgn-steady_amd/csrc/tchain_kernel.h b/gen-fvgn-steady_amd/csrc/tchain_kernel.h
--- a/gen-fvgn-steady_amd/csrc/tchain_kernel.h
+++ b/gen-fvgn-steady_amd/csrc/tchain_kernel.h
@@ -728,7 +728,7 @@
             if (!live) rs = 8.5070592e37f;
             group_scale_out(A.gscale + (size_t)A.nlayers * A.gscale_ld + rowgroup, rs, lane);
           }
-          if (live) {
+          if (live && out) {
             if (pass == 0 && A.out_nores) {
 #pragma unroll
               for (int nt = 0; nt < 8; ++nt) st4(A.out_nores + mc * 128 + 16 * nt + 4 * g, v[nt]);
diff --git a/gen-fvgn-steady_amd/gfv/engine.py b/gen-fvgn-steady_amd/gfv/engine.py
--- a/gen-fvgn-steady_amd/gfv/engine.py
+++ b/gen-fvgn-steady_amd/gfv/engine.py
@@ -118,6 +118,7 @@
         self._tail_main = int(os.environ.get("GFV_TAIL_MAIN", "2"))
         self._tail_split = int(os.environ.get("GFV_TAIL_SPLIT", "1"))
         self._fuse_noout = os.environ.get("GFV_FUSE_NOOUT", "1") != "0"
+        self._fuse_dw1n = os.environ.get("GFV_FUSE_DW1N", "1") != "0"
         self._fuse_dw_min = int(os.environ.get("GFV_COLCHAIN_BWD_MIN_M", "2048"))
         self._cbwd_max_fixed = None
         self._wi, self._wi_key, self._wmax, self._wi_abs = None, None, None, None
@@ -128,6 +129,7 @@
         self._fvm_cnt = None
         self._fvm_fuse = os.environ.get("GFV_FVM_FUSE", "1") != "0"
         self._agg_ln = os.environ.get("GFV_AGG_LN", "1") != "0"
+        self._last_edge_lean = os.environ.get("GFV_LAST_EDGE_LEAN", "1") != "0"
         self._side, self._sides = None, []
         self._keep = []
         self.dist_world, self.dist_group, self.dist_force = 1, None, False
@@ -346,7 +348,7 @@
                 f"{lin}.4.bias"] + ([f"{prefix}.1.weight", f"{prefix}.1.bias"] if ln else [])
 
     def mlp3_fwd(self, P, prefix, M, segs, *, ln=True, res=None, in_add=None, want_nores=False, keep=True, w1=None,
-                 padd=None, saved_segs=None, nores_from_saved=False):
+                 padd=None, saved_segs=None, nores_from_saved=False, no_out=False):
         names = self._mlp_names(prefix, ln)
         W1, b1, W2, b2, W3, b3 = (P[n] for n in names[:6])
         if w1 is not None:
@@ -370,9 +372,12 @@
             z1 = z2 = None
             y3 = _empty(dev, M, 128) if from_saved else None
             stats = _empty(dev, M, 2) if from_saved else None
-        out = _empty(dev, M, nout)
         if want_nores and nores_from_saved and y3 is not None and stats is not None and nout == 128:
             want_nores = False
+            no_out = no_out and keep and z2 is not None
+        else:
+            no_out = False
+        out = None if no_out else _empty(dev, M, nout)
         nores = _empty(dev, M, 128) if want_nores else None
         ops.rowtile_chain(
             M, segs,
@@ -454,6 +459,8 @@
         dev = G.device
         lib = L.load()
         nwg = lib.gfv_rowtile_dw_partials_m(M)
+        if outs is None and self._fuse_dw1n and self._mlp3_bwd_fused_in(P, sv, G, grads, names, W3t, W2t, g_add, nwg):
+            return True
         dwp = _empty(dev, nwg, L.DW_FUSED_FLOATS)
         gz1 = _empty(dev, M, 128)
         gs = _empty(dev, 3, ops.gscale_ld(M))
@@ -478,6 +485,24 @@
         self.defer(side, dwp, gz1, gs, sv["in_add"], *[sg.t for sg in segs], *[sg.idx for sg in segs])
         return True
 
+    def _mlp3_bwd_fused_in(self, P, sv, G, grads, names, W3t, W2t, g_add, nwg):
+        segs = sv["segs"]
+        sg = segs[0]
+        if len(segs) != 1 or sg.idx is not None or sg.csr is not None or sv["in_add"] is not None or sv["z2"] is None:
+            return False
+        M, dev = sv["M"], G.device
+        dwp = _empty(dev, nwg, L.DW_FUSED_FLOATS_IN)
+        layers = [LayerSpec(W3t, None, L.OP_MUL_DGELU, aux=sv["z2"]), LayerSpec(W2t, None, L.OP_MUL_DGELU, aux=sv["z1"])]
+        kw = dict(in_op=L.IN_LNBWD, in_gamma=P[names[6]], in_aux=sv["y3"], in_stats=sv["stats"], dw_partial=dwp, in_add=g_add, dw_in=sg)
+        if not ops.rowtile_chain(M, [Seg(G)], layers, [None], query_fused=True, **kw):
+            return False
+        ops.rowtile_chain(M, [Seg(G)], layers, [None], **kw)
+        first = self._piece(dwp.data_ptr() + 4 * L.DW_FUSED_OFF_IN, self._gview2(grads, names[0], names[1]), nwg,
+                            L.DW_FUSED_FLOATS_IN, 128 * (sg.width + 1))
+        pieces = [first] + self._fused_pieces(dwp, nwg, grads, names)
+        self.defer(lambda: ops.reduce_multi(pieces), dwp)
+        return True
+
     @staticmethod
     def _gview2(grads, n0, n1):
         off, length = grads.block(n0, n1)
@@ -494,7 +519,7 @@
         return self._piece(part, self._gview2(grads, gamma, beta), n_rows, 256, 256)
 
     def _fused_pieces(self, dwp, nwg, grads, names):
-        base, FL, WB = dwp.data_ptr(), L.DW_FUSED_FLOATS, L.DW_FUSED_WB
+        base, FL, WB = dwp.data_ptr(), dwp.stride(0), L.DW_FUSED_WB
         return [self._piece(base + 4 * L.DW_FUSED_OFF_W2, self._gview2(grads, names[2], names[3]), nwg, FL, WB),
                 self._piece(base + 4 * L.DW_FUSED_OFF_W3, self._gview2(grads, names[4], names[5]), nwg, FL, WB),
                 self._piece(base + 4 * L.DW_FUSED_OFF_LN, self._gview2(grads, names[6], names[7]), nwg, FL, 256)]
@@ -580,7 +605,7 @@
     def _put(grads, name, value):
         cmdlist.call(grads.view(name).copy_, value.reshape(grads.shape[name]))
 
-    def gn_fwd(self, P, prefix, x, e, pl, keep=True):
+    def gn_fwd(self, P, prefix, x, e, pl, keep=True, last=False):
         N, E = pl.N, pl.E
         fuse = self.csr_fuse
         if self.factor:
@@ -595,12 +620,14 @@
                 ops.rowtile_chain(N, [Seg(nb)], [LayerSpec(W1[:, 0:128], stack=W1[:, 128:256])],
                                   [(pab, 256), (pab.data_ptr() + 512, 256)])
             e_out, e_new, sv_e = self.mlp3_fwd(P, f"{prefix}.eb_module.net", E, [Seg(e)], res=e, want_nores=True,
-                                               w1=W1[:, 256:384], padd=(pab, pl.es, pl.er), nores_from_saved=self._agg_ln, keep=keep)
+                                               w1=W1[:, 256:384], padd=(pab, pl.es, pl.er), nores_from_saved=self._agg_ln, keep=keep,
+                                               no_out=last and self._last_edge_lean)
             sv_e["nb"] = nb
         else:
             nb = ops.seg_gather_sum(x, pl.n_rowptr, pl.n_col_node, N)
             e_out, e_new, sv_e = self.mlp3_fwd(P, f"{prefix}.eb_module.net", E, [Seg(nb, pl.es), Seg(nb, pl.er), Seg(e)],
-                                               res=e, want_nores=True, nores_from_saved=self._agg_ln, keep=keep)
+                                               res=e, want_nores=True, nores_from_saved=self._agg_ln, keep=keep,
+                                               no_out=last and self._last_edge_lean)
         if e_new is None:
             ln_names = self._mlp_names(f"{prefix}.eb_module.net", True)
             agg = ops.seg_gather_sum_ln(sv_e["y3"], sv_e["stats"], P[ln_names[6]], P[ln_names[7]], pl.n_rowptr, pl.n_col_edge2, N)
@@ -664,6 +691,12 @@
         dev = W1.device
         W3t, W2t, W1ct, Wabt = self._T(W3), self._T(W2), self._T(W1, perm="c"), self._T(W1, perm="ab")
         e = sv["segs"][0].t
+        if G is None:
+            if self.fuse_dw and sv.get("fused", sv.get("stats") is not None) and e.stride(0) == 128:
+                fused = self._edge_bwd_fused(P, sv, None, grads, pl, gadd, names, (W3t, W2t, W1ct, Wabt))
+                if fused is not None:
+                    return fused
+            G = self._zero_edge_grad(M, dev)
         if self.fuse_dw and sv.get("fused", sv.get("stats") is not None) and e.stride(0) == 128 and G.stride(0) == 128:
             fused = self._edge_bwd_fused(P, sv, G, grads, pl, gadd, names, (W3t, W2t, W1ct, Wabt))
             if fused is not None:
@@ -692,8 +725,9 @@
     def _edge_bwd_fused(self, P, sv, G, grads, pl, gadd, names, Wt):
         M, N = sv["M"], pl.N
         W3t, W2t, W1ct, Wabt = Wt
-        dev = G.device
         e = sv["segs"][0].t
+        dev = e.device
+        gseg = ops.NullSeg() if G is None else Seg(G)
         lib = L.load()
         nwg = lib.gfv_rowtile_dw_partials_m(M)
         lean = sv["z2"] is None
@@ -705,9 +739,9 @@
         kw = dict(res=[G], in_op=L.IN_LNBWD, in_gamma=P[names[6]], in_aux=sv["y3"], in_stats=sv["stats"], gadd=gadd[0], gadd_s=gadd[1],
                   gadd_r=gadd[2], dw_partial=dwp, gscale=gs,
                   rc=(P[names[2]], P[names[3]], P[names[4]], P[names[5]]) if lean else None)
-        if not ops.rowtile_chain(M, [Seg(G)], layers, [g_e_in], query_fused=True, **kw):
+        if not ops.rowtile_chain(M, [gseg], layers, [g_e_in], query_fused=True, **kw):
             return None
-        ops.rowtile_chain(M, [Seg(G)], layers, [g_e_in], **kw)
+        ops.rowtile_chain(M, [gseg], layers, [g_e_in], **kw)
         g_nb, G_s, G_r = self._edge_gather_adjoint(gz1, pl, Wabt)
         nb = sv["nb"]
 
@@ -726,6 +760,8 @@
         g_x_in, g_nbm = _empty(dev, N, 128), _empty(dev, N, 64)
         self.mlp3_bwd(P, sv["sv_n"], g_x_out, grads, outs=[g_x_in, (g_nbm, 64)], res=[g_x_out, None], W1t=W1t)
         g_agg = ops.seg_gather_sum(g_nbm, pl.n_rowptr, pl.n_col_node, N, src_scale=pl.inv_deg)
+        if g_e_out is None and "nb" not in sv["sv_e"]:
+            g_e_out = self._zero_edge_grad(E, dev)
         if "nb" in sv["sv_e"]:
             g_nb, g_e_in = self.edge_bwd_factored(P, sv["sv_e"], g_e_out, grads, pl, (g_agg, pl.es, pl.er))
         else:
@@ -1136,7 +1172,7 @@
         if self.net == "EPD":
             blocks = []
             for ig in range(self.mp):
-                xn, en, sv = self.gn_fwd(P, f"{prefix}.GN_block_list.{ig}", xn, en, pl, keep=keep)
+                xn, en, sv = self.gn_fwd(P, f"{prefix}.GN_block_list.{ig}", xn, en, pl, keep=keep, last=ig == self.mp - 1)
                 blocks.append(sv)
             procs.append(dict(blocks=blocks, trans=None))
         else:
@@ -1145,7 +1181,8 @@
                 emb = xn
                 blocks = []
                 for ig in range(self.mp):
-                    xn, en, sv = self.gn_fwd(P, f"{pp}.GN_block_list.{ig}", xn, en, pl, keep=keep)
+                    xn, en, sv = self.gn_fwd(P, f"{pp}.GN_block_list.{ig}", xn, en, pl, keep=keep,
+                                             last=pp is pps[-1] and ig == self.mp - 1)
                     blocks.append(sv)
                 xn, svt = self.trans_fwd(P, f"{pp}.TransBlock", xn, emb, pl, keep=keep)
                 procs.append(dict(blocks=blocks, trans=svt))
@@ -1153,6 +1190,11 @@
         if not keep:
             return dec, None
         return dec, dict(sv_nenc=sv_nenc, sv_eenc=sv_eenc, procs=procs, sv_dec=sv_dec)
+
+    def _zero_edge_grad(self, E, dev):
+        if self._zero_e is None or self._zero_e.shape[0] != E or self._zero_e.device != dev:
+            self._zero_e = torch.zeros((E, 128), dtype=torch.float32, device=dev)
+        return self._zero_e
 
     def simulator_bwd(self, P, sv, g_dec, grads, pl):
         N, E = pl.N, pl.E
@@ -1171,10 +1213,8 @@
             elif pending is not None:
                 g_x, pending = g_x + pending, None
             for blk in reversed(proc["blocks"]):
-                if g_e is None:
-                    if self._zero_e is None or self._zero_e.shape[0] != E or self._zero_e.device != dev:
-                        self._zero_e = torch.zeros((E, 128), dtype=torch.float32, device=dev)
-                    g_e = self._zero_e
+                if g_e is None and not self._last_edge_lean:
+                    g_e = self._zero_edge_grad(E, dev)
                 self._last_gn = proc is sv["procs"][0] and blk is proc["blocks"][0]
                 g_x, g_e = self.gn_bwd(P, blk, g_x, g_e, grads, pl)
             if g_emb is not None:
diff --git a/gen-fvgn-steady_amd/gfv/lib.py b/gen-fvgn-steady_amd/gfv/lib.py
--- a/gen-fvgn-steady_amd/gfv/lib.py
+++ b/gen-fvgn-steady_amd/gfv/lib.py
@@ -41,7 +41,7 @@
         ("padd_ld", C.c_int32), ("flags", C.c_int32), ("wmax", C.c_void_p),
         ("gscale", C.c_void_p), ("gscale_ld", C.c_int32), ("product_form", C.c_int32),
         ("fin_stats", C.c_void_p), ("in_stats", C.c_void_p), ("dw_partial", C.c_void_p), ("dw_partial_stride", C.c_int64),
-        ("dw_in", C.c_void_p), ("dw_in_ld", C.c_int32), ("reserved2_", C.c_int32),
+        ("dw_in", C.c_void_p), ("dw_in_ld", C.c_int32), ("dw_in_width", C.c_int32),
         ("rc_Wh", C.c_void_p * 2), ("rc_bias", C.c_void_p * 2),
     ]
 
@@ -54,6 +54,8 @@
 DW_FUSED_OFF_W2 = DW_FUSED_WB
 DW_FUSED_OFF_LN = 2 * DW_FUSED_WB
 assert DW_FUSED_OFF_LN + 256 == DW_FUSED_FLOATS
+DW_FUSED_OFF_IN = DW_FUSED_FLOATS
+DW_FUSED_FLOATS_IN = DW_FUSED_FLOATS + 128 * 16
 
 
 class WimgDesc(C.Structure):
diff --git a/gen-fvgn-steady_amd/gfv/ops.py b/gen-fvgn-steady_amd/gfv/ops.py
--- a/gen-fvgn-steady_amd/gfv/ops.py
+++ b/gen-fvgn-steady_amd/gfv/ops.py
@@ -117,6 +117,17 @@
         cs.csr_rowptr = None if self.csr is None else self.csr[0].data_ptr()
         cs.csr_scale = _p(self.scale)
         cs.save = _p(self.save)
+
+
+class NullSeg(Seg):
+
+    def __init__(self, width=128):
+        self.t, self.idx, self.width, self.ld, self.offset = None, None, width, width, 0
+        self.csr, self.scale, self.save = None, None, None
+
+    def fill(self, cs):
+        cs.ptr, cs.idx, cs.width, cs.ld = None, None, self.width, self.ld
+        cs.csr_rowptr, cs.csr_scale, cs.save = None, None, None
 
 
 class LayerSpec:
@@ -226,7 +237,7 @@
                   gadd=None, gadd_s=None, gadd_r=None, in_save=None, ln_partial=None, fin_op=L.FIN_PLAIN,
                   fin_gamma=None, fin_beta=None, fin_aux=None, fin_presave=None, res=None, out_nores=None,
                   padd=None, padd_s=None, padd_r=None, wimg=None, gscale=None, family=0, fin_stats=None, in_stats=None,
-                  dw_partial=None, query_fused=False, rc=None):
+                  dw_partial=None, query_fused=False, rc=None, dw_in=None):
     lib = L.load()
     wi = wimg if wimg is not None else _WI
     if layers[-1].stack is not None:
@@ -268,6 +279,9 @@
     a.fin_op = fin_op
     a.fin_gamma, a.fin_beta, a.fin_aux, a.fin_presave = _p(fin_gamma), _p(fin_beta), _p(fin_aux), _p(fin_presave)
     for i, o in enumerate(outs):
+        if o is None:
+            a.out_ld[i] = 128
+            continue
         t, ld = o if isinstance(o, tuple) else (o, o.stride(0))
         a.out[i] = t.data_ptr() if torch.is_tensor(t) else t
         a.out_ld[i] = ld
@@ -283,6 +297,9 @@
     a.fin_stats, a.in_stats = _p(fin_stats), _p(in_stats)
     if dw_partial is not None:
         a.dw_partial, a.dw_partial_stride = dw_partial.data_ptr(), dw_partial.stride(0)
+    if dw_in is not None:
+        assert dw_in.idx is None and dw_in.csr is None
+        a.dw_in, a.dw_in_ld, a.dw_in_width = dw_in.t.data_ptr() + 4 * dw_in.offset, dw_in.ld, dw_in.width
     if rc is not None:
         W2, b2, W3, b3 = rc
         h2, h3 = (wi.lookup(W2), wi.lookup(W3)) if wi is not None else (0, 0)
diff --git a/include/gfv.h b/include/gfv.h
--- a/include/gfv.h
+++ b/include/gfv.h
@@ -102,11 +102,13 @@
   int64_t dw_partial_stride;
   const float* dw_in;
   int32_t dw_in_ld;
-  int32_t reserved2_;
+  int32_t dw_in_width;
   const void* rc_Wh[2];
   const float* rc_bias[2];
 } gfv_rowtile_args_t;
-enum { GFV_DW_FUSED_FLOATS = 2 * 128 * 128 + 4 * 128 };
+enum { GFV_DW_FUSED_FLOATS = 2 * 128 * 128 + 4 * 128,
+       GFV_DW_FUSED_OFF_IN = GFV_DW_FUSED_FLOATS,
+       GFV_DW_FUSED_FLOATS_IN = GFV_DW_FUSED_FLOATS + 128 * 16 };
 int gfv_rowtile_dw_partials(void);
 int gfv_rowtile_dw_partials_m(int32_t M);
 int gfv_rowtile_fuses_dw(const gfv_rowtile_args_t* args);
```

Result: no change. 286.3, median of 6 (+0.5%).
